# Antiparadox/Spartan-BN254

Hardware: AMD Instinct MI355X
Metric: msm_points_per_s (higher is better)
Workload: dtype u32; 1 GPU; synthetic BN254 G1 MSM, 2^20 uniform Fr scalars x distinct bases per GPU, inputs resident in HBM; steps_in_flight=6

## Files before the change

include/sbn254.h:

```cpp
#ifndef SBN254_H
#define SBN254_H
#include <stddef.h>
#include <stdint.h>
#ifdef __cplusplus
extern "C" {
#endif

#define SBN_OK 0
#define SBN_EINVAL (-1)
#define SBN_EHIP (-2)
#define SBN_ENODEV (-3)
#define SBN_ENOMEM (-4)

#define SBN_SCALARS_MONT 1u
#define SBN_POINTS_MONT 2u

typedef struct sbn_ctx sbn_ctx;
typedef struct sbn_bases sbn_bases;
typedef struct sbn_table sbn_table;

int sbn_ctx_create(int device, sbn_ctx** out);
void sbn_ctx_destroy(sbn_ctx* ctx);
const char* sbn_last_error(const sbn_ctx* ctx);
int sbn_ctx_set_stream(sbn_ctx* ctx, void* hip_stream);
int sbn_ctx_sync(sbn_ctx* ctx);
const char* sbn_version(void);

int sbn_dev_alloc(sbn_ctx* ctx, size_t bytes, void** out_dev);
int sbn_dev_free(sbn_ctx* ctx, void* dev);
int sbn_dev_upload(sbn_ctx* ctx, void* dst_dev, const void* src_host, size_t bytes);
int sbn_dev_download(sbn_ctx* ctx, void* dst_host, const void* src_dev, size_t bytes);

int sbn_msm(sbn_ctx* ctx, const uint8_t* scalars, const uint8_t* points, size_t n, uint32_t flags,
            uint8_t out_xy[64], int* out_is_inf);

int sbn_msm_jacobian(sbn_ctx* ctx, const uint8_t* scalars, const uint8_t* points_xyz, size_t n, uint32_t flags,
                     uint8_t out_xy[64], int* out_is_inf);

int sbn_bases_upload(sbn_ctx* ctx, const uint8_t* G_xy, size_t n, const uint8_t* h_xy, uint32_t flags, sbn_bases** out);
void sbn_bases_free(sbn_ctx* ctx, sbn_bases* b);
size_t sbn_bases_len(const sbn_bases* b);
int sbn_bases_precompute(sbn_ctx* ctx, sbn_bases* b, size_t max_bytes, int* window_bits);
int sbn_gens_new(sbn_ctx* ctx, size_t n, const uint8_t* label, size_t label_len, uint8_t* out_xy, sbn_bases** out);

int sbn_bases_synthetic(sbn_ctx* ctx, size_t n, uint64_t first, const uint8_t s0[32], const uint8_t d[32], sbn_bases** out);
int sbn_scalars_synthetic(sbn_ctx* ctx, uint64_t seed, uint64_t first, size_t n, void* out_dev);
int sbn_bases_download(sbn_ctx* ctx, const sbn_bases* b, size_t first, size_t count, uint8_t* out_xy);

int sbn_bases_split_at(sbn_ctx* ctx, const sbn_bases* b, size_t mid, sbn_bases** left, sbn_bases** right);
int sbn_bases_scale(sbn_ctx* ctx, const sbn_bases* b, const uint8_t s[32], sbn_bases** out);

int sbn_msm_bases(sbn_ctx* ctx, const sbn_bases* b, const uint8_t* scalars, size_t n, uint32_t flags,
                  uint8_t out_xy[64], int* out_is_inf);
int sbn_msm_bases_dev(sbn_ctx* ctx, const sbn_bases* b, const void* scalars_dev, size_t n, uint32_t flags,
                      uint8_t out_xy[64], int* out_is_inf);

int sbn_commit_rows(sbn_ctx* ctx, const sbn_bases* b, const uint8_t* Z, const uint8_t* blinds, size_t L, size_t R,
                    uint32_t flags, uint8_t* out_xy, uint8_t* out_inf);
int sbn_commit_rows_dev(sbn_ctx* ctx, const sbn_bases* b, const void* Z_dev, const void* blinds_dev, size_t L, size_t R,
                        uint32_t flags, uint8_t* out_xy, uint8_t* out_inf);
int sbn_g1_compress(const uint8_t* xy, size_t n, uint8_t* out32);
int sbn_g1_sum(const uint8_t* xy, size_t n, uint8_t out_xy[64], int* out_is_inf);
int sbn_unipoly_from_evals(const uint8_t* evals, size_t n, uint8_t* coeffs);
int sbn_unipoly_eval(const uint8_t* coeffs, size_t n, const uint8_t r[32], uint8_t out[32]);
void sbn_factored_lens(size_t ell, size_t* left, size_t* right);

int sbn_table_upload(sbn_ctx* ctx, const uint8_t* Z, size_t len, uint32_t flags, sbn_table** out);
int sbn_table_from_dev(sbn_ctx* ctx, const void* Z_dev, size_t len, uint32_t flags, sbn_table** out);
void sbn_table_free(sbn_ctx* ctx, sbn_table* t);
size_t sbn_table_len(const sbn_table* t);
int sbn_table_download(sbn_ctx* ctx, const sbn_table* t, uint8_t* out );
int sbn_table_read0(sbn_ctx* ctx, const sbn_table* t, uint8_t out[32]);
int sbn_table_read0_many(sbn_ctx* ctx, const sbn_table* const* ts, size_t count, uint8_t* out);
int sbn_bind_top(sbn_ctx* ctx, sbn_table* t, const uint8_t r[32]);
int sbn_bind_top_many(sbn_ctx* ctx, sbn_table* const* ts, size_t count, const uint8_t r[32]);
int sbn_sc_eval_cubic(sbn_ctx* ctx, const sbn_table* A, const sbn_table* B, const sbn_table* C, uint8_t out[96]);
int sbn_sc_eval_cubic_batched(sbn_ctx* ctx, const sbn_table* const* A, const sbn_table* const* B,
                              const sbn_table* const* C, size_t count, uint8_t* out );
int sbn_sc_eval_r1cs(sbn_ctx* ctx, const sbn_table* tau, const sbn_table* Az, const sbn_table* Bz, const sbn_table* Cz,
                     uint8_t out[96]);
int sbn_sc_eval_quad(sbn_ctx* ctx, const sbn_table* Z, const sbn_table* ABC, uint8_t out[64]);
int sbn_sc_bind_eval_cubic_batched(sbn_ctx* ctx, sbn_table* const* A, sbn_table* const* B, sbn_table* const* C, size_t count,
                                   const uint8_t r[32], uint8_t* out );
int sbn_sc_bind_eval_r1cs(sbn_ctx* ctx, sbn_table* tau, sbn_table* Az, sbn_table* Bz, sbn_table* Cz, const uint8_t r[32], uint8_t out[96]);
int sbn_sc_bind_eval_quad(sbn_ctx* ctx, sbn_table* Z, sbn_table* ABC, const uint8_t r[32], uint8_t out[64]);
typedef struct sbn_sumcheck sbn_sumcheck;
int sbn_sumcheck_begin(sbn_ctx* ctx, const sbn_table* const* A_par, const sbn_table* const* B_par, const sbn_table* C_par, size_t n_par,
                       const sbn_table* const* A_seq, const sbn_table* const* B_seq, const sbn_table* const* C_seq, size_t n_seq,
                       const uint8_t* coeffs, uint8_t out_evals[96], sbn_sumcheck** out);
int sbn_sumcheck_begin_eq(sbn_ctx* ctx, const sbn_table* const* A_par, const sbn_table* const* B_par, size_t n_par, const uint8_t* rand, size_t ell,
                          const sbn_table* const* A_seq, const sbn_table* const* B_seq, const sbn_table* const* C_seq, size_t n_seq,
                          const uint8_t* coeffs, uint8_t out_evals[96], sbn_sumcheck** out);
int sbn_sumcheck_round(sbn_ctx* ctx, sbn_sumcheck* st, const uint8_t r[32], uint8_t out_evals[96]);
size_t sbn_sumcheck_len(const sbn_sumcheck* st);
int sbn_sumcheck_finish(sbn_ctx* ctx, sbn_sumcheck* st, uint8_t* finals);
void sbn_sumcheck_free(sbn_ctx* ctx, sbn_sumcheck* st);
typedef struct sbn_transcript sbn_transcript;
int sbn_transcript_new(const uint8_t* label, size_t label_len, sbn_transcript** out);
int sbn_transcript_clone(const sbn_transcript* t, sbn_transcript** out);
void sbn_transcript_free(sbn_transcript* t);
int sbn_transcript_append_message(sbn_transcript* t, const uint8_t* label, size_t label_len, const uint8_t* msg, size_t msg_len);
int sbn_transcript_challenge_bytes(sbn_transcript* t, const uint8_t* label, size_t label_len, uint8_t* out, size_t out_len);
int sbn_transcript_challenge_scalar(sbn_transcript* t, const uint8_t* label, size_t label_len, uint8_t out[32]);
int sbn_transcript_state(const sbn_transcript* t, uint8_t out[203]);
int sbn_transcript_from_state(const uint8_t in[203], sbn_transcript** out);
int sbn_fr_from_wide(const uint8_t in[64], uint8_t out[32]);
int sbn_sumcheck_prove(sbn_ctx* ctx, sbn_sumcheck* st, sbn_transcript* tr, const uint8_t claim[32], uint8_t* out_polys, uint8_t* out_r, uint8_t* finals);
int sbn_product_proof_prove(sbn_ctx* ctx, const sbn_table* const* layers, size_t n_circ, size_t n_layers,
                            const sbn_table* const* dotp_left, const sbn_table* const* dotp_right, const sbn_table* const* dotp_weight, size_t n_dotp,
                            sbn_transcript* tr, uint8_t* out_polys, uint8_t* out_claims, uint8_t* out_rand, uint8_t* out_claims_final);
int sbn_eq_evals(sbn_ctx* ctx, const uint8_t* r, size_t ell, sbn_table** out);

int sbn_table_dot(sbn_ctx* ctx, const sbn_table* a, const sbn_table* b, uint8_t out[32]);
int sbn_table_evaluate(sbn_ctx* ctx, const sbn_table* Z, const uint8_t* r, size_t ell, uint8_t out[32]);
int sbn_table_evaluate_many(sbn_ctx* ctx, const sbn_table* const* Z, size_t count, const uint8_t* r, size_t ell, uint8_t* out);
int sbn_table_bound(sbn_ctx* ctx, const sbn_table* Z, const sbn_table* Lvec, sbn_table** out);

typedef struct sbn_bullet sbn_bullet;
int sbn_bullet_begin(sbn_ctx* ctx, const sbn_bases* G, const uint8_t* Q_xy, const sbn_table* a, const sbn_table* b, const uint8_t* blind,
                     uint8_t* Gamma_xy, int* Gamma_is_inf, sbn_bullet** out);
int sbn_bullet_begin_scaled(sbn_ctx* ctx, const sbn_bases* G, const uint8_t* Q_base_xy, const uint8_t q_scale[32], const sbn_table* a, const sbn_table* b,
                            const uint8_t* blind, uint8_t* Gamma_xy, int* Gamma_is_inf, sbn_bullet** out);
void sbn_bullet_free(sbn_ctx* ctx, sbn_bullet* st);
size_t sbn_bullet_len(const sbn_bullet* st);
int sbn_bullet_cross(sbn_ctx* ctx, sbn_bullet* st, const uint8_t* blind_L, const uint8_t* blind_R, uint8_t L_xy[64], int* L_is_inf,
                     uint8_t R_xy[64], int* R_is_inf, uint8_t c_L[32], uint8_t c_R[32]);
int sbn_bullet_fold(sbn_ctx* ctx, sbn_bullet* st, const uint8_t u[32], const uint8_t u_inv[32]);
int sbn_bullet_fold_cross(sbn_ctx* ctx, sbn_bullet* st, const uint8_t u[32], const uint8_t u_inv[32], const uint8_t* blind_L, const uint8_t* blind_R,
                          uint8_t L_xy[64], int* L_is_inf, uint8_t R_xy[64], int* R_is_inf, uint8_t c_L[32], uint8_t c_R[32]);
int sbn_bullet_finish(sbn_ctx* ctx, sbn_bullet* st, uint8_t a_hat[32], uint8_t b_hat[32], uint8_t g_hat_xy[64], int* g_hat_is_inf);

int sbn_polyeval_prove(sbn_ctx* ctx, const sbn_bases* gens, const sbn_table* Z, const uint8_t* blinds, const uint8_t* r, size_t ell, const uint8_t Zr[32],
                       const uint8_t* blind_Zr, const uint8_t* rnd, sbn_transcript* tr, uint8_t* out_proof,
                       uint8_t out_Cx_xy[64], int* Cx_is_inf, uint8_t out_Cy_xy[64], int* Cy_is_inf);
int sbn_joint_opening_prove(sbn_ctx* ctx, const sbn_bases* gens, const sbn_table* Z, const uint8_t* evals, size_t count,
                            const uint8_t* label_evals, size_t label_evals_len, const uint8_t* label_chal, size_t label_chal_len,
                            const uint8_t* label_claim, size_t label_claim_len, const uint8_t* r, size_t ell_r, const uint8_t* rnd, sbn_transcript* tr,
                            uint8_t* out_challenges, uint8_t out_joint_claim[32], uint8_t* out_proof,
                            uint8_t out_Cx_xy[64], int* Cx_is_inf, uint8_t out_Cy_xy[64], int* Cy_is_inf);

int sbn_zk_sumcheck_prove_r1cs(sbn_ctx* ctx, sbn_table* tau, sbn_table* Az, sbn_table* Bz, sbn_table* Cz,
                               const sbn_bases* gens_1, const sbn_bases* gens_4,
                               const uint8_t claim[32], const uint8_t blind_claim[32], const uint8_t* rnd, sbn_transcript* tr,
                               uint8_t* out_proof, uint8_t* out_r, uint8_t out_finals[128], uint8_t out_blind[32]);
int sbn_zk_sumcheck_prove_quad(sbn_ctx* ctx, sbn_table* Z, sbn_table* ABC,
                               const sbn_bases* gens_1, const sbn_bases* gens_3,
                               const uint8_t claim[32], const uint8_t blind_claim[32], const uint8_t* rnd, sbn_transcript* tr,
                               uint8_t* out_proof, uint8_t* out_r, uint8_t out_finals[64], uint8_t out_blind[32]);

int sbn_hash_layer(sbn_ctx* ctx, const void* addr_dev, const sbn_table* val, const void* ts_dev, uint32_t ts_add,
                   const uint8_t r_hash[32], const uint8_t r_multiset[32], sbn_table** out);
int sbn_hash_layer_pair(sbn_ctx* ctx, const void* addr_dev, const sbn_table* val, const void* ts_a_dev, uint32_t ts_a_add, const void* ts_b_dev, uint32_t ts_b_add,
                        const uint8_t r_hash[32], const uint8_t r_multiset[32], sbn_table** out_a, sbn_table** out_b);
int sbn_hash_layer_pair_product(sbn_ctx* ctx, const void* addr_dev, const sbn_table* val, const void* ts_a_dev, uint32_t ts_a_add, const void* ts_b_dev, uint32_t ts_b_add,
                                const uint8_t r_hash[32], const uint8_t r_multiset[32], sbn_table** out_a, sbn_table** out_b, sbn_table** prod_a, sbn_table** prod_b);
int sbn_product_layer(sbn_ctx* ctx, const sbn_table* in, sbn_table** out);
int sbn_product_circuit(sbn_ctx* ctx, const sbn_table* in, sbn_table** layers, size_t cap, size_t* count);
int sbn_product_circuit_many(sbn_ctx* ctx, const sbn_table* const* ins, size_t n, sbn_table** layers, size_t cap, size_t* count);
int sbn_table_halves(sbn_ctx* ctx, const sbn_table* t, sbn_table** left, sbn_table** right);

int sbn_table_slice(sbn_ctx* ctx, const sbn_table* t, size_t first, size_t len, sbn_table** out);

int sbn_gather_merge(sbn_ctx* ctx, const sbn_table* const* mem, const void* const* addr_dev, size_t count, size_t n, sbn_table** out);
int sbn_gather_merge_rows(sbn_ctx* ctx, const sbn_table* const* mem, const void* const* addr_dev, size_t count, size_t n, size_t R,
                          size_t row0, size_t rstep, size_t nrows, sbn_table** out);
int sbn_commit_table(sbn_ctx* ctx, const sbn_bases* b, const sbn_table* t, const uint8_t* blinds, size_t L, size_t R,
                     uint8_t* out_xy, uint8_t* out_inf);

typedef struct sbn_group sbn_group;
typedef struct sbn_group_bases sbn_group_bases;
int sbn_group_create(const int* devices, size_t n, sbn_group** out);
void sbn_group_destroy(sbn_group* g);
size_t sbn_group_size(const sbn_group* g);
sbn_ctx* sbn_group_ctx(sbn_group* g, size_t i);
const char* sbn_group_last_error(const sbn_group* g);
int sbn_group_bases_upload(sbn_group* g, const uint8_t* G_xy, size_t n, const uint8_t* h_xy, uint32_t flags, sbn_group_bases** out);
int sbn_group_gens_new(sbn_group* g, size_t n, const uint8_t* label, size_t label_len, uint8_t* out_xy, sbn_group_bases** out);
int sbn_group_bases_precompute(sbn_group* g, sbn_group_bases* gb, size_t max_bytes_per_device, int* window_bits);
void sbn_group_bases_free(sbn_group* g, sbn_group_bases* gb);
int sbn_group_commit_rows(sbn_group* g, const sbn_group_bases* gb, const uint8_t* Z, const uint8_t* blinds, size_t L, size_t R,
                          uint32_t flags, uint8_t* out_xy, uint8_t* out_inf);
int sbn_group_commit_rows_dev(sbn_group* g, const sbn_group_bases* gb, const void* const* Z_dev, const void* const* blinds_dev, size_t L, size_t R,
                              uint32_t flags, uint8_t* out_xy, uint8_t* out_inf);
int sbn_group_gather_commit(sbn_group* g, const sbn_group_bases* gb, const sbn_table* const* mem, const void* const* addr_dev, size_t count, size_t n,
                            size_t L, size_t R, uint8_t* out_xy, uint8_t* out_inf);
int sbn_group_msm(sbn_group* g, const uint8_t* scalars, const uint8_t* points, size_t n, uint32_t flags, uint8_t out_xy[64], int* out_is_inf);
int sbn_group_bases_upload_ranges(sbn_group* g, const uint8_t* G_xy, size_t n, uint32_t flags, sbn_group_bases** out);
int sbn_group_bases_synthetic_ranges(sbn_group* g, size_t n, const uint8_t s0[32], const uint8_t d[32], sbn_group_bases** out);
void sbn_group_range(const sbn_group_bases* gb, size_t device, size_t* lo, size_t* hi);
int sbn_group_msm_bases(sbn_group* g, const sbn_group_bases* gb, const uint8_t* scalars, size_t n, uint32_t flags, uint8_t out_xy[64], int* out_is_inf);
int sbn_group_msm_bases_dev(sbn_group* g, const sbn_group_bases* gb, const void* const* scalars_dev, uint32_t flags, uint8_t out_xy[64], int* out_is_inf);

int sbn_kzg_srs_upload(sbn_ctx* ctx, const uint8_t* powers_xy, size_t n, uint32_t flags, sbn_bases** out);
int sbn_kzg_srs_from_tau(sbn_ctx* ctx, const uint8_t tau[32], size_t n, sbn_bases** out);
int sbn_kzg_commit(sbn_ctx* ctx, const sbn_bases* srs, const sbn_table* t, size_t n, uint8_t out_xy[64], int* out_is_inf);
int sbn_poly_div_linear(sbn_ctx* ctx, const sbn_table* t, size_t n, const uint8_t z[32], uint8_t eval[32], sbn_table** q);
int sbn_kzg_open(sbn_ctx* ctx, const sbn_bases* srs, const sbn_table* t, size_t n, const uint8_t z[32],
                 uint8_t eval[32], uint8_t proof_xy[64], int* proof_is_inf);
int sbn_kzg_open_batched(sbn_ctx* ctx, const sbn_bases* srs, const sbn_table* const* ts, const size_t* ns, size_t count,
                         const uint8_t z[32], const uint8_t gamma[32], uint8_t* evals, uint8_t proof_xy[64], int* proof_is_inf);

typedef struct sbn_r1cs sbn_r1cs;
int sbn_r1cs_upload(sbn_ctx* ctx, size_t num_cons, size_t num_vars, const uint32_t* const* rows, const uint32_t* const* cols,
                    const uint8_t* const* vals, const size_t* nnz, uint32_t flags, sbn_r1cs** out);
void sbn_r1cs_free(sbn_ctx* ctx, sbn_r1cs* m);
int sbn_r1cs_multiply(sbn_ctx* ctx, const sbn_r1cs* m, const sbn_table* z, sbn_table** Az, sbn_table** Bz, sbn_table** Cz);
int sbn_r1cs_eval_table(sbn_ctx* ctx, const sbn_r1cs* m, const uint8_t* rx, size_t ell_x, const uint8_t rA[32], const uint8_t rB[32],
                        const uint8_t rC[32], sbn_table** out);
int sbn_r1cs_evaluate(sbn_ctx* ctx, const sbn_r1cs* m, const uint8_t* rx, size_t ell_x, const uint8_t* ry, size_t ell_y, uint8_t out[96]);

int sbn_r1cs_proof_sizes(size_t num_cons, size_t num_vars, size_t* rnd_scalars, size_t* proof_bytes);
int sbn_r1cs_proof_prove(sbn_ctx* ctx, const sbn_r1cs* inst, const sbn_table* vars, const uint8_t* input, size_t num_inputs,
                         const sbn_bases* gens_pc, const sbn_bases* gens_3, const sbn_bases* gens_4, const uint8_t* rnd, sbn_transcript* tr,
                         uint8_t* out_proof, uint8_t* out_rx, uint8_t* out_ry);

typedef struct sbn_dense sbn_dense;
int sbn_dense_build(sbn_ctx* ctx, size_t num_vars_x, size_t num_vars_y, const uint32_t* const* rows, const uint32_t* const* cols,
                    const uint8_t* const* vals, const size_t* nnz, size_t batch, uint32_t flags, sbn_dense** out);
void sbn_dense_free(sbn_ctx* ctx, sbn_dense* d);
size_t sbn_dense_num_ops(const sbn_dense* d);
size_t sbn_dense_num_cells(const sbn_dense* d);
size_t sbn_dense_batch(const sbn_dense* d);
const void* sbn_dense_addr_dev(const sbn_dense* d, int side, size_t k);
const void* sbn_dense_read_ts_dev(const sbn_dense* d, int side, size_t k);
const void* sbn_dense_audit_ts_dev(const sbn_dense* d, int side);
const sbn_table* sbn_dense_comb_ops(const sbn_dense* d);
const sbn_table* sbn_dense_comb_mem(const sbn_dense* d);

int sbn_sparse_eval_sizes(size_t num_vars_x, size_t num_vars_y, size_t num_ops , size_t batch, size_t* rnd_scalars, size_t* proof_bytes);
int sbn_sparse_eval_prove(sbn_ctx* ctx, const sbn_dense* dense, const uint8_t* rx, size_t nx, const uint8_t* ry, size_t ny, const uint8_t* evals ,
                          const sbn_bases* gens_ops, const sbn_bases* gens_mem, const sbn_bases* gens_derefs, const uint8_t* rnd, sbn_transcript* tr, uint8_t* out_proof);

typedef struct sbn_derefs_key sbn_derefs_key;
int sbn_derefs_key_build(sbn_ctx* ctx, const sbn_dense* dense, const sbn_bases* srs, sbn_derefs_key** out);
void sbn_derefs_key_free(sbn_ctx* ctx, sbn_derefs_key* key);
size_t sbn_derefs_key_len(const sbn_derefs_key* key);
int sbn_derefs_key_download(sbn_ctx* ctx, const sbn_derefs_key* key, size_t first, size_t count, uint32_t* out_cell, uint8_t* out_xy);
int sbn_derefs_key_commit(sbn_ctx* ctx, const sbn_derefs_key* key, const sbn_table* mem_rx, const sbn_table* mem_ry, uint8_t out_xy[64], int* out_is_inf);

int sbn_sparse_eval_kzg_sizes(size_t num_vars_x, size_t num_vars_y, size_t num_ops , size_t batch, size_t* rnd_scalars, size_t* proof_bytes);
int sbn_sparse_eval_prove_kzg(sbn_ctx* ctx, const sbn_dense* dense, const uint8_t* rx, size_t nx, const uint8_t* ry, size_t ny, const uint8_t* evals ,
                              const sbn_bases* gens_ops, const sbn_bases* gens_mem, const sbn_bases* srs, const sbn_derefs_key* key ,
                              const uint8_t* rnd, sbn_transcript* tr, uint8_t* out_proof);

int sbn_prof_enable(sbn_ctx* ctx, int on);
int sbn_prof_reset(sbn_ctx* ctx);
int sbn_prof_count(sbn_ctx* ctx);
int sbn_prof_get(sbn_ctx* ctx, int i, const char** name, double* total_ms, uint64_t* launches);
int sbn_prof_last_job(sbn_ctx* ctx, uint64_t out[4]);
int sbn_prof_last_acc(sbn_ctx* ctx, uint64_t out[8]);

int sbn_prof_last_polyeval(sbn_ctx* ctx, double out_us[3]);

#ifdef __cplusplus
}
#endif
#endif
```

spartan-bn254_amd/binding.py:

```python
import ctypes as C
import os
import subprocess

_HERE = os.path.dirname(os.path.abspath(__file__))
SBN_SCALARS_MONT = 1
SBN_POINTS_MONT = 2

EXPORTED_SYMBOLS = [
    "sbn_ctx_create", "sbn_ctx_destroy", "sbn_last_error", "sbn_ctx_set_stream", "sbn_ctx_sync", "sbn_version",
    "sbn_dev_alloc", "sbn_dev_free", "sbn_dev_upload", "sbn_dev_download",
    "sbn_msm", "sbn_msm_jacobian", "sbn_bases_split_at", "sbn_bases_scale", "sbn_bases_upload", "sbn_bases_precompute", "sbn_bases_free", "sbn_bases_len", "sbn_gens_new", "sbn_bases_synthetic", "sbn_scalars_synthetic", "sbn_bases_download",
    "sbn_msm_bases", "sbn_msm_bases_dev", "sbn_commit_rows", "sbn_commit_rows_dev", "sbn_g1_compress", "sbn_g1_sum", "sbn_unipoly_from_evals", "sbn_unipoly_eval", "sbn_factored_lens",
    "sbn_table_upload", "sbn_table_from_dev", "sbn_table_free", "sbn_table_len", "sbn_table_download", "sbn_table_read0", "sbn_table_read0_many",
    "sbn_bind_top", "sbn_bind_top_many", "sbn_sc_eval_cubic", "sbn_sc_eval_cubic_batched", "sbn_sc_eval_r1cs", "sbn_sc_eval_quad",
    "sbn_sc_bind_eval_cubic_batched", "sbn_sc_bind_eval_r1cs", "sbn_sc_bind_eval_quad",
    "sbn_sumcheck_begin", "sbn_sumcheck_begin_eq", "sbn_sumcheck_round", "sbn_sumcheck_len", "sbn_sumcheck_finish", "sbn_sumcheck_free",
    "sbn_transcript_new", "sbn_transcript_clone", "sbn_transcript_free", "sbn_transcript_append_message", "sbn_transcript_challenge_bytes", "sbn_transcript_challenge_scalar",
    "sbn_transcript_state", "sbn_transcript_from_state", "sbn_fr_from_wide", "sbn_sumcheck_prove", "sbn_product_proof_prove",
    "sbn_polyeval_prove", "sbn_joint_opening_prove", "sbn_prof_last_polyeval", "sbn_zk_sumcheck_prove_r1cs", "sbn_zk_sumcheck_prove_quad",
    "sbn_group_create", "sbn_group_destroy", "sbn_group_size", "sbn_group_ctx", "sbn_group_last_error", "sbn_group_bases_upload", "sbn_group_gens_new", "sbn_group_bases_precompute",
    "sbn_group_bases_free", "sbn_group_commit_rows", "sbn_group_commit_rows_dev", "sbn_group_gather_commit", "sbn_group_msm", "sbn_group_bases_upload_ranges", "sbn_group_bases_synthetic_ranges", "sbn_group_range", "sbn_group_msm_bases", "sbn_group_msm_bases_dev",
    "sbn_eq_evals", "sbn_hash_layer", "sbn_hash_layer_pair", "sbn_hash_layer_pair_product", "sbn_product_layer", "sbn_product_circuit", "sbn_product_circuit_many", "sbn_table_halves", "sbn_table_slice", "sbn_table_dot", "sbn_table_evaluate", "sbn_table_evaluate_many", "sbn_table_bound", "sbn_gather_merge", "sbn_gather_merge_rows", "sbn_commit_table", "sbn_bullet_begin", "sbn_bullet_begin_scaled", "sbn_bullet_free", "sbn_bullet_len", "sbn_bullet_cross", "sbn_bullet_fold_cross", "sbn_bullet_fold", "sbn_bullet_finish", "sbn_prof_enable", "sbn_prof_reset", "sbn_prof_count", "sbn_prof_get", "sbn_prof_last_job", "sbn_prof_last_acc",
    "sbn_kzg_srs_upload", "sbn_kzg_srs_from_tau", "sbn_kzg_commit", "sbn_poly_div_linear", "sbn_kzg_open", "sbn_kzg_open_batched",
    "sbn_r1cs_upload", "sbn_r1cs_free", "sbn_r1cs_multiply", "sbn_r1cs_eval_table", "sbn_r1cs_evaluate",
    "sbn_r1cs_proof_sizes", "sbn_r1cs_proof_prove", "sbn_sparse_eval_sizes", "sbn_sparse_eval_prove",
    "sbn_derefs_key_build", "sbn_derefs_key_free", "sbn_derefs_key_len", "sbn_derefs_key_download", "sbn_derefs_key_commit",
    "sbn_sparse_eval_kzg_sizes", "sbn_sparse_eval_prove_kzg",
    "sbn_dense_build", "sbn_dense_free", "sbn_dense_num_ops", "sbn_dense_num_cells", "sbn_dense_batch", "sbn_dense_addr_dev", "sbn_dense_read_ts_dev",
    "sbn_dense_audit_ts_dev", "sbn_dense_comb_ops", "sbn_dense_comb_mem",
]


class SbnError(RuntimeError):
    pass


def lib_path():
    return os.path.join(_HERE, "libsbn254_hip.so")


def build_library():
    subprocess.run(["make", "-s", "-C", _HERE], check=True)
    return lib_path()


_LIB = None


def lib():
    global _LIB
    if _LIB is None:
        try:
            import torch
        except ImportError:
            pass
        p = lib_path()
        if not os.path.exists(p):
            raise SbnError(f"{p} is missing: run `make -C {_HERE}` (or __graft_entry__.build()); there is no CPU fallback")
        L = C.CDLL(p)
        L.sbn_last_error.restype = C.c_char_p
        L.sbn_version.restype = C.c_char_p
        missing = [s for s in EXPORTED_SYMBOLS if not hasattr(L, s)]
        if missing:
            raise SbnError(f"{p} does not export {missing}; rebuild it")
        L.sbn_bases_len.restype = C.c_size_t
        L.sbn_table_len.restype = C.c_size_t
        L.sbn_bullet_len.restype = C.c_size_t
        L.sbn_sumcheck_len.restype = C.c_size_t
        L.sbn_group_size.restype = C.c_size_t
        L.sbn_group_ctx.restype = C.c_void_p
        L.sbn_group_last_error.restype = C.c_char_p
        L.sbn_factored_lens.restype = None
        for name in ("sbn_ctx_destroy", "sbn_bases_free", "sbn_table_free", "sbn_bullet_free", "sbn_sumcheck_free", "sbn_group_destroy", "sbn_group_bases_free", "sbn_group_range", "sbn_r1cs_free", "sbn_dense_free", "sbn_transcript_free"):
            getattr(L, name).restype = None
        for name in ("sbn_dense_num_ops", "sbn_dense_num_cells", "sbn_dense_batch"):
            getattr(L, name).restype = C.c_size_t; getattr(L, name).argtypes = [C.c_void_p]
        for name in ("sbn_dense_addr_dev", "sbn_dense_read_ts_dev"):
            getattr(L, name).restype = C.c_void_p; getattr(L, name).argtypes = [C.c_void_p, C.c_int, C.c_size_t]
        L.sbn_transcript_free.argtypes = [C.c_void_p]
        L.sbn_sumcheck_prove.argtypes = [C.c_void_p] * 7
        L.sbn_product_proof_prove.argtypes = [C.c_void_p, C.c_void_p, C.c_size_t, C.c_size_t, C.c_void_p, C.c_void_p, C.c_void_p, C.c_size_t] + [C.c_void_p] * 5
        L.sbn_polyeval_prove.argtypes = [C.c_void_p] * 5 + [C.c_size_t] + [C.c_void_p] * 9
        L.sbn_joint_opening_prove.argtypes = [C.c_void_p] * 4 + [C.c_size_t] + [C.c_void_p, C.c_size_t] * 3 + [C.c_void_p, C.c_size_t] + [C.c_void_p] * 9
        L.sbn_zk_sumcheck_prove_r1cs.argtypes = [C.c_void_p] * 15
        L.sbn_zk_sumcheck_prove_quad.argtypes = [C.c_void_p] * 13
        L.sbn_r1cs_proof_sizes.argtypes = [C.c_size_t, C.c_size_t, C.c_void_p, C.c_void_p]
        L.sbn_r1cs_proof_prove.argtypes = [C.c_void_p] * 4 + [C.c_size_t] + [C.c_void_p] * 8
        L.sbn_sparse_eval_sizes.argtypes = [C.c_size_t] * 4 + [C.c_void_p] * 2
        L.sbn_sparse_eval_prove.argtypes = [C.c_void_p] * 3 + [C.c_size_t, C.c_void_p, C.c_size_t] + [C.c_void_p] * 7
        L.sbn_sparse_eval_kzg_sizes.argtypes = [C.c_size_t] * 4 + [C.c_void_p] * 2
        L.sbn_sparse_eval_prove_kzg.argtypes = [C.c_void_p] * 3 + [C.c_size_t, C.c_void_p, C.c_size_t] + [C.c_void_p] * 8
        L.sbn_derefs_key_build.argtypes = [C.c_void_p] * 4
        L.sbn_derefs_key_free.restype = None; L.sbn_derefs_key_free.argtypes = [C.c_void_p] * 2
        L.sbn_derefs_key_len.restype = C.c_size_t; L.sbn_derefs_key_len.argtypes = [C.c_void_p]
        L.sbn_derefs_key_download.argtypes = [C.c_void_p, C.c_void_p, C.c_size_t, C.c_size_t, C.c_void_p, C.c_void_p]
        L.sbn_derefs_key_commit.argtypes = [C.c_void_p] * 6
        L.sbn_dense_audit_ts_dev.restype = C.c_void_p; L.sbn_dense_audit_ts_dev.argtypes = [C.c_void_p, C.c_int]
        for name in ("sbn_dense_comb_ops", "sbn_dense_comb_mem"):
            getattr(L, name).restype = C.c_void_p; getattr(L, name).argtypes = [C.c_void_p]
        _LIB = L
    return _LIB


HARNESS_STAGES = ["r1cs_sat_proof", "eq_evals", "derefs_computation", "derefs_commitment", "network_construction", "network_proof",
                  "sub_witness_commit", "sub_phase1_sumcheck", "sub_phase2_sumcheck", "sub_witness_opening", "sub_ops_sumchecks", "sub_mem_sumchecks",
                  "sub_evaluations", "sub_openings"]


class HarnessParams(C.Structure):
    _fields_ = [("log_ops", C.c_int32), ("log_mem", C.c_int32), ("log_cons", C.c_int32), ("stateful_sumcheck", C.c_int32),
                ("lookup_bytes_sat", C.c_uint64), ("lookup_bytes_eval", C.c_uint64), ("seed", C.c_uint64), ("rounds_out", C.c_uint32 * 4),
                ("passes", C.c_uint32), ("trace_markers", C.c_uint32)]


_HARNESS = None


def harness_lib():
    global _HARNESS
    if _HARNESS is None:
        lib()
        p = os.path.join(_HERE, "libsbn_prove_harness.so")
        if not os.path.exists(p):
            raise SbnError(f"{p} is missing: run `make -C {_HERE}`")
        _HARNESS = C.CDLL(p)
    return _HARNESS


def harness_prove(ctx, log_ops, log_mem, log_cons, stateful=True, lookup_bytes_sat=0, lookup_bytes_eval=0, seed=1, trace_cap=0, passes=1, trace_markers=False):
    prm = HarnessParams(log_ops, log_mem, log_cons, 1 if stateful else 0, lookup_bytes_sat, lookup_bytes_eval, seed)
    prm.passes = passes
    prm.trace_markers = 1 if trace_markers else 0
    ms = (C.c_double * 16)(); dig = (C.c_uint8 * 32)(); err = C.create_string_buffer(512)
    tr = (C.c_uint8 * trace_cap)() if trace_cap else None; tl = C.c_size_t(0)
    rc = harness_lib().sbn_harness_prove(ctx.h, C.byref(prm), ms, dig, tr, C.c_size_t(trace_cap), C.byref(tl), err, C.c_size_t(512))
    if rc:
        raise SbnError("sbn_harness_prove: " + err.value.decode())
    stages = {n: ms[i] for i, n in enumerate(HARNESS_STAGES)}
    rounds = {"sumcheck_rounds_ops": prm.rounds_out[0], "sumcheck_rounds_mem": prm.rounds_out[1], "bullet_rounds": prm.rounds_out[2], "layers": prm.rounds_out[3]}
    return stages, bytes(dig), (bytes(tr[:tl.value]) if trace_cap else b""), rounds


def _ptr(x):
    if x is None:
        return None
    if isinstance(x, (bytes, bytearray)):
        return (C.c_uint8 * len(x)).from_buffer_copy(x) if isinstance(x, bytes) else (C.c_uint8 * len(x)).from_buffer(x)
    if hasattr(x, "ctypes"):
        return x.ctypes.data_as(C.POINTER(C.c_uint8))
    raise TypeError(type(x))


def g1_compress(xy):
    n = len(xy) // 64
    out = (C.c_uint8 * (32 * n))()
    rc = lib().sbn_g1_compress(_ptr(xy), C.c_size_t(n), out)
    if rc:
        raise SbnError(f"sbn_g1_compress rc={rc}")
    return bytes(out)


def g1_sum(xy):
    n = len(xy) // 64
    out = (C.c_uint8 * 64)(); inf = C.c_int()
    rc = lib().sbn_g1_sum(_ptr(xy), C.c_size_t(n), out, C.byref(inf))
    if rc:
        raise SbnError(f"sbn_g1_sum rc={rc}")
    return bytes(out), bool(inf.value)


def unipoly_from_evals(evals):
    n = len(evals) // 32; out = (C.c_uint8 * (32 * n))()
    rc = lib().sbn_unipoly_from_evals(_ptr(evals), C.c_size_t(n), out)
    if rc:
        raise SbnError(f"sbn_unipoly_from_evals rc={rc}")
    return bytes(out)


def unipoly_eval(coeffs, r):
    out = (C.c_uint8 * 32)()
    rc = lib().sbn_unipoly_eval(_ptr(coeffs), C.c_size_t(len(coeffs) // 32), _ptr(r), out)
    if rc:
        raise SbnError(f"sbn_unipoly_eval rc={rc}")
    return bytes(out)


def r1cs_proof_sizes(num_cons, num_vars):
    a, b = C.c_size_t(0), C.c_size_t(0)
    rc = lib().sbn_r1cs_proof_sizes(C.c_size_t(num_cons), C.c_size_t(num_vars), C.byref(a), C.byref(b))
    if rc != 0:
        raise SbnError(f"sbn_r1cs_proof_sizes: {num_cons} x {num_vars} is a shape the call refuses (rc={rc})")
    return a.value, b.value


def factored_lens(ell):
    a, b = C.c_size_t(), C.c_size_t()
    lib().sbn_factored_lens(C.c_size_t(ell), C.byref(a), C.byref(b))
    return a.value, b.value


class Bases:
    def __init__(self, ctx, handle):
        self.ctx, self.h = ctx, handle

    def __len__(self):
        return lib().sbn_bases_len(self.h)

    def free(self):
        if self.h:
            lib().sbn_bases_free(self.ctx.h, self.h)
            self.h = None


class Bullet:
    def __init__(self, ctx, handle):
        self.ctx, self.h = ctx, handle

    def __len__(self):
        return lib().sbn_bullet_len(self.h)

    def free(self):
        if self.h:
            lib().sbn_bullet_free(self.ctx.h, self.h)
            self.h = None


def fr_from_wide(b64):
    if len(b64) != 64:
        raise ValueError("64 bytes are needed")
    out = (C.c_uint8 * 32)()
    rc = lib().sbn_fr_from_wide(_ptr(b64), out)
    if rc:
        raise SbnError(f"sbn_fr_from_wide rc={rc}")
    return bytes(out)


class Transcript:

    def __init__(self, label=None, _handle=None):
        if _handle is None:
            _handle = C.c_void_p()
            self._chk(lib().sbn_transcript_new(_ptr(label), C.c_size_t(len(label)), C.byref(_handle)), "sbn_transcript_new")
        self.h = _handle

    @staticmethod
    def _chk(rc, what):
        if rc:
            raise SbnError(f"{what} rc={rc}")

    def append_message(self, label, msg):
        self._chk(lib().sbn_transcript_append_message(self.h, _ptr(label), C.c_size_t(len(label)), _ptr(msg), C.c_size_t(len(msg))), "sbn_transcript_append_message")

    def append_scalar(self, label, scalar32):
        self.append_message(label, scalar32)

    def challenge_bytes(self, label, n):
        out = (C.c_uint8 * max(n, 1))()
        self._chk(lib().sbn_transcript_challenge_bytes(self.h, _ptr(label), C.c_size_t(len(label)), out, C.c_size_t(n)), "sbn_transcript_challenge_bytes")
        return bytes(out[:n])

    def challenge_scalar(self, label):
        out = (C.c_uint8 * 32)()
        self._chk(lib().sbn_transcript_challenge_scalar(self.h, _ptr(label), C.c_size_t(len(label)), out), "sbn_transcript_challenge_scalar")
        return bytes(out)

    def state(self):
        out = (C.c_uint8 * 203)()
        self._chk(lib().sbn_transcript_state(self.h, out), "sbn_transcript_state")
        return bytes(out)

    @classmethod
    def from_state(cls, rec):
        if len(rec) != 203:
            raise ValueError("a transcript state record has 203 bytes")
        h = C.c_void_p()
        cls._chk(lib().sbn_transcript_from_state(_ptr(rec), C.byref(h)), "sbn_transcript_from_state")
        return cls(_handle=h)

    def clone(self):
        h = C.c_void_p()
        self._chk(lib().sbn_transcript_clone(self.h, C.byref(h)), "sbn_transcript_clone")
        return Transcript(_handle=h)

    def free(self):
        if self.h:
            lib().sbn_transcript_free(self.h)
            self.h = None

    def __del__(self):
        try:
            self.free()
        except Exception:
            pass


class Sumcheck:

    def __init__(self, ctx, handle, n_par, n_seq):
        self.ctx, self.h, self.ntab = ctx, handle, 2 * n_par + (1 if n_par else 0) + 3 * n_seq

    def __len__(self):
        return lib().sbn_sumcheck_len(self.h)

    def round(self, r):
        out = (C.c_uint8 * 96)()
        self.ctx._chk(lib().sbn_sumcheck_round(self.ctx.h, self.h, _ptr(r), out), "sbn_sumcheck_round")
        return bytes(out)

    def finish(self):
        out = (C.c_uint8 * (32 * self.ntab))()
        self.ctx._chk(lib().sbn_sumcheck_finish(self.ctx.h, self.h, out), "sbn_sumcheck_finish")
        return [bytes(out[32 * t:32 * t + 32]) for t in range(self.ntab)]

    def free(self):
        if self.h:
            lib().sbn_sumcheck_free(self.ctx.h, self.h)
            self.h = None


class Table:
    def __init__(self, ctx, handle):
        self.ctx, self.h = ctx, handle

    def __len__(self):
        return lib().sbn_table_len(self.h)

    def free(self):
        if self.h:
            lib().sbn_table_free(self.ctx.h, self.h)
            self.h = None


class _BorrowedTable(Table):

    def free(self):
        self.h = None


class R1cs:

    def __init__(self, ctx, handle, num_cons, num_vars):
        self.ctx, self.h, self.num_cons, self.num_vars = ctx, handle, num_cons, num_vars

    def free(self):
        if self.h:
            lib().sbn_r1cs_free(self.ctx.h, self.h)
            self.h = None


def sparse_eval_sizes(num_vars_x, num_vars_y, num_ops, batch):
    a, b = C.c_size_t(0), C.c_size_t(0)
    rc = lib().sbn_sparse_eval_sizes(C.c_size_t(num_vars_x), C.c_size_t(num_vars_y), C.c_size_t(num_ops), C.c_size_t(batch), C.byref(a), C.byref(b))
    if rc:
        raise SbnError(f"sbn_sparse_eval_sizes: ({num_vars_x}, {num_vars_y}, N = {num_ops}, batch = {batch}) is a shape the call refuses (rc={rc})")
    return a.value, b.value


def sparse_eval_kzg_sizes(num_vars_x, num_vars_y, num_ops, batch):
    a, b = C.c_size_t(0), C.c_size_t(0)
    rc = lib().sbn_sparse_eval_kzg_sizes(C.c_size_t(num_vars_x), C.c_size_t(num_vars_y), C.c_size_t(num_ops), C.c_size_t(batch), C.byref(a), C.byref(b))
    if rc:
        raise SbnError(f"sbn_sparse_eval_kzg_sizes: ({num_vars_x}, {num_vars_y}, N = {num_ops}, batch = {batch}) is a shape the call refuses (rc={rc})")
    return a.value, b.value


class DerefsKey:

    def __init__(self, ctx, handle):
        self.ctx, self.h = ctx, handle

    def __len__(self):
        return lib().sbn_derefs_key_len(self.h)

    def download(self, first=0, count=None):
        count = len(self) - first if count is None else count
        ids = (C.c_uint32 * max(count, 1))(); xy = (C.c_uint8 * (64 * max(count, 1)))()
        self.ctx._chk(lib().sbn_derefs_key_download(self.ctx.h, self.h, C.c_size_t(first), C.c_size_t(count), ids, xy), "sbn_derefs_key_download")
        raw = bytes(xy)
        return [int(ids[j]) for j in range(count)], [raw[64 * j:64 * j + 64] for j in range(count)]

    def free(self):
        if self.h:
            lib().sbn_derefs_key_free(self.ctx.h, self.h)
            self.h = None


class Dense:

    def __init__(self, ctx, handle):
        self.ctx, self.h = ctx, handle
        self.num_ops = lib().sbn_dense_num_ops(handle); self.num_cells = lib().sbn_dense_num_cells(handle); self.batch = lib().sbn_dense_batch(handle)
        self.comb_ops = _BorrowedTable(ctx, C.c_void_p(lib().sbn_dense_comb_ops(handle)))
        self.comb_mem = _BorrowedTable(ctx, C.c_void_p(lib().sbn_dense_comb_mem(handle)))

    def addr_dev(self, side, k):
        return lib().sbn_dense_addr_dev(self.h, side, k)

    def read_ts_dev(self, side, k):
        return lib().sbn_dense_read_ts_dev(self.h, side, k)

    def audit_ts_dev(self, side):
        return lib().sbn_dense_audit_ts_dev(self.h, side)

    def ops_slice(self, group, j):
        return self.ctx.table_slice(self.comb_ops, (group * self.batch + j) * self.num_ops, self.num_ops)

    def free(self):
        if self.h:
            self.comb_ops.h = self.comb_mem.h = None
            lib().sbn_dense_free(self.ctx.h, self.h)
            self.h = None


class GroupBases:
    def __init__(self, group, handle):
        self.group, self.h = group, handle

    def range(self, device):
        lo, hi = C.c_size_t(), C.c_size_t()
        lib().sbn_group_range(self.h, C.c_size_t(device), C.byref(lo), C.byref(hi)); return lo.value, hi.value

    def free(self):
        if self.h:
            lib().sbn_group_bases_free(self.group.h, self.h); self.h = None


class Group:

    def __init__(self, devices):
        self.h = C.c_void_p()
        arr = (C.c_int * len(devices))(*devices)
        rc = lib().sbn_group_create(arr, C.c_size_t(len(devices)), C.byref(self.h))
        if rc:
            raise SbnError(f"sbn_group_create failed rc={rc}")

    def close(self):
        if self.h:
            lib().sbn_group_destroy(self.h); self.h = None

    def __len__(self):
        return lib().sbn_group_size(self.h)

    def _chk(self, rc, what):
        if rc:
            raise SbnError(f"{what}: rc={rc}: {lib().sbn_group_last_error(self.h).decode()}")

    def ctx(self, i):
        c = Context.__new__(Context); c.h = C.c_void_p(lib().sbn_group_ctx(self.h, C.c_size_t(i))); c.owned = False
        return c

    def bases_upload(self, G_xy, h_xy=None, flags=0):
        o = C.c_void_p()
        self._chk(lib().sbn_group_bases_upload(self.h, _ptr(G_xy), C.c_size_t(len(G_xy) // 64), _ptr(h_xy), C.c_uint32(flags), C.byref(o)), "sbn_group_bases_upload")
        return GroupBases(self, o)

    def gens_new(self, n, label, want_points=True):
        o = C.c_void_p(); out = (C.c_uint8 * (64 * (n + 1)))() if want_points else None
        self._chk(lib().sbn_group_gens_new(self.h, C.c_size_t(n), _ptr(label), C.c_size_t(len(label)), out, C.byref(o)), "sbn_group_gens_new")
        return GroupBases(self, o), (bytes(out) if want_points else None)

    def bases_precompute(self, gb, max_bytes_per_device):
        cw = C.c_int(0)
        self._chk(lib().sbn_group_bases_precompute(self.h, gb.h, C.c_size_t(max_bytes_per_device), C.byref(cw)), "sbn_group_bases_precompute"); return cw.value

    def commit_rows(self, gb, Z, blinds, L, R, flags=0):
        out = (C.c_uint8 * (64 * L))(); inf = (C.c_uint8 * L)()
        self._chk(lib().sbn_group_commit_rows(self.h, gb.h, _ptr(Z), _ptr(blinds), C.c_size_t(L), C.c_size_t(R), C.c_uint32(flags), out, inf), "sbn_group_commit_rows")
        return bytes(out), bytes(inf)

    def commit_rows_dev(self, gb, z_ptrs, blind_ptrs, L, R, flags=0):
        N = len(self)
        za = (C.c_void_p * N)(*z_ptrs); ba = (C.c_void_p * N)(*blind_ptrs) if blind_ptrs is not None else None
        out = (C.c_uint8 * (64 * L))(); inf = (C.c_uint8 * L)()
        self._chk(lib().sbn_group_commit_rows_dev(self.h, gb.h, za, ba, C.c_size_t(L), C.c_size_t(R), C.c_uint32(flags), out, inf), "sbn_group_commit_rows_dev")
        return bytes(out), bytes(inf)

    def gather_commit(self, gb, mem, addr_ptrs, n, L, R):
        N = len(self); count = len(mem[0])
        ma = (C.c_void_p * (N * count))(*[t.h for row in mem for t in row])
        aa = (C.c_void_p * (N * count))(*[a for row in addr_ptrs for a in row])
        out = (C.c_uint8 * (64 * L))(); inf = (C.c_uint8 * L)()
        self._chk(lib().sbn_group_gather_commit(self.h, gb.h, ma, aa, C.c_size_t(count), C.c_size_t(n), C.c_size_t(L), C.c_size_t(R), out, inf), "sbn_group_gather_commit")
        return bytes(out), bytes(inf)

    def msm(self, scalars, points, flags=0):
        out = (C.c_uint8 * 64)(); inf = C.c_int()
        self._chk(lib().sbn_group_msm(self.h, _ptr(scalars), _ptr(points), C.c_size_t(len(scalars) // 32), C.c_uint32(flags), out, C.byref(inf)), "sbn_group_msm")
        return bytes(out), bool(inf.value)

    def bases_upload_ranges(self, G_xy, flags=0):
        o = C.c_void_p()
        self._chk(lib().sbn_group_bases_upload_ranges(self.h, _ptr(G_xy), C.c_size_t(len(G_xy) // 64), C.c_uint32(flags), C.byref(o)), "sbn_group_bases_upload_ranges")
        return GroupBases(self, o)

    def bases_synthetic_ranges(self, n, s0, d):
        o = C.c_void_p()
        self._chk(lib().sbn_group_bases_synthetic_ranges(self.h, C.c_size_t(n), _ptr(s0), _ptr(d), C.byref(o)), "sbn_group_bases_synthetic_ranges")
        return GroupBases(self, o)

    def msm_bases(self, gb, scalars, flags=0):
        out = (C.c_uint8 * 64)(); inf = C.c_int()
        self._chk(lib().sbn_group_msm_bases(self.h, gb.h, _ptr(scalars), C.c_size_t(len(scalars) // 32), C.c_uint32(flags), out, C.byref(inf)), "sbn_group_msm_bases")
        return bytes(out), bool(inf.value)

    def msm_bases_dev(self, gb, dev_ptrs, flags=0):
        arr = (C.c_void_p * len(dev_ptrs))(*dev_ptrs); out = (C.c_uint8 * 64)(); inf = C.c_int()
        self._chk(lib().sbn_group_msm_bases_dev(self.h, gb.h, arr, C.c_uint32(flags), out, C.byref(inf)), "sbn_group_msm_bases_dev")
        return bytes(out), bool(inf.value)


class Context:
    owned = True

    def __init__(self, device=0):
        self.h = C.c_void_p()
        rc = lib().sbn_ctx_create(device, C.byref(self.h))
        if rc:
            raise SbnError(f"sbn_ctx_create failed rc={rc} (no gfx950 device? there is no CPU fallback)")

    def close(self):
        if self.h and self.owned:
            lib().sbn_ctx_destroy(self.h)
        self.h = None

    def __enter__(self):
        return self

    def __exit__(self, *a):
        self.close()

    def _chk(self, rc, what):
        if rc:
            raise SbnError(f"{what}: rc={rc}: {lib().sbn_last_error(self.h).decode()}")

    def set_stream(self, stream_ptr):
        self._chk(lib().sbn_ctx_set_stream(self.h, C.c_void_p(stream_ptr)), "set_stream")

    def sync(self):
        self._chk(lib().sbn_ctx_sync(self.h), "sync")

    def msm(self, scalars, points, flags=0):
        n = len(scalars) // 32
        assert len(points) == 64 * n
        out = (C.c_uint8 * 64)(); inf = C.c_int()
        self._chk(lib().sbn_msm(self.h, _ptr(scalars), _ptr(points), C.c_size_t(n), C.c_uint32(flags), out, C.byref(inf)), "sbn_msm")
        return bytes(out), bool(inf.value)

    def msm_jacobian(self, scalars, points_xyz, flags=0):
        n = len(scalars) // 32
        assert len(points_xyz) == 96 * n
        out = (C.c_uint8 * 64)(); inf = C.c_int()
        self._chk(lib().sbn_msm_jacobian(self.h, _ptr(scalars), _ptr(points_xyz), C.c_size_t(n), C.c_uint32(flags), out, C.byref(inf)), "sbn_msm_jacobian")
        return bytes(out), bool(inf.value)

    def bases_precompute(self, bases, max_bytes):
        cw = C.c_int(0)
        self._chk(lib().sbn_bases_precompute(self.h, bases.h, C.c_size_t(max_bytes), C.byref(cw)), "sbn_bases_precompute")
        return cw.value

    def bases_split_at(self, bases, mid):
        l, r = C.c_void_p(), C.c_void_p()
        self._chk(lib().sbn_bases_split_at(self.h, bases.h, C.c_size_t(mid), C.byref(l), C.byref(r)), "sbn_bases_split_at")
        return Bases(self, l), Bases(self, r)

    def bases_scale(self, bases, s):
        o = C.c_void_p()
        self._chk(lib().sbn_bases_scale(self.h, bases.h, _ptr(s), C.byref(o)), "sbn_bases_scale")
        return Bases(self, o)

    def bases_upload(self, G_xy, h_xy=None, flags=0):
        n = len(G_xy) // 64
        hb = C.c_void_p()
        self._chk(lib().sbn_bases_upload(self.h, _ptr(G_xy), C.c_size_t(n), _ptr(h_xy), C.c_uint32(flags), C.byref(hb)), "sbn_bases_upload")
        return Bases(self, hb)

    def gens_new(self, n, label, want_points=True):
        hb = C.c_void_p()
        out = (C.c_uint8 * (64 * (n + 1)))() if want_points else None
        self._chk(lib().sbn_gens_new(self.h, C.c_size_t(n), _ptr(label), C.c_size_t(len(label)), out, C.byref(hb)), "sbn_gens_new")
        return Bases(self, hb), (bytes(out) if want_points else None)

    def bases_synthetic(self, n, first, s0, d):
        hb = C.c_void_p()
        self._chk(lib().sbn_bases_synthetic(self.h, C.c_size_t(n), C.c_uint64(first), _ptr(s0), _ptr(d), C.byref(hb)), "sbn_bases_synthetic")
        return Bases(self, hb)

    def scalars_synthetic(self, seed, first, n, out_dev_ptr):
        self._chk(lib().sbn_scalars_synthetic(self.h, C.c_uint64(seed), C.c_uint64(first), C.c_size_t(n), C.c_void_p(out_dev_ptr)), "sbn_scalars_synthetic")

    def bases_download(self, bases, first, count):
        out = (C.c_uint8 * (64 * count))()
        self._chk(lib().sbn_bases_download(self.h, bases.h, C.c_size_t(first), C.c_size_t(count), out), "sbn_bases_download")
        return bytes(out)

    def msm_bases(self, bases, scalars, flags=0):
        n = len(scalars) // 32
        out = (C.c_uint8 * 64)(); inf = C.c_int()
        self._chk(lib().sbn_msm_bases(self.h, bases.h, _ptr(scalars), C.c_size_t(n), C.c_uint32(flags), out, C.byref(inf)), "sbn_msm_bases")
        return bytes(out), bool(inf.value)

    def msm_bases_dev(self, bases, scalars_dev_ptr, n, flags=0):
        out = (C.c_uint8 * 64)(); inf = C.c_int()
        self._chk(lib().sbn_msm_bases_dev(self.h, bases.h, C.c_void_p(scalars_dev_ptr), C.c_size_t(n), C.c_uint32(flags), out, C.byref(inf)), "sbn_msm_bases_dev")
        return bytes(out), bool(inf.value)

    def commit_rows(self, bases, Z, blinds, L, R, flags=0):
        out = (C.c_uint8 * (64 * L))(); inf = (C.c_uint8 * L)()
        self._chk(lib().sbn_commit_rows(self.h, bases.h, _ptr(Z), _ptr(blinds), C.c_size_t(L), C.c_size_t(R), C.c_uint32(flags), out, inf), "sbn_commit_rows")
        return bytes(out), bytes(inf)

    def commit_rows_dev(self, bases, Z_dev_ptr, blinds_dev_ptr, L, R, flags=0):
        out = (C.c_uint8 * (64 * L))(); inf = (C.c_uint8 * L)()
        self._chk(lib().sbn_commit_rows_dev(self.h, bases.h, C.c_void_p(Z_dev_ptr), C.c_void_p(blinds_dev_ptr or 0), C.c_size_t(L), C.c_size_t(R), C.c_uint32(flags), out, inf), "sbn_commit_rows_dev")
        return bytes(out), bytes(inf)

    def dev_alloc(self, nbytes):
        p = C.c_void_p(); self._chk(lib().sbn_dev_alloc(self.h, C.c_size_t(nbytes), C.byref(p)), "sbn_dev_alloc"); return p.value

    def dev_free(self, p):
        self._chk(lib().sbn_dev_free(self.h, C.c_void_p(p)), "sbn_dev_free")

    def dev_upload(self, dst, data):
        self._chk(lib().sbn_dev_upload(self.h, C.c_void_p(dst), _ptr(data), C.c_size_t(len(data) if not hasattr(data, "nbytes") else data.nbytes)), "sbn_dev_upload")

    def dev_download(self, src, nbytes):
        out = (C.c_uint8 * nbytes)(); self._chk(lib().sbn_dev_download(self.h, out, C.c_void_p(src), C.c_size_t(nbytes)), "sbn_dev_download"); return bytes(out)

    def table_upload(self, Z, flags=0):
        n = len(Z) // 32; ht = C.c_void_p()
        self._chk(lib().sbn_table_upload(self.h, _ptr(Z), C.c_size_t(n), C.c_uint32(flags), C.byref(ht)), "sbn_table_upload")
        return Table(self, ht)

    def table_from_dev(self, dev_ptr, n, flags=0):
        ht = C.c_void_p()
        self._chk(lib().sbn_table_from_dev(self.h, C.c_void_p(dev_ptr), C.c_size_t(n), C.c_uint32(flags), C.byref(ht)), "sbn_table_from_dev")
        return Table(self, ht)

    def table_download(self, t):
        n = len(t); out = (C.c_uint8 * (32 * n))()
        self._chk(lib().sbn_table_download(self.h, t.h, out), "sbn_table_download"); return bytes(out)

    def table_read0(self, t):
        out = (C.c_uint8 * 32)(); self._chk(lib().sbn_table_read0(self.h, t.h, out), "sbn_table_read0"); return bytes(out)

    def table_read0_many(self, ts):
        n = len(ts)
        arr = (C.c_void_p * max(n, 1))(*[t.h for t in ts]); out = (C.c_uint8 * (32 * max(n, 1)))()
        self._chk(lib().sbn_table_read0_many(self.h, arr, C.c_size_t(n), out), "sbn_table_read0_many")
        return [bytes(out[32 * i:32 * i + 32]) for i in range(n)]

    def bind_top(self, t, r):
        self._chk(lib().sbn_bind_top(self.h, t.h, _ptr(r)), "sbn_bind_top")

    def bind_top_many(self, ts, r):
        arr = (C.c_void_p * len(ts))(*[t.h for t in ts])
        self._chk(lib().sbn_bind_top_many(self.h, arr, C.c_size_t(len(ts)), _ptr(r)), "sbn_bind_top_many")

    def sc_eval_cubic(self, A, B, Cc):
        out = (C.c_uint8 * 96)(); self._chk(lib().sbn_sc_eval_cubic(self.h, A.h, B.h, Cc.h, out), "sbn_sc_eval_cubic"); return bytes(out)

    def sc_eval_cubic_batched(self, As, Bs, Cs):
        k = len(As); mk = lambda ts: (C.c_void_p * k)(*[t.h for t in ts])
        out = (C.c_uint8 * (96 * k))()
        self._chk(lib().sbn_sc_eval_cubic_batched(self.h, mk(As), mk(Bs), mk(Cs), C.c_size_t(k), out), "sbn_sc_eval_cubic_batched"); return bytes(out)

    def sc_eval_r1cs(self, T, A, B, Cc):
        out = (C.c_uint8 * 96)(); self._chk(lib().sbn_sc_eval_r1cs(self.h, T.h, A.h, B.h, Cc.h, out), "sbn_sc_eval_r1cs"); return bytes(out)

    def sc_eval_quad(self, Z, ABC):
        out = (C.c_uint8 * 64)(); self._chk(lib().sbn_sc_eval_quad(self.h, Z.h, ABC.h, out), "sbn_sc_eval_quad"); return bytes(out)

    def sc_bind_eval_cubic_batched(self, As, Bs, Cs, r):
        k = len(As); mk = lambda ts: (C.c_void_p * k)(*[t.h for t in ts])
        out = (C.c_uint8 * (96 * k))()
        self._chk(lib().sbn_sc_bind_eval_cubic_batched(self.h, mk(As), mk(Bs), mk(Cs), C.c_size_t(k), _ptr(r), out), "sbn_sc_bind_eval_cubic_batched"); return bytes(out)

    def sc_bind_eval_r1cs(self, T, A, B, Cc, r):
        out = (C.c_uint8 * 96)(); self._chk(lib().sbn_sc_bind_eval_r1cs(self.h, T.h, A.h, B.h, Cc.h, _ptr(r), out), "sbn_sc_bind_eval_r1cs"); return bytes(out)

    def sc_bind_eval_quad(self, Z, ABC, r):
        out = (C.c_uint8 * 64)(); self._chk(lib().sbn_sc_bind_eval_quad(self.h, Z.h, ABC.h, _ptr(r), out), "sbn_sc_bind_eval_quad"); return bytes(out)

    def sumcheck_begin(self, A_par, B_par, C_par, A_seq, B_seq, C_seq, coeffs):
        mk = lambda ts: (C.c_void_p * max(1, len(ts)))(*[t.h for t in ts])
        st = C.c_void_p(); out = (C.c_uint8 * 96)()
        self._chk(lib().sbn_sumcheck_begin(self.h, mk(A_par), mk(B_par), C_par.h if C_par is not None else None, C.c_size_t(len(A_par)),
                                           mk(A_seq), mk(B_seq), mk(C_seq), C.c_size_t(len(A_seq)), _ptr(coeffs), out, C.byref(st)), "sbn_sumcheck_begin")
        return Sumcheck(self, st, len(A_par), len(A_seq)), bytes(out)

    def sumcheck_begin_eq(self, A_par, B_par, rand, A_seq, B_seq, C_seq, coeffs):
        mk = lambda ts: (C.c_void_p * max(1, len(ts)))(*[t.h for t in ts])
        st = C.c_void_p(); out = (C.c_uint8 * 96)()
        self._chk(lib().sbn_sumcheck_begin_eq(self.h, mk(A_par), mk(B_par), C.c_size_t(len(A_par)), _ptr(rand), C.c_size_t(len(rand) // 32),
                                              mk(A_seq), mk(B_seq), mk(C_seq), C.c_size_t(len(A_seq)), _ptr(coeffs), out, C.byref(st)), "sbn_sumcheck_begin_eq")
        return Sumcheck(self, st, len(A_par), len(A_seq)), bytes(out)

    def sumcheck_prove(self, st, tr, claim):
        n = len(st)
        rounds = n.bit_length() - 1
        polys = (C.c_uint8 * (128 * max(rounds, 1)))(); rs = (C.c_uint8 * (32 * max(rounds, 1)))(); fin = (C.c_uint8 * (32 * st.ntab))()
        self._chk(lib().sbn_sumcheck_prove(self.h, st.h, tr.h, _ptr(claim), polys, rs, fin), "sbn_sumcheck_prove")
        pb, rb = bytes(polys), bytes(rs)
        return ([[pb[128 * j + 32 * k:128 * j + 32 * k + 32] for k in range(4)] for j in range(rounds)], [rb[32 * j:32 * j + 32] for j in range(rounds)],
                [bytes(fin[32 * t:32 * t + 32]) for t in range(st.ntab)])

    def product_proof_prove(self, layers, dotps, tr):
        n, L, nd = len(layers), len(layers[0]), len(dotps)
        arr = (C.c_void_p * (n * L))(*[layers[i][j].h for i in range(n) for j in range(L)])
        mk = lambda k: (C.c_void_p * max(1, nd))(*[d[k].h for d in dotps])
        polys = (C.c_uint8 * (128 * max(1, L * (L - 1) // 2)))(); claims = (C.c_uint8 * (32 * (2 * n * L + 3 * nd)))()
        rand = (C.c_uint8 * (32 * L))(); fin = (C.c_uint8 * (32 * n))()
        self._chk(lib().sbn_product_proof_prove(self.h, arr, C.c_size_t(n), C.c_size_t(L), mk(0), mk(1), mk(2), C.c_size_t(nd), tr.h, polys, claims, rand, fin),
                  "sbn_product_proof_prove")
        return bytes(polys)[:128 * (L * (L - 1) // 2)], bytes(claims), bytes(rand), bytes(fin)

    def eq_evals(self, r):
        ell = len(r) // 32; ht = C.c_void_p()
        self._chk(lib().sbn_eq_evals(self.h, _ptr(r), C.c_size_t(ell), C.byref(ht)), "sbn_eq_evals"); return Table(self, ht)

    def hash_layer(self, addr_dev_ptr, val, ts_dev_ptr, ts_add, r_hash, r_multiset):
        ht = C.c_void_p()
        self._chk(lib().sbn_hash_layer(self.h, C.c_void_p(addr_dev_ptr or 0), val.h, C.c_void_p(ts_dev_ptr or 0), C.c_uint32(ts_add), _ptr(r_hash), _ptr(r_multiset), C.byref(ht)), "sbn_hash_layer")
        return Table(self, ht)

    def hash_layer_pair(self, addr_dev_ptr, val, ts_a_ptr, ts_a_add, ts_b_ptr, ts_b_add, r_hash, r_multiset):
        ha, hb = C.c_void_p(), C.c_void_p()
        self._chk(lib().sbn_hash_layer_pair(self.h, C.c_void_p(addr_dev_ptr or 0), val.h, C.c_void_p(ts_a_ptr or 0), C.c_uint32(ts_a_add), C.c_void_p(ts_b_ptr or 0), C.c_uint32(ts_b_add),
                                            _ptr(r_hash), _ptr(r_multiset), C.byref(ha), C.byref(hb)), "sbn_hash_layer_pair")
        return Table(self, ha), Table(self, hb)

    def hash_layer_pair_product(self, addr_dev_ptr, val, ts_a_ptr, ts_a_add, ts_b_ptr, ts_b_add, r_hash, r_multiset):
        hs = [C.c_void_p() for _ in range(4)]
        self._chk(lib().sbn_hash_layer_pair_product(self.h, C.c_void_p(addr_dev_ptr or 0), val.h, C.c_void_p(ts_a_ptr or 0), C.c_uint32(ts_a_add), C.c_void_p(ts_b_ptr or 0),
                                                    C.c_uint32(ts_b_add), _ptr(r_hash), _ptr(r_multiset), *[C.byref(h) for h in hs]), "sbn_hash_layer_pair_product")
        return tuple(Table(self, h) for h in hs)

    def product_layer(self, t):
        ht = C.c_void_p(); self._chk(lib().sbn_product_layer(self.h, t.h, C.byref(ht)), "sbn_product_layer"); return Table(self, ht)

    def product_circuit(self, t):
        cap = max(1, len(t).bit_length())
        arr = (C.c_void_p * cap)(); cnt = C.c_size_t(0)
        self._chk(lib().sbn_product_circuit(self.h, t.h, arr, C.c_size_t(cap), C.byref(cnt)), "sbn_product_circuit")
        return [Table(self, C.c_void_p(arr[i])) for i in range(cnt.value)]

    def product_circuit_many(self, ts):
        n = len(ts); cap = max(1, len(ts[0]).bit_length())
        ins = (C.c_void_p * n)(*[t.h for t in ts]); arr = (C.c_void_p * (n * cap))(); cnt = C.c_size_t(0)
        self._chk(lib().sbn_product_circuit_many(self.h, ins, C.c_size_t(n), arr, C.c_size_t(cap), C.byref(cnt)), "sbn_product_circuit_many")
        return [[Table(self, C.c_void_p(arr[i * cap + k])) for k in range(cnt.value)] for i in range(n)]

    def table_halves(self, t):
        l, r = C.c_void_p(), C.c_void_p()
        self._chk(lib().sbn_table_halves(self.h, t.h, C.byref(l), C.byref(r)), "sbn_table_halves"); return Table(self, l), Table(self, r)

    def table_dot(self, a, b):
        out = (C.c_uint8 * 32)(); self._chk(lib().sbn_table_dot(self.h, a.h, b.h, out), "sbn_table_dot"); return bytes(out)

    def table_evaluate(self, Z, r):
        out = (C.c_uint8 * 32)(); self._chk(lib().sbn_table_evaluate(self.h, Z.h, _ptr(r), C.c_size_t(len(r) // 32), out), "sbn_table_evaluate"); return bytes(out)

    def table_evaluate_many(self, Zs, r):
        k = len(Zs); arr = (C.c_void_p * k)(*[t.h for t in Zs]); out = (C.c_uint8 * (32 * k))()
        self._chk(lib().sbn_table_evaluate_many(self.h, arr, C.c_size_t(k), _ptr(r), C.c_size_t(len(r) // 32), out), "sbn_table_evaluate_many")
        return bytes(out)

    def table_bound(self, Z, Lvec):
        ht = C.c_void_p(); self._chk(lib().sbn_table_bound(self.h, Z.h, Lvec.h, C.byref(ht)), "sbn_table_bound"); return Table(self, ht)

    def table_slice(self, t, first, length):
        ht = C.c_void_p()
        self._chk(lib().sbn_table_slice(self.h, t.h, C.c_size_t(first), C.c_size_t(length), C.byref(ht)), "sbn_table_slice")
        return Table(self, ht)

    def gather_merge(self, mems, addr_dev_ptrs, n):
        k = len(mems)
        ma = (C.c_void_p * k)(*[t.h for t in mems]); aa = (C.c_void_p * k)(*addr_dev_ptrs)
        ht = C.c_void_p()
        self._chk(lib().sbn_gather_merge(self.h, ma, aa, C.c_size_t(k), C.c_size_t(n), C.byref(ht)), "sbn_gather_merge")
        return Table(self, ht)

    def gather_merge_rows(self, mems, addr_dev_ptrs, n, R, row0, rstep, nrows):
        k = len(mems)
        ma = (C.c_void_p * k)(*[t.h for t in mems]); aa = (C.c_void_p * k)(*addr_dev_ptrs)
        ht = C.c_void_p()
        self._chk(lib().sbn_gather_merge_rows(self.h, ma, aa, C.c_size_t(k), C.c_size_t(n), C.c_size_t(R), C.c_size_t(row0), C.c_size_t(rstep), C.c_size_t(nrows), C.byref(ht)), "sbn_gather_merge_rows")
        return Table(self, ht)

    def commit_table(self, bases, t, blinds, L, R):
        out = (C.c_uint8 * (64 * L))(); inf = (C.c_uint8 * L)()
        self._chk(lib().sbn_commit_table(self.h, bases.h, t.h, _ptr(blinds), C.c_size_t(L), C.c_size_t(R), out, inf), "sbn_commit_table")
        return bytes(out), bytes(inf)

    def bullet_begin(self, G, Q_xy, a, b, blind=None, want_gamma=True):
        st = C.c_void_p(); gm = (C.c_uint8 * 64)() if want_gamma else None; gi = C.c_int(0)
        self._chk(lib().sbn_bullet_begin(self.h, G.h, _ptr(Q_xy), a.h, b.h, _ptr(blind), gm, C.byref(gi), C.byref(st)), "sbn_bullet_begin")
        return Bullet(self, st), (bytes(gm) if want_gamma else None)

    def bullet_begin_scaled(self, G, Q_base_xy, q_scale, a, b, blind=None, want_gamma=True):
        st = C.c_void_p(); gm = (C.c_uint8 * 64)() if want_gamma else None; gi = C.c_int(0)
        self._chk(lib().sbn_bullet_begin_scaled(self.h, G.h, _ptr(Q_base_xy), _ptr(q_scale), a.h, b.h, _ptr(blind), gm, C.byref(gi), C.byref(st)), "sbn_bullet_begin_scaled")
        return Bullet(self, st), (bytes(gm) if want_gamma else None)

    def bullet_cross(self, st, blind_L=None, blind_R=None):
        Lo, Ro = (C.c_uint8 * 64)(), (C.c_uint8 * 64)(); li, ri = C.c_int(0), C.c_int(0)
        cl, cr = (C.c_uint8 * 32)(), (C.c_uint8 * 32)()
        self._chk(lib().sbn_bullet_cross(self.h, st.h, _ptr(blind_L), _ptr(blind_R), Lo, C.byref(li), Ro, C.byref(ri), cl, cr), "sbn_bullet_cross")
        return bytes(Lo), bool(li.value), bytes(Ro), bool(ri.value), bytes(cl), bytes(cr)

    def bullet_fold_cross(self, st, u, u_inv, blind_L=None, blind_R=None):
        Lo, Ro = (C.c_uint8 * 64)(), (C.c_uint8 * 64)(); li, ri = C.c_int(0), C.c_int(0)
        cl, cr = (C.c_uint8 * 32)(), (C.c_uint8 * 32)()
        self._chk(lib().sbn_bullet_fold_cross(self.h, st.h, _ptr(u), _ptr(u_inv), _ptr(blind_L), _ptr(blind_R), Lo, C.byref(li), Ro, C.byref(ri), cl, cr), "sbn_bullet_fold_cross")
        return bytes(Lo), bool(li.value), bytes(Ro), bool(ri.value), bytes(cl), bytes(cr)

    def bullet_fold(self, st, u, u_inv):
        self._chk(lib().sbn_bullet_fold(self.h, st.h, _ptr(u), _ptr(u_inv)), "sbn_bullet_fold")

    def bullet_finish(self, st):
        ah, bh, gh = (C.c_uint8 * 32)(), (C.c_uint8 * 32)(), (C.c_uint8 * 64)(); gi = C.c_int(0)
        self._chk(lib().sbn_bullet_finish(self.h, st.h, ah, bh, gh, C.byref(gi)), "sbn_bullet_finish")
        return bytes(ah), bytes(bh), bytes(gh)

    def polyeval_prove(self, gens, Z, r, Zr, rnd, tr, blinds=None, blind_Zr=None):
        ell = len(r) // 32
        lg = ell - ell // 2
        proof = (C.c_uint8 * (64 * lg + 128))(); cx, cy = (C.c_uint8 * 64)(), (C.c_uint8 * 64)(); xi, yi = C.c_int(0), C.c_int(0)
        self._chk(lib().sbn_polyeval_prove(self.h, gens.h, Z.h, _ptr(blinds), _ptr(r), C.c_size_t(ell), _ptr(Zr), _ptr(blind_Zr), _ptr(rnd), tr.h,
                                           proof, cx, C.byref(xi), cy, C.byref(yi)), "sbn_polyeval_prove")
        return bytes(proof), bytes(cx), bytes(cy)

    def joint_opening_prove(self, gens, Z, evals, labels, r, rnd, tr):
        count = len(evals) // 32
        lc = count.bit_length() - 1
        ell = lc + len(r) // 32
        lg = ell - ell // 2
        ch = (C.c_uint8 * max(32 * lc, 1))(); claim = (C.c_uint8 * 32)()
        proof = (C.c_uint8 * (64 * lg + 128))(); cx, cy = (C.c_uint8 * 64)(), (C.c_uint8 * 64)(); xi, yi = C.c_int(0), C.c_int(0)
        le, lch, lcl = labels
        self._chk(lib().sbn_joint_opening_prove(self.h, gens.h, Z.h, _ptr(evals), C.c_size_t(count), _ptr(le), C.c_size_t(len(le)), _ptr(lch), C.c_size_t(len(lch)),
                                                _ptr(lcl), C.c_size_t(len(lcl)), _ptr(r), C.c_size_t(len(r) // 32), _ptr(rnd), tr.h, ch, claim, proof,
                                                cx, C.byref(xi), cy, C.byref(yi)), "sbn_joint_opening_prove")
        return bytes(ch[:32 * lc]), bytes(claim), bytes(proof), bytes(cx), bytes(cy)

    def prof_last_polyeval(self):
        out = (C.c_double * 3)()
        self._chk(lib().sbn_prof_last_polyeval(self.h, out), "sbn_prof_last_polyeval")
        return tuple(out)

    def _zk_sumcheck_prove(self, fn, name, tables, n, gens_1, gens_n, claim, blind_claim, rnd, tr):
        rounds = max(len(tables[0]).bit_length() - 1, 0)
        proof = (C.c_uint8 * max((6 + n) * 32 * rounds, 1))(); rs = (C.c_uint8 * max(32 * rounds, 1))()
        fin = (C.c_uint8 * (32 * len(tables)))(); bl = (C.c_uint8 * 32)()
        self._chk(fn(self.h, *[t.h for t in tables], gens_1.h, gens_n.h, _ptr(claim), _ptr(blind_claim), _ptr(rnd), tr.h, proof, rs, fin, bl), name)
        return bytes(proof[:(6 + n) * 32 * rounds]), bytes(rs[:32 * rounds]), bytes(fin), bytes(bl)

    def zk_sumcheck_prove_r1cs(self, tau, Az, Bz, Cz, gens_1, gens_4, claim, blind_claim, rnd, tr):
        return self._zk_sumcheck_prove(lib().sbn_zk_sumcheck_prove_r1cs, "sbn_zk_sumcheck_prove_r1cs", (tau, Az, Bz, Cz), 4, gens_1, gens_4, claim, blind_claim, rnd, tr)

    def zk_sumcheck_prove_quad(self, Z, ABC, gens_1, gens_3, claim, blind_claim, rnd, tr):
        return self._zk_sumcheck_prove(lib().sbn_zk_sumcheck_prove_quad, "sbn_zk_sumcheck_prove_quad", (Z, ABC), 3, gens_1, gens_3, claim, blind_claim, rnd, tr)

    def r1cs_proof_prove(self, inst, vars, inputs, gens_pc, gens_3, gens_4, rnd, tr):
        n_rnd, n_proof = r1cs_proof_sizes(inst.num_cons, inst.num_vars)
        if len(rnd) != 32 * n_rnd:
            raise ValueError(f"r1cs_proof_prove: rnd holds {len(rnd)} bytes, the shape needs {32 * n_rnd}")
        nx, ny = inst.num_cons.bit_length() - 1, inst.num_vars.bit_length()
        proof = (C.c_uint8 * n_proof)(); rx = (C.c_uint8 * (32 * nx))(); ry = (C.c_uint8 * (32 * ny))()
        self._chk(lib().sbn_r1cs_proof_prove(self.h, inst.h, vars.h, _ptr(inputs) if inputs else None, C.c_size_t(len(inputs) // 32 if inputs else 0),
                                             gens_pc.h, gens_3.h, gens_4.h, _ptr(rnd), tr.h, proof, rx, ry), "sbn_r1cs_proof_prove")
        return bytes(proof), bytes(rx), bytes(ry)

    def sparse_eval_prove(self, dense, rx, ry, evals, gens_ops, gens_mem, gens_derefs, rnd, tr):
        nx, ny = len(rx) // 32, len(ry) // 32
        n_rnd, n_proof = sparse_eval_sizes(nx, ny, dense.num_ops, dense.batch)
        if len(rnd) != 32 * n_rnd:
            raise ValueError(f"sparse_eval_prove: rnd holds {len(rnd)} bytes, the shape needs {32 * n_rnd}")
        if len(evals) != 32 * dense.batch:
            raise ValueError(f"sparse_eval_prove: evals holds {len(evals)} bytes, the batch needs {32 * dense.batch}  [sparse_mlpoly_full.rs:1711 assert_eq]")
        proof = (C.c_uint8 * n_proof)()
        self._chk(lib().sbn_sparse_eval_prove(self.h, dense.h, _ptr(rx) if rx else None, C.c_size_t(nx), _ptr(ry) if ry else None, C.c_size_t(ny), _ptr(evals),
                                              gens_ops.h, gens_mem.h, gens_derefs.h, _ptr(rnd), tr.h, proof), "sbn_sparse_eval_prove")
        return bytes(proof)

    def derefs_key_build(self, dense, srs):
        h = C.c_void_p()
        self._chk(lib().sbn_derefs_key_build(self.h, dense.h, srs.h, C.byref(h)), "sbn_derefs_key_build")
        return DerefsKey(self, h)

    def derefs_key_commit(self, key, mem_rx, mem_ry):
        out = (C.c_uint8 * 64)(); inf = C.c_int()
        self._chk(lib().sbn_derefs_key_commit(self.h, key.h, mem_rx.h, mem_ry.h, out, C.byref(inf)), "sbn_derefs_key_commit")
        return bytes(out), bool(inf.value)

    def sparse_eval_prove_kzg(self, dense, rx, ry, evals, gens_ops, gens_mem, srs, key, rnd, tr):
        nx, ny = len(rx) // 32, len(ry) // 32
        n_rnd, n_proof = sparse_eval_kzg_sizes(nx, ny, dense.num_ops, dense.batch)
        if len(rnd) != 32 * n_rnd:
            raise ValueError(f"sparse_eval_prove_kzg: rnd holds {len(rnd)} bytes, the shape needs {32 * n_rnd}")
        if len(evals) != 32 * dense.batch:
            raise ValueError(f"sparse_eval_prove_kzg: evals holds {len(evals)} bytes, the batch needs {32 * dense.batch}  [sparse_mlpoly_full.rs:1769 assert_eq]")
        proof = (C.c_uint8 * n_proof)()
        self._chk(lib().sbn_sparse_eval_prove_kzg(self.h, dense.h, _ptr(rx) if rx else None, C.c_size_t(nx), _ptr(ry) if ry else None, C.c_size_t(ny), _ptr(evals),
                                                  gens_ops.h, gens_mem.h, srs.h, key.h if key is not None else None, _ptr(rnd), tr.h, proof), "sbn_sparse_eval_prove_kzg")
        return bytes(proof)

    def kzg_srs_upload(self, powers_xy, flags=0):
        hb = C.c_void_p()
        self._chk(lib().sbn_kzg_srs_upload(self.h, _ptr(powers_xy), C.c_size_t(len(powers_xy) // 64), C.c_uint32(flags), C.byref(hb)), "sbn_kzg_srs_upload")
        return Bases(self, hb)

    def kzg_srs_from_tau(self, tau, n):
        hb = C.c_void_p()
        self._chk(lib().sbn_kzg_srs_from_tau(self.h, _ptr(tau), C.c_size_t(n), C.byref(hb)), "sbn_kzg_srs_from_tau")
        return Bases(self, hb)

    def kzg_commit(self, srs, t, n=None):
        out = (C.c_uint8 * 64)(); inf = C.c_int()
        self._chk(lib().sbn_kzg_commit(self.h, srs.h, t.h, C.c_size_t(len(t) if n is None else n), out, C.byref(inf)), "sbn_kzg_commit")
        return bytes(out), bool(inf.value)

    def poly_div_linear(self, t, n, z):
        ev = (C.c_uint8 * 32)(); q = C.c_void_p()
        self._chk(lib().sbn_poly_div_linear(self.h, t.h, C.c_size_t(n), _ptr(z), ev, C.byref(q)), "sbn_poly_div_linear")
        return bytes(ev), (Table(self, q) if q.value else None)

    def kzg_open(self, srs, t, n, z):
        ev = (C.c_uint8 * 32)(); out = (C.c_uint8 * 64)(); inf = C.c_int()
        self._chk(lib().sbn_kzg_open(self.h, srs.h, t.h, C.c_size_t(n), _ptr(z), ev, out, C.byref(inf)), "sbn_kzg_open")
        return bytes(ev), bytes(out), bool(inf.value)

    def kzg_open_batched(self, srs, ts, ns, z, gamma):
        k = len(ts)
        arr = (C.c_void_p * max(k, 1))(*[t.h for t in ts]); nn = (C.c_size_t * max(k, 1))(*ns)
        ev = (C.c_uint8 * (32 * max(k, 1)))(); out = (C.c_uint8 * 64)(); inf = C.c_int()
        self._chk(lib().sbn_kzg_open_batched(self.h, srs.h, arr, nn, C.c_size_t(k), _ptr(z), _ptr(gamma), ev, out, C.byref(inf)), "sbn_kzg_open_batched")
        return [bytes(ev[32 * i:32 * i + 32]) for i in range(k)], bytes(out), bool(inf.value)

    def r1cs_upload(self, num_cons, num_vars, mats, flags=0):
        import numpy as np
        if len(mats) != 3:
            raise ValueError("r1cs_upload: mats must hold A, B and C")
        keep, rows, cols, vals, nnz = [], (C.c_void_p * 3)(), (C.c_void_p * 3)(), (C.c_void_p * 3)(), (C.c_size_t * 3)()
        for m, (r, c, v) in enumerate(mats):
            r = np.ascontiguousarray(r, dtype=np.uint32); c = np.ascontiguousarray(c, dtype=np.uint32)
            v = np.frombuffer(v, dtype=np.uint8) if isinstance(v, (bytes, bytearray)) else np.ascontiguousarray(v, dtype=np.uint8).reshape(-1)
            n = len(r)
            if len(c) != n or len(v) != 32 * n:
                raise ValueError(f"r1cs_upload: matrix {m}: {n} rows, {len(c)} cols, {len(v)} value bytes")
            keep += [r, c, v]
            nnz[m] = n
            rows[m] = r.ctypes.data if n else None; cols[m] = c.ctypes.data if n else None; vals[m] = v.ctypes.data if n else None
        h = C.c_void_p()
        self._chk(lib().sbn_r1cs_upload(self.h, C.c_size_t(num_cons), C.c_size_t(num_vars), rows, cols, vals, nnz, C.c_uint32(flags), C.byref(h)),
                  "sbn_r1cs_upload")
        return R1cs(self, h, num_cons, num_vars)

    def r1cs_multiply(self, m, z):
        a, b, c = C.c_void_p(), C.c_void_p(), C.c_void_p()
        self._chk(lib().sbn_r1cs_multiply(self.h, m.h, z.h, C.byref(a), C.byref(b), C.byref(c)), "sbn_r1cs_multiply")
        return Table(self, a), Table(self, b), Table(self, c)

    def r1cs_eval_table(self, m, rx, rA, rB, rC):
        ht = C.c_void_p()
        self._chk(lib().sbn_r1cs_eval_table(self.h, m.h, _ptr(rx), C.c_size_t(len(rx) // 32), _ptr(rA), _ptr(rB), _ptr(rC), C.byref(ht)),
                  "sbn_r1cs_eval_table")
        return Table(self, ht)

    def r1cs_evaluate(self, m, rx, ry):
        out = (C.c_uint8 * 96)()
        self._chk(lib().sbn_r1cs_evaluate(self.h, m.h, _ptr(rx), C.c_size_t(len(rx) // 32), _ptr(ry), C.c_size_t(len(ry) // 32), out),
                  "sbn_r1cs_evaluate")
        return bytes(out[0:32]), bytes(out[32:64]), bytes(out[64:96])

    def dense_build(self, num_vars_x, num_vars_y, mats, flags=0):
        import numpy as np
        b = len(mats); nb = max(b, 1)
        keep, rows, cols, vals, nnz = [], (C.c_void_p * nb)(), (C.c_void_p * nb)(), (C.c_void_p * nb)(), (C.c_size_t * nb)()
        for m, (r, c, v) in enumerate(mats):
            r = np.ascontiguousarray(r, dtype=np.uint32); c = np.ascontiguousarray(c, dtype=np.uint32)
            v = np.frombuffer(v, dtype=np.uint8) if isinstance(v, (bytes, bytearray)) else np.ascontiguousarray(v, dtype=np.uint8).reshape(-1)
            n = len(r)
            if len(c) != n or len(v) != 32 * n:
                raise ValueError(f"dense_build: matrix {m}: {n} rows, {len(c)} cols, {len(v)} value bytes")
            keep += [r, c, v]
            nnz[m] = n
            rows[m] = r.ctypes.data if n else None; cols[m] = c.ctypes.data if n else None; vals[m] = v.ctypes.data if n else None
        h = C.c_void_p()
        self._chk(lib().sbn_dense_build(self.h, C.c_size_t(num_vars_x), C.c_size_t(num_vars_y), rows, cols, vals, nnz, C.c_size_t(b), C.c_uint32(flags),
                                        C.byref(h)), "sbn_dense_build")
        return Dense(self, h)

    def prof_enable(self, on=True):
        self._chk(lib().sbn_prof_enable(self.h, int(on)), "prof_enable")

    def prof_last_job(self):
        o = (C.c_uint64 * 4)(); self._chk(lib().sbn_prof_last_job(self.h, o), "prof_last_job")
        return {"c": int(o[0]), "W": int(o[1]), "slots": int(o[2]), "buckets": int(o[3])}

    def prof_last_acc(self):
        o = (C.c_uint64 * 8)(); self._chk(lib().sbn_prof_last_acc(self.h, o), "prof_last_acc")
        return dict(zip(("SEG", "LPB", "L", "chunks", "levels", "quad", "extra_count", "big_count"), (int(v) for v in o)))

    def prof_reset(self):
        self._chk(lib().sbn_prof_reset(self.h), "prof_reset")

    def prof_get(self):
        res = {}
        for i in range(lib().sbn_prof_count(self.h)):
            name = C.c_char_p(); ms = C.c_double(); cnt = C.c_uint64()
            lib().sbn_prof_get(self.h, i, C.byref(name), C.byref(ms), C.byref(cnt))
            res[name.value.decode()] = (ms.value, cnt.value)
        return res
```

spartan-bn254_amd/csrc/abi_derefs_key.inc:

```

struct sbn_derefs_key {
  size_t batch = 0, N = 0, cells = 0, srs_n = 0;
  const sbn_dense* dense = nullptr;
  const sbn_bases* srs = nullptr;
  sbn_bases* pts = nullptr;
  void* d_ids = nullptr;
  std::vector<uint32_t> ids;
};

static uint32_t derefs_key_seg(size_t cells, size_t bN, uint32_t maxcnt) {
  const size_t NB = 2 * cells, mean = bN / cells + 1;
  uint32_t SEG = 32; while (SEG < 2 * mean && SEG < ACC_SEG_MAX) SEG <<= 1;
  if (NB < 262144) { const size_t total = 2 * bN; uint32_t cap = 32; while ((size_t)cap * 262144 < total && cap < ACC_SEG_MAX) cap <<= 1; if (SEG > cap) SEG = cap; }
  while ((size_t)maxcnt / SEG / 64 > ACC_SEG_MAX && SEG < ACC_SEG_MAX) SEG <<= 1;
  return SEG;
}

static void derefs_key_release(sbn_ctx* c, sbn_derefs_key* k) {
  if (k->pts) sbn_bases_free(c, k->pts);
  if (k->d_ids) hipFree(k->d_ids);
  delete k;
}

static int derefs_key_commit_locked(sbn_ctx* c, const sbn_derefs_key* k, const sbn_table* mem_rx, const sbn_table* mem_ry, uint8_t out_xy[64], int* out_is_inf) {
  const size_t len = k->ids.size();
  int rc; if ((rc = ensure(c, c->scal_canon, len * 32))) return rc;
  LAUNCH(c, "k_dk_scalars", k_dk_scalars, stream_grid(len), 256, (const uint32_t*)mem_rx->d, (const uint32_t*)mem_ry->d, (const uint32_t*)k->d_ids, len, (uint32_t*)c->scal_canon.p);
  LAUNCHCHK(c);
  return msm_device(c, (const uint32_t*)c->scal_canon.p, (const uint32_t*)k->pts->d_pts, len, out_xy, out_is_inf, k->pts);
}

extern "C" {

int sbn_derefs_key_build(sbn_ctx* c, const sbn_dense* dn, const sbn_bases* srs, sbn_derefs_key** out) {
  if (!c || !dn || !srs || !out) return SBN_EINVAL;
  *out = nullptr;
  std::lock_guard<std::mutex> g(c->mu); hipSetDevice(c->device);
  const size_t b = dn->batch, N = dn->N, cells = dn->cells, bN = b * N, NB = 2 * cells;
  if (srs->has_h) return fail(c, SBN_EINVAL, "derefs key: the SRS handle has an h; an SRS is sbn_kzg_srs_upload's or sbn_kzg_srs_from_tau's");
  if (2 * bN >= ((size_t)1 << 31)) return fail(c, SBN_EINVAL, "derefs key: 2 * batch * N = %zu: an entry's index must leave bit 31 clear", 2 * bN);
  if (srs->n < 2 * bN) return fail(c, SBN_EINVAL, "derefs key: the SRS has %zu points, the derefs polynomial's non-zero prefix %zu coefficients", srs->n, 2 * bN);
  if (bN == 0 || cells == 0 || cells > ((size_t)1 << 30)) return fail(c, SBN_EINVAL, "derefs key: %zu cells, batch * N = %zu", cells, bN);
  int rc;
  std::vector<uint32_t> h(NB);
  HIPCHK(c, hipStreamSynchronize(c->stream));
  HIPCHK(c, hipMemcpy(h.data(), dense_audit(dn, 0), NB * 4, hipMemcpyDeviceToHost));
  uint32_t maxcnt = 0;
  std::unique_ptr<sbn_derefs_key> kp(new sbn_derefs_key());
  for (size_t t = 0; t < NB; t++) {
    if (h[t] > bN) return fail(c, SBN_EINVAL, "derefs key: audit_ts[%zu] = %u exceeds batch * N = %zu", t, h[t], bN);
    maxcnt = std::max(maxcnt, h[t]);
    if (h[t]) kp->ids.push_back((uint32_t)((t / cells) << 31) | (uint32_t)(t % cells));
  }
  for (int side = 0; side < 2; side++) {
    size_t sum = 0; for (size_t a = 0; a < cells; a++) sum += h[(size_t)side * cells + a];
    if (sum != bN) return fail(c, SBN_EINVAL, "derefs key: the %s side's audit_ts sum to %zu, not batch * N = %zu", side ? "column" : "row", sum, bN);
  }
  const size_t len = kp->ids.size();
  const uint32_t SEG = derefs_key_seg(cells, bN, maxcnt);
  const size_t max_extra = 2 * bN / SEG + 1, max_big = std::min(NB, max_extra);
  if ((rc = ensure(c, c->offs, NB * 4))) return rc;
  if ((rc = ensure(c, c->sorted, 2 * bN * 4))) return rc;
  if ((rc = ensure(c, c->buckets, NB * 128))) return rc;
  if ((rc = ensure(c, c->acc_ctr, 64 + (ACC_SEG_MAX + 2) * 4))) return rc;
  if ((rc = ensure(c, c->extra_list, max_extra * sizeof(ExtraItem)))) return rc;
  if ((rc = ensure(c, c->extra_out, max_extra * 128))) return rc;
  if ((rc = ensure(c, c->big_list, max_big * sizeof(BigItem)))) return rc;
  if ((rc = ensure(c, c->perm, NB * 4))) return rc;
  if ((rc = ensure(c, c->gen_tmp, len * 128))) return rc;
  const uint32_t* hist = dense_audit(dn, 0);
  uint32_t* offs = (uint32_t*)c->offs.p; uint32_t* sorted = (uint32_t*)c->sorted.p; uint32_t* buckets = (uint32_t*)c->buckets.p;
  AccCounters* ctr = (AccCounters*)c->acc_ctr.p;
  const uint32_t* points = (const uint32_t*)srs->d_pts;
  sbn_bases* pts = new sbn_bases(); pts->n = len; pts->has_h = false;
  kp->pts = pts;
  auto bail = [&](int code) { hipStreamSynchronize(c->stream); sbn_derefs_key* k = kp.release(); derefs_key_release(nullptr, k); return code; };
  if (hipMalloc(&pts->d_pts, len * 64) != hipSuccess || hipMalloc(&kp->d_ids, len * 4) != hipSuccess) { (void)hipGetLastError(); return bail(fail(c, SBN_ENOMEM, "derefs key: hipMalloc of %zu points", len)); }
  if (hipMemcpyAsync(kp->d_ids, kp->ids.data(), len * 4, hipMemcpyHostToDevice, c->stream) != hipSuccess) return bail(fail(c, SBN_EHIP, "derefs key: upload of the cell ids"));
  if (hipMemsetAsync(ctr, 0, 64 + (ACC_SEG_MAX + 2) * 4, c->stream) != hipSuccess) return bail(fail(c, SBN_EHIP, "derefs key: clearing the counters"));
  c->last_job[0] = 0; c->last_job[1] = 2; c->last_job[2] = (uint64_t)(2 * bN); c->last_job[3] = (uint64_t)NB;
  c->last_acc[0] = SEG; c->last_acc[1] = 1; c->last_acc[2] = 0; c->last_acc[3] = 0; c->last_acc[4] = 0; c->last_acc[5] = 0;
  LAUNCH(c, "k_scan", k_scan, 2, 1024, hist, offs, (int)cells);
  LAUNCH(c, "k_dk_place", k_dk_place, stream_grid(2 * bN), 256, (const uint32_t*)dn->u32s, bN, (uint32_t)cells, hist, (const uint32_t*)offs, sorted);
  uint32_t* size_bins = (uint32_t*)((uint8_t*)c->acc_ctr.p + 64);
  LAUNCH(c, "k_size_sort", k_size_hist, (unsigned)((NB + 1023) / 1024), 1024, hist, NB, SEG, size_bins);
  LAUNCH(c, "k_size_sort", k_size_scan, 1, 64, size_bins, SEG);
  LAUNCH(c, "k_size_sort", k_size_scatter, (unsigned)((NB + 1023) / 1024), 1024, hist, NB, SEG, size_bins, (uint32_t*)c->perm.p);
  LAUNCH(c, "k_acc_first", k_acc_first<1>, (unsigned)((NB + 255) / 256), 256, points, NB, (int)cells, bN, SEG, hist, (const uint32_t*)offs, (const uint32_t*)sorted,
         (const uint32_t*)c->perm.p, buckets, ctr, (ExtraItem*)c->extra_list.p, (BigItem*)c->big_list.p);
  LAUNCH(c, "k_acc_extra", k_acc_extra, 2048, 256, points, (int)cells, bN, SEG, hist, (const uint32_t*)offs, (const uint32_t*)sorted, (const AccCounters*)ctr,
         (const ExtraItem*)c->extra_list.p, (uint32_t*)c->extra_out.p);
  LAUNCH(c, "k_acc_merge", k_acc_merge, 4096, 64, (const AccCounters*)ctr, (const BigItem*)c->big_list.p, (const uint32_t*)c->extra_out.p, buckets, 1);
  LAUNCH(c, "k_dk_gather", k_dk_gather, stream_grid(len), 256, (const uint32_t*)buckets, (const uint32_t*)kp->d_ids, (uint32_t)cells, len, (uint32_t*)c->gen_tmp.p);
  LAUNCH(c, "k_xyzz_to_affine", k_xyzz_to_affine, (unsigned)((len + 63) / 64), 64, (const uint32_t*)c->gen_tmp.p, (uint32_t*)pts->d_pts, (uint32_t*)nullptr, (uint8_t*)nullptr, len);
  const hipError_t le = hipGetLastError(), se = hipStreamSynchronize(c->stream);
  if (c->prof) prof_drain(c);
  if (le != hipSuccess || se != hipSuccess) return bail(fail(c, SBN_EHIP, "derefs key build: %s", hipGetErrorString(le != hipSuccess ? le : se)));
  kp->batch = b; kp->N = N; kp->cells = cells; kp->srs_n = srs->n; kp->dense = dn; kp->srs = srs;
  *out = kp.release();
  return SBN_OK;
}

void sbn_derefs_key_free(sbn_ctx* c, sbn_derefs_key* k) {
  if (!k) return;
  std::unique_lock<std::mutex> g;
  if (c) { g = std::unique_lock<std::mutex>(c->mu); hipSetDevice(c->device); hipStreamSynchronize(c->stream); }
  derefs_key_release(c, k);
}

size_t sbn_derefs_key_len(const sbn_derefs_key* k) { return k ? k->ids.size() : 0; }

int sbn_derefs_key_download(sbn_ctx* c, const sbn_derefs_key* k, size_t first, size_t count, uint32_t* out_cell, uint8_t* out_xy) {
  if (!c || !k || (count && (!out_cell || !out_xy))) return SBN_EINVAL;
  if (first > k->ids.size() || count > k->ids.size() - first) return fail(c, SBN_EINVAL, "derefs key download: [%zu, %zu) of %zu cells", first, first + count, k->ids.size());
  if (!count) return SBN_OK;
  std::lock_guard<std::mutex> g(c->mu); hipSetDevice(c->device);
  int rc; if ((rc = ensure(c, c->out_small, count * 64))) return rc;
  LAUNCH(c, "k_points_from_mont", k_points_from_mont, (unsigned)((count + 255) / 256), 256, (const uint32_t*)k->pts->d_pts + 16 * first, (uint32_t*)c->out_small.p, count);
  LAUNCHCHK(c);
  HIPCHK(c, hipMemcpyAsync(out_xy, c->out_small.p, count * 64, hipMemcpyDeviceToHost, c->stream));
  HIPCHK(c, hipStreamSynchronize(c->stream));
  if (c->prof) prof_drain(c);
  memcpy(out_cell, k->ids.data() + first, count * 4);
  return SBN_OK;
}

int sbn_derefs_key_commit(sbn_ctx* c, const sbn_derefs_key* k, const sbn_table* mem_rx, const sbn_table* mem_ry, uint8_t out_xy[64], int* out_is_inf) {
  if (!c || !k || !mem_rx || !mem_ry || !out_xy) return SBN_EINVAL;
  if (mem_rx->len < k->cells || mem_ry->len < k->cells) return fail(c, SBN_EINVAL, "derefs key commit: the eq tables hold %zu and %zu entries, the memories %zu cells", mem_rx->len, mem_ry->len, k->cells);
  std::lock_guard<std::mutex> g(c->mu); hipSetDevice(c->device);
  return derefs_key_commit_locked(c, k, mem_rx, mem_ry, out_xy, out_is_inf);
}

}
```

spartan-bn254_amd/csrc/ctx.hpp:

```cpp
#pragma once
static const uint32_t SBN_SCALARS_INTERNAL = 0x10000u;
struct ProfEntry { std::string name; double ms = 0; uint64_t launches = 0; };
struct PendingEvt { int idx; hipEvent_t e0, e1; };

struct DevBuf {
  void* p = nullptr; size_t cap = 0;
};

struct ScKnobs {
  size_t comb_grid = 0;
  size_t comb_blocks = 512, seq_blocks = 512, comb_eval_blocks_mixed = 768, eval_blocks_mixed = 768, comb_eval_blocks = 1024, eval_blocks = 2048;
  size_t comb_min_q = (size_t)1 << 14, comb_lanes = 262144, single_max = (size_t)1 << 14, grid = 0, block_rounds = 4;
};
static ScKnobs sc_knobs_read() {
  ScKnobs k;
  auto num = [](const char* n, long long lo, size_t* out) { const char* e = getenv(n); if (!e) return false; const long long x = atoll(e); if (x < lo) return false; *out = (size_t)x; return true; };
  num("SBN_SC_COMB_GRID", 1, &k.comb_grid); num("SBN_SC_COMB_BLOCKS", 1, &k.comb_blocks); num("SBN_SC_SEQ_BLOCKS", 1, &k.seq_blocks);
  if (num("SBN_SC_COMB_EVAL_BLOCKS", 1, &k.comb_eval_blocks)) k.comb_eval_blocks_mixed = k.comb_eval_blocks;
  if (num("SBN_SC_EVAL_BLOCKS", 1, &k.eval_blocks)) k.eval_blocks_mixed = k.eval_blocks;
  num("SBN_SC_COMB_MIN_Q", 1, &k.comb_min_q); num("SBN_SC_COMB_LANES", 1, &k.comb_lanes); num("SBN_SC_SINGLE_MAX", 2, &k.single_max); num("SBN_SC_GRID", 1, &k.grid);
  { size_t v = 0; if (num("SBN_SC_BLOCK_ROUNDS", 1, &v) && v <= 16) k.block_rounds = v; }
  return k;
}

struct sbn_ctx {
  int device = 0;
  ScKnobs sck;
  hipStream_t own_stream = nullptr, stream = nullptr;
  std::mutex mu;
  std::string err;
  DevBuf scal_canon, hist, offs, sorted, buckets, red_a, red_b, wsum, stage_scal, stage_pts, out_small;
  DevBuf sc_args, sc_partial, sc_out, sc_r, sc_tabs, sc_tickets, sc_prove, gen_tmp, acc_ctr, extra_list, extra_out, big_list, digits, blockhist, perm, merged;
  hipStream_t copy_stream = nullptr;
  hipStream_t pp_stream = nullptr;
  hipEvent_t z_consumed = nullptr;
  DevBuf zstage[2], out_rows, comb_partial;
  DevBuf s2_cnt, s2_part, s2_idx, s2_lo;
  DevBuf glv_scal;
  DevBuf kzg_ws;
  DevBuf r1cs_ws;
  DevBuf dense_ws;
  int msm_glv = -1;
  bool sort2_ok = false;
  size_t sort2_min = (size_t)1 << 20;
  bool sort_rows_ok = false;
  int sort_rs_max = 16384;
  void* pin = nullptr; size_t pin_cap = 0;
  uint32_t* d_bad = nullptr;
  uint32_t* h_bad = nullptr;
  uint32_t* mbox = nullptr; uint32_t mbox_seq = 0;
  std::vector<std::pair<void*, size_t>> pool; size_t pool_bytes = 0;
  uint64_t last_job[4] = {0, 0, 0, 0};
  uint64_t last_acc[6] = {0, 0, 0, 0, 0, 0};
  double polyeval_us[3] = {0, 0, 0};
  bool prof = false;
  std::vector<ProfEntry> prof_entries;
  std::vector<PendingEvt> prof_pending;
  std::vector<hipEvent_t> evt_pool;
};

struct sbn_bases {
  size_t n = 0;
  bool has_h = false;
  void* d_pts = nullptr;
  mutable std::unordered_map<int, void*> tables;
  sbn_bases* uniq = nullptr;
  size_t U = 0; uint32_t nbig = 0; uint32_t hcol = 0;
  void* d_csr_off = nullptr; void* d_csr_cols = nullptr; void* d_big = nullptr;
  void* d_comb = nullptr; int comb_c = 0; size_t comb_bytes = 0;
  mutable std::vector<std::pair<std::string, sbn_bases*>> bullet_ext;
  mutable void* d_glv = nullptr;
  mutable std::string zk_key;
};
static const uint32_t MERGE_BIG = 64;
extern "C" void sbn_bases_free(sbn_ctx* c, sbn_bases* b);

struct sbn_table {
  void* d = nullptr; size_t len = 0; size_t cap = 0; bool owned = true;
  void* d2 = nullptr; size_t cap2 = 0; bool owned2 = true;
};

static const size_t POOL_MAX_ENTRIES = 1024;
static const size_t POOL_MAX_BYTES = (size_t)24 << 30;
static hipError_t pool_get(sbn_ctx* c, size_t bytes, void** out, size_t* got_bytes) {
  if (bytes == 0) bytes = 32;
  int best = -1;
  for (size_t i = 0; i < c->pool.size(); i++)
    if (c->pool[i].second >= bytes && c->pool[i].second <= 2 * bytes && (best < 0 || c->pool[i].second < c->pool[(size_t)best].second)) best = (int)i;
  if (best >= 0) { *out = c->pool[(size_t)best].first; *got_bytes = c->pool[(size_t)best].second; c->pool_bytes -= *got_bytes; c->pool.erase(c->pool.begin() + best); return hipSuccess; }
  hipError_t e = hipMalloc(out, bytes);
  if (e != hipSuccess && !c->pool.empty()) {
    (void)hipGetLastError();
    for (auto& b : c->pool) hipFree(b.first);
    c->pool.clear(); c->pool_bytes = 0;
    e = hipMalloc(out, bytes);
  }
  *got_bytes = bytes;
  return e;
}
static void pool_put(sbn_ctx* c, void* p, size_t bytes) {
  if (!p) return;
  if (!c || c->pool.size() >= POOL_MAX_ENTRIES || c->pool_bytes + bytes > POOL_MAX_BYTES) { hipFree(p); return; }
  c->pool.emplace_back(p, bytes); c->pool_bytes += bytes;
}

static int fail(sbn_ctx* c, int code, const char* fmt, ...) {
  char buf[512]; va_list ap; va_start(ap, fmt); vsnprintf(buf, sizeof buf, fmt, ap); va_end(ap);
  if (c) c->err = buf;
  return code;
}
#define HIPCHK(c, call) do { hipError_t _e = (call); if (_e != hipSuccess) return fail((c), SBN_EHIP, "%s failed: %s (%s:%d)", #call, hipGetErrorString(_e), __FILE__, __LINE__); } while (0)

static void table_release(sbn_ctx* c, sbn_table* t) {
  if (!t) return;
  if (t->d && t->owned) pool_put(c, t->d, t->cap * 32);
  if (t->d2 && t->owned2) pool_put(c, t->d2, t->cap2 * 32);
  delete t;
}
static int table_alloc(sbn_ctx* c, size_t len, const char* what, sbn_table** out) {
  sbn_table* t = new sbn_table(); t->len = len;
  size_t got = 0; const hipError_t e = pool_get(c, len * 32, &t->d, &got);
  if (e != hipSuccess) { delete t; *out = nullptr; return fail(c, SBN_ENOMEM, "hipMalloc %s: %s", what, hipGetErrorString(e)); }
  t->cap = got / 32;
  *out = t;
  return SBN_OK;
}
static sbn_table* table_view(const sbn_table* t, size_t first, size_t len) {
  sbn_table* v = new sbn_table();
  v->d = (uint8_t*)t->d + first * 32; v->len = v->cap = len; v->owned = false;
  return v;
}
struct TableScope {
  sbn_ctx* c; bool ok = false;
  std::vector<sbn_table*> held;
  explicit TableScope(sbn_ctx* c_) : c(c_) {}
  TableScope(const TableScope&) = delete;
  TableScope& operator=(const TableScope&) = delete;
  ~TableScope() {
    if (!ok) hipStreamSynchronize(c->stream);
    for (sbn_table* t : held) table_release(c, t);
  }
  sbn_table* keep(sbn_table* t) { if (t) held.push_back(t); return t; }
  int alloc(size_t len, const char* what, sbn_table** out) { const int rc = table_alloc(c, len, what, out); keep(*out); return rc; }
  const sbn_table* view(const sbn_table* t, size_t first, size_t len) { return keep(table_view(t, first, len)); }
  sbn_table* give(sbn_table* t) { held.erase(std::find(held.begin(), held.end(), t)); return t; }
  void give_all() { held.clear(); }
  int done() { ok = true; return SBN_OK; }
};

static int ensure(sbn_ctx* c, DevBuf& b, size_t bytes) {
  if (bytes <= b.cap) return SBN_OK;
  if (b.p) { HIPCHK(c, hipStreamSynchronize(c->stream)); HIPCHK(c, hipFree(b.p)); b.p = nullptr; b.cap = 0; }
  size_t want = bytes + (bytes >> 3);
  hipError_t e = hipMalloc(&b.p, want);
  if (e != hipSuccess) { b.p = nullptr; return fail(c, SBN_ENOMEM, "hipMalloc(%zu) failed: %s", want, hipGetErrorString(e)); }
  b.cap = want;
  return SBN_OK;
}
static int input_check_begin(sbn_ctx* c) { HIPCHK(c, hipMemsetAsync(c->d_bad, 0, 4, c->stream)); return SBN_OK; }
static int input_check_fetch(sbn_ctx* c) { HIPCHK(c, hipMemcpyAsync(c->h_bad, c->d_bad, 4, hipMemcpyDeviceToHost, c->stream)); return SBN_OK; }
static int input_check_end(sbn_ctx* c) {
  if (*c->h_bad) return fail(c, SBN_EINVAL, "%u input scalars are not canonical (>= r; Scalar::from_bytes rejects them, scalar.rs:87-95)", *c->h_bad);
  return SBN_OK;
}
static int ensure_pin(sbn_ctx* c, size_t bytes) {
  if (bytes <= c->pin_cap) return SBN_OK;
  if (c->pin) { HIPCHK(c, hipStreamSynchronize(c->stream)); HIPCHK(c, hipHostFree(c->pin)); c->pin = nullptr; c->pin_cap = 0; }
  HIPCHK(c, hipHostMalloc(&c->pin, bytes, hipHostMallocDefault));
  c->pin_cap = bytes;
  return SBN_OK;
}

static int prof_index(sbn_ctx* c, const char* name) {
  for (size_t i = 0; i < c->prof_entries.size(); i++) if (c->prof_entries[i].name == name) return (int)i;
  ProfEntry e; e.name = name; c->prof_entries.push_back(e); return (int)c->prof_entries.size() - 1;
}
static hipEvent_t evt_get(sbn_ctx* c) {
  if (!c->evt_pool.empty()) { hipEvent_t e = c->evt_pool.back(); c->evt_pool.pop_back(); return e; }
  hipEvent_t e; hipEventCreate(&e); return e;
}
static void prof_drain(sbn_ctx* c) {
  for (auto& p : c->prof_pending) {
    hipEventSynchronize(p.e1);
    float ms = 0; hipEventElapsedTime(&ms, p.e0, p.e1);
    c->prof_entries[p.idx].ms += ms; c->prof_entries[p.idx].launches += 1;
    c->evt_pool.push_back(p.e0); c->evt_pool.push_back(p.e1);
  }
  c->prof_pending.clear();
}
struct ProfScope {
  sbn_ctx* c; PendingEvt pe; bool on;
  ProfScope(sbn_ctx* c_, const char* name) : c(c_), on(c_->prof) {
    if (on) { pe.idx = prof_index(c, name); pe.e0 = evt_get(c); pe.e1 = evt_get(c); hipEventRecord(pe.e0, c->stream); }
  }
  ~ProfScope() { if (on) { hipEventRecord(pe.e1, c->stream); c->prof_pending.push_back(pe); } }
};
#define LAUNCH(c, name, kern, grid, block, ...) \
  do { ProfScope _ps((c), name); hipLaunchKernelGGL(kern, dim3(grid), dim3(block), 0, (c)->stream, __VA_ARGS__); } while (0)
#define LAUNCHCHK(c) HIPCHK(c, hipGetLastError())

static int sc_tickets(sbn_ctx* c) {
  if (c->mbox && c->sc_tickets.cap) return SBN_OK;
  if (!c->mbox) {
    uint32_t* mb = nullptr;
    HIPCHK(c, hipHostMalloc((void**)&mb, SC_MBOX_WORDS * 4, hipHostMallocMapped | hipHostMallocCoherent));
    memset(mb, 0, SC_MBOX_WORDS * 4);
    c->mbox = mb;
  }
  if (!c->sc_tickets.cap) {
    int rc; if ((rc = ensure(c, c->sc_tickets, 4096 * 4))) return rc;
    HIPCHK(c, hipMemsetAsync(c->sc_tickets.p, 0, 4096 * 4, c->stream));
  }
  return SBN_OK;
}
static int sc_mbox_wait(sbn_ctx* c, size_t count, uint32_t seq) {
  volatile uint32_t* fl = c->mbox + SC_MBOX_FLAGS;
  if (!c->prof) {
    for (int spin = 0; spin < 200000; spin++) {
      size_t done = 0; while (done < count && fl[done] == seq) done++;
      if (done == count) { std::atomic_thread_fence(std::memory_order_acquire); return SBN_OK; }
    }
  }
  HIPCHK(c, hipStreamSynchronize(c->stream));
  if (c->prof) prof_drain(c);
  for (size_t i = 0; i < count; i++) if (fl[i] != seq) return fail(c, SBN_EHIP, "sumcheck round: result flag %zu missing after synchronisation", i);
  return SBN_OK;
}
static int sc_flag_wait(sbn_ctx* c, volatile uint32_t* flag, uint32_t seq) {
  if (!c->prof) {
    for (int spin = 0; spin < 200000; spin++) if (*flag == seq) { std::atomic_thread_fence(std::memory_order_acquire); return SBN_OK; }
  }
  HIPCHK(c, hipStreamSynchronize(c->stream));
  if (c->prof) prof_drain(c);
  if (*flag != seq) return fail(c, SBN_EHIP, "result flag missing in the host mailbox after synchronisation");
  return SBN_OK;
}
```

spartan-bn254_amd/csrc/msm_host.hpp:

```cpp
#pragma once
static int ilog2_ceil(size_t n) { int l = 0; while (((size_t)1 << l) < n) l++; return l; }

static MsmShape make_shape(int c, int bits = 254) {
  MsmShape s; s.c = c; s.nb = 1 << (c - 1);
  int W = (bits + c - 1) / c;
  int tb = bits - (W - 1) * c;
  if (tb > c - 1) W += 1;
  s.W = W;
  return s;
}
static MsmShape choose_shape(size_t terms, bool shared_bucket_set, int cmax, size_t problems = 0, int chard = MSM_C_MAX) {
  const char* env = getenv("SBN_MSM_C");
  if (env && atoi(env) >= 7 && atoi(env) <= chard) return make_shape(atoi(env));
  if (cmax > chard) cmax = chard;
  if (problems && problems * terms <= 32768) {
    if (!shared_bucket_set && problems == 1 && terms >= 512 && terms <= 4096 && cmax >= 8) return make_shape(terms <= 512 ? 8 : 7);
    double bl = 1e300; int bcl = 7;
    for (int c = 7; c <= cmax; c++) {
      MsmShape s = make_shape(c);
      const int tb = 254 - (s.W - 1) * c;
      const double top = (double)terms / (double)(1u << (tb > 0 ? (tb < 20 ? tb : 20) : 0));
      const double load = (shared_bucket_set ? (double)terms * s.W / s.nb : (double)terms / s.nb) + top;
      if (load <= 6.0) return s;
      if (load < bl) { bl = load; bcl = c; }
    }
    return make_shape(bcl);
  }
  if (!shared_bucket_set && terms < ((size_t)1 << 20) && cmax >= 15) return make_shape(15);
  double best = 1e300; int bc = 7;
  for (int c = 7; c <= cmax; c++) {
    MsmShape s = make_shape(c);
    double sets = shared_bucket_set ? 1.0 : (double)s.W;
    const double per_bucket = (chard > MSM_C_MAX || (shared_bucket_set && problems >= 256)) ? 40.0 : 56.0;
    double cost = (double)terms * s.W * 10.0 + sets * s.nb * per_bucket;
    if (!shared_bucket_set && 254 - (s.W - 1) * c < c - 1) cost += (double)terms * 5.0;
    if (cost < best) { best = cost; bc = c; }
  }
  return make_shape(bc);
}

#define S2_FOR_EACH_C(X) X(13) X(14) X(15) X(16) X(17) X(18) X(19) X(20) X(21) X(22)
#define S2_GLV_FOR_EACH_C(X) X(13) X(14) X(15) X(16) X(17)
static bool sort2_set_lds() {
  bool ok = true;
  const int bytes = (int)s2_scatter_lds_bytes(S2_P_MAX);
  if (hipFuncSetAttribute((const void*)k_s2_place, hipFuncAttributeMaxDynamicSharedMemorySize, (int)s2_place_lds_bytes(S2_LO_LOG_MAX)) != hipSuccess) { (void)hipGetLastError(); ok = false; }
#define X(C) if (hipFuncSetAttribute((const void*)k_s2_scatter<C, S2_SPT>, hipFuncAttributeMaxDynamicSharedMemorySize, bytes) != hipSuccess) { (void)hipGetLastError(); ok = false; } \
             if (hipFuncSetAttribute((const void*)k_s2_scatter<C, S2_SPT_SMALL>, hipFuncAttributeMaxDynamicSharedMemorySize, bytes) != hipSuccess) { (void)hipGetLastError(); ok = false; }
  S2_FOR_EACH_C(X)
#undef X
  const int cnt_bytes = 24 * S2_P_MAX * 4;
#define X(C) if (hipFuncSetAttribute((const void*)k_s2_count<C, S2_SPT>, hipFuncAttributeMaxDynamicSharedMemorySize, cnt_bytes) != hipSuccess) { (void)hipGetLastError(); ok = false; } \
             if (hipFuncSetAttribute((const void*)k_s2_count<C, S2_SPT_SMALL>, hipFuncAttributeMaxDynamicSharedMemorySize, cnt_bytes) != hipSuccess) { (void)hipGetLastError(); ok = false; }
  S2_FOR_EACH_C(X)
#undef X
#define X(C) if (hipFuncSetAttribute((const void*)k_s2_count<C, S2_SPT, 4>, hipFuncAttributeMaxDynamicSharedMemorySize, cnt_bytes) != hipSuccess) { (void)hipGetLastError(); ok = false; } \
             if (hipFuncSetAttribute((const void*)k_s2_count<C, S2_SPT_SMALL, 4>, hipFuncAttributeMaxDynamicSharedMemorySize, cnt_bytes) != hipSuccess) { (void)hipGetLastError(); ok = false; } \
             if (hipFuncSetAttribute((const void*)k_s2_scatter<C, S2_SPT, 4>, hipFuncAttributeMaxDynamicSharedMemorySize, bytes) != hipSuccess) { (void)hipGetLastError(); ok = false; } \
             if (hipFuncSetAttribute((const void*)k_s2_scatter<C, S2_SPT_SMALL, 4>, hipFuncAttributeMaxDynamicSharedMemorySize, bytes) != hipSuccess) { (void)hipGetLastError(); ok = false; }
  S2_GLV_FOR_EACH_C(X)
#undef X
  return ok;
}
static bool sort2_applies(const sbn_ctx* c, int mode, size_t n, int cbits) {
  return mode == MODE_SINGLE && c->sort2_ok && c->sort2_min && n >= c->sort2_min && cbits >= S2_C_MIN && cbits <= S2_C_MAX;
}
static int sort2_run(sbn_ctx* c, const uint32_t* scalars, size_t n, const MsmShape& s, size_t estride, uint32_t* hist, uint32_t* offs, uint32_t* sorted, bool glv = false, size_t glv_gap = 0) {
  S2Geom g; g.n = n; g.c = s.c; g.W = s.W; g.half = n / 2; g.gap = glv ? glv_gap : 0;
  if (glv && (s.c < 13 || s.c > 17)) return fail(c, SBN_EINVAL, "two-level sort: no GLV instantiation for windows of %d bits", s.c);
  g.lo_log = std::max(s.c - 1 - 8, 8); if (g.lo_log > S2_LO_LOG_MAX) g.lo_log = S2_LO_LOG_MAX;
  if (const char* e = getenv("SBN_SORT2_LO")) { int v = atoi(e); if (v >= 4 && v <= S2_LO_LOG_MAX) g.lo_log = v; }
  if (s.c - 1 - g.lo_log < 0) g.lo_log = s.c - 1;
  while ((s.nb >> g.lo_log) > S2_P_MAX) g.lo_log++;
  if (g.lo_log > S2_LO_LOG_MAX) return fail(c, SBN_EINVAL, "two-level sort: window of %d bits is too wide", s.c);
  g.P = s.nb >> g.lo_log;
  const int LO = 1 << g.lo_log;
  int spt = (n <= ((size_t)1 << 21) && g.P <= 64) ? S2_SPT_SMALL : S2_SPT;
  if (const char* e = getenv("SBN_SORT2_SPT")) { const int v = atoi(e); if (v == S2_SPT || v == S2_SPT_SMALL) spt = v; }
  const size_t ch = (size_t)1024 * spt;
  g.K = (int)((n + ch - 1) / ch);
  const size_t WP = (size_t)g.W * g.P;
  const size_t max_sc = ((size_t)g.W * n) / S2_SUB + WP;
  int rc;
  if ((rc = ensure(c, c->s2_cnt, WP * g.K * 4))) return rc;
  if ((rc = ensure(c, c->s2_part, (3 * WP + 1) * 4))) return rc;
  if ((rc = ensure(c, c->s2_idx, (size_t)g.W * n * 4))) return rc;
  if ((rc = ensure(c, c->s2_lo, (size_t)g.W * n * 2))) return rc;
  if ((rc = ensure(c, c->blockhist, max_sc * LO * 4))) return rc;
  uint32_t* cntA = (uint32_t*)c->s2_cnt.p; uint32_t* part_cnt = (uint32_t*)c->s2_part.p; uint32_t* part_off = part_cnt + WP; uint32_t* sc_off = part_off + WP;
  uint32_t* tmp_idx = (uint32_t*)c->s2_idx.p; uint16_t* tmp_lo = (uint16_t*)c->s2_lo.p; uint32_t* bh = (uint32_t*)c->blockhist.p;
  const size_t lds_a = WP * 4, lds_c = s2_scatter_lds_bytes(g.P, spt);
  if (lds_a > (size_t)24 * S2_P_MAX * 4) return fail(c, SBN_EINVAL, "two-level sort: %zu level-1 counters do not fit the LDS granted to k_s2_count", WP);
  {
    ProfScope _ps(c, "k_s2_count");
    if (glv) switch (s.c) {
#define X(C) case C: if (spt == S2_SPT) hipLaunchKernelGGL((k_s2_count<C, S2_SPT, 4>), dim3(g.K), dim3(1024), lds_a, c->stream, scalars, g, cntA, c->d_bad); \
                     else hipLaunchKernelGGL((k_s2_count<C, S2_SPT_SMALL, 4>), dim3(g.K), dim3(1024), lds_a, c->stream, scalars, g, cntA, c->d_bad); break;
      S2_GLV_FOR_EACH_C(X)
#undef X
    } else switch (s.c) {
#define X(C) case C: if (spt == S2_SPT) hipLaunchKernelGGL((k_s2_count<C, S2_SPT>), dim3(g.K), dim3(1024), lds_a, c->stream, scalars, g, cntA, c->d_bad); \
                     else hipLaunchKernelGGL((k_s2_count<C, S2_SPT_SMALL>), dim3(g.K), dim3(1024), lds_a, c->stream, scalars, g, cntA, c->d_bad); break;
      S2_FOR_EACH_C(X)
#undef X
    }
  }
  LAUNCH(c, "k_s2_prefix", k_s2_prefix_k, (unsigned)WP, 256, cntA, g.K, part_cnt);
  LAUNCH(c, "k_s2_prefix", k_s2_prefix_hi, 1, 1024, (const uint32_t*)part_cnt, g.W, g.P, part_off, sc_off);
  {
    ProfScope _ps(c, "k_s2_scatter");
    if (glv) switch (s.c) {
#define X(C) case C: if (spt == S2_SPT) hipLaunchKernelGGL((k_s2_scatter<C, S2_SPT, 4>), dim3(g.K), dim3(1024), lds_c, c->stream, scalars, g, (const uint32_t*)cntA, (const uint32_t*)part_off, tmp_idx, tmp_lo); \
                     else hipLaunchKernelGGL((k_s2_scatter<C, S2_SPT_SMALL, 4>), dim3(g.K), dim3(1024), lds_c, c->stream, scalars, g, (const uint32_t*)cntA, (const uint32_t*)part_off, tmp_idx, tmp_lo); break;
      S2_GLV_FOR_EACH_C(X)
#undef X
    } else switch (s.c) {
#define X(C) case C: if (spt == S2_SPT) hipLaunchKernelGGL((k_s2_scatter<C, S2_SPT>), dim3(g.K), dim3(1024), lds_c, c->stream, scalars, g, (const uint32_t*)cntA, (const uint32_t*)part_off, tmp_idx, tmp_lo); \
                     else hipLaunchKernelGGL((k_s2_scatter<C, S2_SPT_SMALL>), dim3(g.K), dim3(1024), lds_c, c->stream, scalars, g, (const uint32_t*)cntA, (const uint32_t*)part_off, tmp_idx, tmp_lo); break;
      S2_FOR_EACH_C(X)
#undef X
    }
  }
  const unsigned l2 = s2_level2_blocks(max_sc);
  LAUNCH(c, "k_s2_hist", k_s2_hist, l2, 1024, (const uint16_t*)tmp_lo, g, (const uint32_t*)part_off, (const uint32_t*)part_cnt, (const uint32_t*)sc_off, bh);
  LAUNCH(c, "k_s2_prefix", k_s2_prefix2, (unsigned)WP, 1024, bh, g, (const uint32_t*)part_off, (const uint32_t*)sc_off, hist, offs);
  {
    ProfScope _ps(c, "k_s2_place");
    hipLaunchKernelGGL(k_s2_place, dim3(l2), dim3(1024), s2_place_lds_bytes(g.lo_log), c->stream,
                       (const uint16_t*)tmp_lo, (const uint32_t*)tmp_idx, g, (const uint32_t*)part_off, (const uint32_t*)part_cnt, (const uint32_t*)sc_off, (const uint32_t*)bh, (const uint32_t*)offs, sorted, estride);
  }
  LAUNCHCHK(c);
  return SBN_OK;
}

struct BucketJob {
  int mode; DigitArgs da; MsmShape s;
  size_t P;
  size_t threads;
  const uint32_t* points;
  const uint8_t* skip;
  bool glv;
  size_t glv_gap;
};

static int run_bucket_job(sbn_ctx* c, const BucketJob& J) {
  const MsmShape& s = J.s;
  const size_t NB = J.P * (size_t)s.nb;
  if (NB > 0xffffffffull) return fail(c, SBN_EINVAL, "bucket space too large");
  const size_t estride = J.da.estride;
  c->last_job[0] = (uint64_t)s.c; c->last_job[1] = (uint64_t)s.W; c->last_job[2] = (uint64_t)(J.P * estride); c->last_job[3] = (uint64_t)NB;
  size_t mean = estride / (size_t)s.nb + 1;
  uint32_t SEG = 32; while (SEG < 2 * mean && SEG < ACC_SEG_MAX) SEG <<= 1;
  if (NB < 262144) { const size_t total = J.P * estride; uint32_t cap = 32; while ((size_t)cap * 262144 < total && cap < ACC_SEG_MAX) cap <<= 1; if (SEG > cap) SEG = cap; }
  if (J.mode == MODE_SINGLE && J.da.n >= 512 && J.da.n <= 4096) SEG = 8;
  if (const char* es = getenv("SBN_MSM_SEG")) { int v = atoi(es); if (v >= 8 && v <= (int)ACC_SEG_MAX) SEG = (uint32_t)v; }
  int LPB = 1; if (J.mode == MODE_SINGLE && mean >= 48 && NB <= ((size_t)1 << 19)) LPB = 2;
  const size_t max_extra = J.P * estride / SEG + 1;
  const size_t max_big = std::min(NB, max_extra);
  int rc;
  if ((rc = ensure(c, c->hist, NB * 4))) return rc;
  if ((rc = ensure(c, c->offs, NB * 4))) return rc;
  if ((rc = ensure(c, c->sorted, J.P * estride * 4))) return rc;
  if ((rc = ensure(c, c->buckets, NB * 128 * (size_t)LPB))) return rc;
  if ((rc = ensure(c, c->acc_ctr, 64 + (ACC_SEG_MAX + 2) * 4))) return rc;
  if ((rc = ensure(c, c->extra_list, max_extra * sizeof(ExtraItem)))) return rc;
  if ((rc = ensure(c, c->extra_out, max_extra * 128))) return rc;
  if ((rc = ensure(c, c->big_list, max_big * sizeof(BigItem)))) return rc;
  int L = 1; while ((size_t)L * 64 * 2048 < NB && L < 16) L <<= 1;
  if (L < 4) L = 4;
  if (L > s.nb / 64) L = s.nb / 64;
  if (L < 1) L = 1;
  if (NB <= (size_t)64 * 16 * 1024) {
    double best = 1e300; int bl = L;
    for (int t = 1; t <= 32 && t * 64 <= std::max(s.nb, 64); t++) {
      const size_t waves = J.P * (size_t)((s.nb + 64 * t - 1) / (64 * t));
      const double cost = (double)((waves + 1023) / 1024) * (double)((2 * t - 1) + t * (LPB - 1) + 10);
      if (cost < best) { best = cost; bl = t; }
    }
    L = bl;
  }
  if (const char* el = getenv("SBN_RED_L")) { int v = atoi(el); if (v >= 1 && v <= 64) L = v; }
  const int chunks = (s.nb + 64 * L - 1) / (64 * L);
  if ((rc = ensure(c, c->red_a, J.P * chunks * 256))) return rc;
  if ((rc = ensure(c, c->red_b, J.P * ((chunks + 63) / 64) * 256))) return rc;
  if ((rc = ensure(c, c->wsum, J.P * 128))) return rc;

  uint32_t* hist = (uint32_t*)c->hist.p; uint32_t* offs = (uint32_t*)c->offs.p;
  uint32_t* sorted = (uint32_t*)c->sorted.p; uint32_t* buckets = (uint32_t*)c->buckets.p;
  AccCounters* ctr = (AccCounters*)c->acc_ctr.p;

  static_assert(sizeof(AccCounters) <= 64, "the size bins follow the counters at byte 64");
  HIPCHK(c, hipMemsetAsync(ctr, 0, 64 + (ACC_SEG_MAX + 2) * 4, c->stream));
  SortGeom g; memset(&g, 0, sizeof g);
  g.E = estride; g.estride = estride; g.nb = s.nb; g.mode = J.mode; g.ncol = J.da.n; g.tstride = J.da.tstride;
  g.RS = std::min(s.nb, c->sort_rs_max); g.logRS = 0; while ((1 << g.logRS) < g.RS) g.logRS++;
  g.R = s.nb / g.RS;
  { size_t want = (1024 + J.P * g.R - 1) / (J.P * g.R); size_t maxk = std::max<size_t>(1, estride / 4096); g.K = (int)std::max<size_t>(1, std::min(want, maxk)); }
  g.chunk = (estride + g.K - 1) / g.K;
  const uint8_t* skip = nullptr;
  const bool two_level = sort2_applies(c, J.mode, J.da.n, s.c) && !J.skip;
  if (s.c > MSM_C_MAX && !two_level) return fail(c, SBN_EINVAL, "window of %d bits needs the two-level sort", s.c);
  if (J.glv && !two_level) return fail(c, SBN_EINVAL, "GLV half-scalars need the two-level sort");
  if (two_level) {
    if ((rc = sort2_run(c, J.da.scalars, J.da.n, s, estride, hist, offs, sorted, J.glv, J.glv_gap))) return rc;
  } else {
  if (J.P > 65535 || g.R > 65535) return fail(c, SBN_EINVAL, "sort grid too large (P=%zu R=%d)", J.P, g.R);
  if ((rc = ensure(c, c->digits, J.P * estride * sizeof(dig_t)))) return rc;
  if ((rc = ensure(c, c->blockhist, J.P * (size_t)g.R * g.K * g.RS * 4))) return rc;
  dig_t* dig = (dig_t*)c->digits.p; uint32_t* bh = (uint32_t*)c->blockhist.p;
  const unsigned gd = (unsigned)((J.threads + 255) / 256);
  const size_t rows_lds = sort_rows_lds_bytes(s.nb);
  const bool fused_rows = J.mode == MODE_ROWS && c->sort_rows_ok && rows_lds <= 160 * 1024 && estride <= 8 * (size_t)SORT_SL;
  skip = fused_rows ? J.skip : nullptr;
  if (J.mode == MODE_SINGLE) LAUNCH(c, "k_digits_store", (k_digits_store<MODE_SINGLE>), gd, 256, J.da, s, dig, (const uint8_t*)nullptr);
  else LAUNCH(c, "k_digits_store", (k_digits_store<MODE_ROWS>), gd, 256, J.da, s, dig, skip);
  if (c->z_consumed && J.mode == MODE_ROWS) HIPCHK(c, hipEventRecord(c->z_consumed, c->stream));
  if (fused_rows) {
    ProfScope _ps(c, "k_sort_rows");
    hipLaunchKernelGGL(k_sort_rows, dim3((unsigned)J.P), dim3(1024), rows_lds, c->stream, (const dig_t*)dig, g, hist, offs, sorted, skip);
  } else {
    {
      ProfScope _ps(c, "k_hist_lds");
      hipLaunchKernelGGL(k_hist_lds, dim3(g.K, g.R, (unsigned)J.P), dim3(1024), (size_t)g.RS * 4, c->stream, (const dig_t*)dig, g, bh);
    }
    LAUNCH(c, "k_block_prefix", k_block_prefix, (unsigned)((NB + 255) / 256), 256, bh, g, NB, hist);
    LAUNCH(c, "k_scan", k_scan, (unsigned)J.P, 1024, hist, offs, s.nb);
    {
      ProfScope _ps(c, "k_scatter_lds");
      hipLaunchKernelGGL(k_scatter_lds, dim3(g.K, g.R, (unsigned)J.P), dim3(1024), (size_t)g.RS * 4, c->stream, (const dig_t*)dig, g, (const uint32_t*)bh, (const uint32_t*)offs, sorted);
    }
  }
  }
  if ((rc = ensure(c, c->perm, NB * 4))) return rc;
  uint32_t* size_bins = (uint32_t*)((uint8_t*)c->acc_ctr.p + 64);
  LAUNCH(c, "k_size_sort", k_size_hist, (unsigned)((NB + 1023) / 1024), 1024, hist, NB, SEG, size_bins);
  LAUNCH(c, "k_size_sort", k_size_scan, 1, 64, size_bins, SEG);
  LAUNCH(c, "k_size_sort", k_size_scatter, (unsigned)((NB + 1023) / 1024), 1024, hist, NB, SEG, size_bins, (uint32_t*)c->perm.p);
  const unsigned agrid = (unsigned)((NB * (size_t)LPB + 255) / 256);
#define ACC_FIRST_ARGS J.points, NB, s.nb, estride, SEG, hist, offs, sorted, (const uint32_t*)c->perm.p, buckets, ctr, (ExtraItem*)c->extra_list.p, (BigItem*)c->big_list.p
  if (LPB == 1) LAUNCH(c, "k_acc_first", k_acc_first<1>, agrid, 256, ACC_FIRST_ARGS);
  else LAUNCH(c, "k_acc_first", k_acc_first<2>, agrid, 256, ACC_FIRST_ARGS);
#undef ACC_FIRST_ARGS
  LAUNCH(c, "k_acc_extra", k_acc_extra, 2048, 256, J.points, s.nb, estride, SEG, hist, offs, sorted, ctr, (const ExtraItem*)c->extra_list.p, (uint32_t*)c->extra_out.p);
  LAUNCH(c, "k_acc_merge", k_acc_merge, 4096, 64, ctr, (const BigItem*)c->big_list.p, (const uint32_t*)c->extra_out.p, buckets, LPB);
  const bool red_quad = J.P * (size_t)chunks <= 2048;
  LAUNCH(c, "k_reduce_l1", k_reduce_l1, (unsigned)(J.P * chunks), 64, buckets, L, s.nb, (uint32_t*)c->red_a.p, skip, chunks, LPB);
  uint32_t* in = (uint32_t*)c->red_a.p; uint32_t* outb = (uint32_t*)c->red_b.p;
  int G = chunks, k64 = 1;
  c->last_acc[0] = SEG; c->last_acc[1] = (uint64_t)LPB; c->last_acc[2] = (uint64_t)L; c->last_acc[3] = (uint64_t)chunks; c->last_acc[4] = 0; c->last_acc[5] = red_quad ? 1 : 0;
  for (;;) {
    c->last_acc[4] += 1;
    int Gout = (G + 63) / 64;
    int final = (Gout == 1);
    if (red_quad) LAUNCH(c, "k_reduce_combine", k_reduce_combine_quad, (unsigned)(J.P * Gout), 256, in, G, Gout, k64, L, final, final ? (uint32_t*)c->wsum.p : outb);
    else LAUNCH(c, "k_reduce_combine", k_reduce_combine, (unsigned)(J.P * Gout), 64, in, G, Gout, k64, L, final, final ? (uint32_t*)c->wsum.p : outb);
    if (final) break;
    std::swap(in, outb); G = Gout; k64 += 1;
  }
  LAUNCHCHK(c);
  return SBN_OK;
}

static std::mutex g_bases_tables_mu;

static double single_msm_cost(size_t terms, const MsmShape& s, int bits) {
  double cost = (double)terms * s.W * 10.0 + (double)s.W * s.nb * 40.0;
  if (bits - (s.W - 1) * s.c < s.c - 1) cost += (double)terms * 5.0;
  return cost;
}
static MsmShape glv_shape(size_t n) {
  if (const char* env = getenv("SBN_MSM_C")) { const int v = atoi(env); if (v >= 13 && v <= 17) return make_shape(v, 127); }
  MsmShape best = make_shape(16, 127);
  for (int cc = 13; cc <= 17; cc++) { const MsmShape s = make_shape(cc, 127); if (single_msm_cost(2 * n, s, 127) < single_msm_cost(2 * n, best, 127)) best = s; }
  return best;
}
static bool glv_applies(const sbn_ctx* c, const sbn_bases* b, size_t n, const MsmShape& plain) {
  if (!b || c->msm_glv == 0 || (c->msm_glv < 0 && getenv("SBN_MSM_C"))) return false;
  const size_t npts = b->n + (b->has_h ? 1 : 0);
  if (2 * npts > 0x7fffffffull || !sort2_applies(c, MODE_SINGLE, 2 * n, S2_C_MIN)) return false;
  if (c->msm_glv == 1) return true;
  return single_msm_cost(2 * n, glv_shape(n), 127) * 1.04 < single_msm_cost(n, plain, 254);
}
static int bases_glv_table(sbn_ctx* c, const sbn_bases* b, const uint32_t** out) {
  std::lock_guard<std::mutex> tg(g_bases_tables_mu);
  if (b->d_glv) { *out = (const uint32_t*)b->d_glv; return SBN_OK; }
  const size_t npts = b->n + (b->has_h ? 1 : 0);
  void* tab = nullptr;
  hipError_t e = hipMalloc(&tab, 2 * npts * 64);
  if (e != hipSuccess) { (void)hipGetLastError(); return fail(c, SBN_ENOMEM, "hipMalloc GLV table (%zu B): %s", 2 * npts * 64, hipGetErrorString(e)); }
  LAUNCH(c, "k_glv_table", k_glv_table, (unsigned)((npts + 255) / 256), 256, (const uint32_t*)b->d_pts, npts, (uint32_t*)tab);
  hipError_t le = hipGetLastError();
  hipError_t se = hipStreamSynchronize(c->stream);
  if (le != hipSuccess || se != hipSuccess) { hipFree(tab); return fail(c, SBN_EHIP, "GLV table build: %s", hipGetErrorString(le != hipSuccess ? le : se)); }
  b->d_glv = tab;
  *out = (const uint32_t*)tab;
  return SBN_OK;
}

static int msm_device(sbn_ctx* c, const uint32_t* d_scal, const uint32_t* d_bases, size_t n, uint8_t out_xy[64], int* out_is_inf, const sbn_bases* b = nullptr) {
  if (n == 0) { memset(out_xy, 0, 64); if (out_is_inf) *out_is_inf = 1; return SBN_OK; }
  if (n > 0x7fffffffull) return fail(c, SBN_EINVAL, "msm: n=%zu exceeds 2^31-1", n);
  BucketJob J; memset(&J, 0, sizeof J);
  J.mode = MODE_SINGLE;
  {
    int cm = 1; while ((1 << cm) < c->sort_rs_max) cm++;
    const bool s2 = sort2_applies(c, MODE_SINGLE, n, S2_C_MIN);
    J.s = choose_shape(n, false, s2 ? S2_C_MAX : cm + 1, 1, s2 ? S2_C_MAX : MSM_C_MAX);
  }
  J.P = (size_t)J.s.W; J.threads = n; J.points = d_bases;
  J.da.scalars = d_scal; J.da.n = n; J.da.estride = n; J.da.bad = c->d_bad;
  const bool glv = glv_applies(c, b, n, J.s);
  int rc;
  if (glv) {
    const uint32_t* tab;
    if ((rc = bases_glv_table(c, b, &tab))) return rc;
    if ((rc = ensure(c, c->glv_scal, 2 * n * 16))) return rc;
    J.s = glv_shape(n); J.P = (size_t)J.s.W; J.threads = 2 * n; J.points = tab;
    J.da.scalars = (const uint32_t*)c->glv_scal.p; J.da.n = 2 * n; J.da.estride = 2 * n;
    J.glv = true; J.glv_gap = b->n + (b->has_h ? 1 : 0) - n;
  }
  if ((rc = ensure_pin(c, std::max<size_t>(4096, J.P * 128)))) return rc;
  if ((rc = input_check_begin(c))) return rc;
  if (glv) LAUNCH(c, "k_glv_split", k_glv_split, (unsigned)((n + 255) / 256), 256, d_scal, n, (uint32_t*)c->glv_scal.p, c->d_bad);
  if ((rc = run_bucket_job(c, J))) return rc;
  HIPCHK(c, hipMemcpyAsync(c->pin, c->wsum.p, J.P * 128, hipMemcpyDeviceToHost, c->stream));
  if ((rc = input_check_fetch(c))) return rc;
  HIPCHK(c, hipStreamSynchronize(c->stream));
  if (c->prof) prof_drain(c);
  if ((rc = input_check_end(c))) return rc;
  std::vector<sbn_host::Pt> S((size_t)J.s.W);
  for (int w = 0; w < J.s.W; w++) S[(size_t)w] = sbn_host::pt_from_device(((const sbn_host::Pt*)c->pin)[w]);
  sbn_host::Pt total = sbn_host::combine_windows(S.data(), J.s.W, J.s.c);
  sbn_host::to_affine_bytes(total, out_xy, out_is_inf);
  return SBN_OK;
}

static int bases_window_table(sbn_ctx* c, const sbn_bases* b, const MsmShape& s, const uint32_t** out) {
  std::lock_guard<std::mutex> tg(g_bases_tables_mu);
  auto it = b->tables.find(s.c);
  if (it != b->tables.end()) { *out = (const uint32_t*)it->second; return SBN_OK; }
  const size_t npts = b->n + (b->has_h ? 1 : 0);
  const size_t tot = npts * (size_t)s.W;
  int rc;
  if ((rc = ensure(c, c->gen_tmp, tot * 128))) return rc;
  void* tab = nullptr;
  hipError_t e = hipMalloc(&tab, tot * 64);
  if (e != hipSuccess) return fail(c, SBN_ENOMEM, "hipMalloc window table (%zu B): %s", tot * 64, hipGetErrorString(e));
  LAUNCH(c, "k_window_table", k_window_table, (unsigned)((npts + 63) / 64), 64, (const uint32_t*)b->d_pts, npts, s.c, s.W, (uint32_t*)c->gen_tmp.p);
  LAUNCH(c, "k_xyzz_to_affine", k_xyzz_to_affine, (unsigned)((tot + 63) / 64), 64, (const uint32_t*)c->gen_tmp.p, (uint32_t*)tab, (uint32_t*)nullptr, (uint8_t*)nullptr, tot);
  LAUNCHCHK(c);
  HIPCHK(c, hipStreamSynchronize(c->stream));
  b->tables[s.c] = tab;
  *out = (const uint32_t*)tab;
  return SBN_OK;
}

static int bases_build_comb(sbn_ctx* c, sbn_bases* b, size_t max_bytes) {
  const size_t npts = b->n + (b->has_h ? 1 : 0);
  if (npts == 0) return fail(c, SBN_EINVAL, "precompute: empty generator set");
  int cc = 0; size_t bytes = 0;
  for (int t = COMB_C_MAX; t >= 7; t--) {
    const MsmShape s = make_shape(t);
    const size_t need = npts * (size_t)s.W * (size_t)s.nb * 64;
    if (need <= max_bytes) { cc = t; bytes = need; break; }
  }
  if (!cc) return fail(c, SBN_EINVAL, "precompute: even the c = 7 table (%zu B) exceeds the budget of %zu B", npts * (size_t)make_shape(7).W * 64 * 64, max_bytes);
  {
    std::lock_guard<std::mutex> tg(g_bases_tables_mu);
    if (b->d_comb && b->comb_c == cc) return SBN_OK;
  }
  const MsmShape s = make_shape(cc);
  int rc; const uint32_t* wtab;
  if ((rc = bases_window_table(c, b, s, &wtab))) return rc;
  std::lock_guard<std::mutex> tg(g_bases_tables_mu);
  if (b->d_comb) { HIPCHK(c, hipStreamSynchronize(c->stream)); hipFree(b->d_comb); b->d_comb = nullptr; b->comb_c = 0; }
  void* tab = nullptr;
  hipError_t e = hipMalloc(&tab, bytes);
  if (e != hipSuccess) { (void)hipGetLastError(); return fail(c, SBN_ENOMEM, "hipMalloc lookup table (%zu B): %s", bytes, hipGetErrorString(e)); }
  const size_t slab_lanes = npts * ((size_t)s.nb / COMB_CH);
  const size_t BL = std::min<size_t>(slab_lanes, (size_t)1 << 18);
  void* tx = nullptr; void* tp = nullptr;
  if ((e = hipMalloc(&tx, BL * COMB_CH * 128)) != hipSuccess || (e = hipMalloc(&tp, BL * COMB_CH * 32)) != hipSuccess) {
    (void)hipGetLastError(); hipFree(tab); if (tx) hipFree(tx);
    return fail(c, SBN_ENOMEM, "hipMalloc lookup-table build scratch: %s", hipGetErrorString(e));
  }
  for (int w = 0; w < s.W; w++)
    for (size_t l0 = 0; l0 < slab_lanes; l0 += BL) {
      const size_t lanes = std::min(BL, slab_lanes - l0);
      LAUNCH(c, "k_comb_build", k_comb_build, (unsigned)((lanes + 63) / 64), 64, wtab + 16 * ((size_t)w * npts), npts, cc, l0, lanes, (uint32_t*)tx, (uint32_t*)tp,
             (uint32_t*)tab + 16 * (((size_t)w * npts) << (cc - 1)));
    }
  hipError_t le = hipGetLastError();
  hipError_t se = hipStreamSynchronize(c->stream);
  hipFree(tx); hipFree(tp);
  if (le != hipSuccess || se != hipSuccess) { hipFree(tab); return fail(c, SBN_EHIP, "lookup-table build: %s", hipGetErrorString(le != hipSuccess ? le : se)); }
  if (c->prof) prof_drain(c);
  b->d_comb = tab; b->comb_c = cc; b->comb_bytes = bytes;
  return SBN_OK;
}

struct RowInfo {
  const uint8_t* flags = nullptr;
  bool skip_zero = false;
  size_t col_value = ~(size_t)0, col_blind = ~(size_t)0;
  bool internal_rows = false;
  bool mont_scalars = false;
};
static int commit_rows_launch(sbn_ctx* c, const sbn_bases* b, const uint32_t* dZ, const uint32_t* dBl, size_t L, size_t R, uint32_t* d_xy, uint8_t* d_inf, const RowInfo& ri = RowInfo()) {
  if (L == 0) return SBN_OK;
  const uint8_t* skip_rows = ri.skip_zero ? ri.flags : nullptr;
  if (b->uniq) {
    const size_t U = b->U; int rc;
    if ((rc = ensure(c, c->merged, L * (U + 1) * 32 + L))) return rc;
    uint32_t* m = (uint32_t*)c->merged.p; uint8_t* rowflags = (uint8_t*)c->merged.p + L * (U + 1) * 32;
    if (ri.internal_rows) rowflags = nullptr;
    else if (R) LAUNCH(c, "k_merge_scalars", k_row_const_flags, (unsigned)L, 256, dZ, dBl, R, rowflags, ri.mont_scalars ? (uint32_t*)nullptr : c->d_bad);
    else HIPCHK(c, hipMemsetAsync(rowflags, 0, L, c->stream));
    {
      const size_t nsmall = (L * (U + 1) + 255) / 256, nbigb = L * (size_t)b->nbig;
      if (nsmall + nbigb > 0x7fffffffull) return fail(c, SBN_EINVAL, "commit: merge grid too large");
      LAUNCH(c, "k_merge_scalars", k_merge, (unsigned)(nsmall + nbigb), 256, dZ, dBl, L, R, U, (const uint32_t*)b->d_csr_off, (const uint32_t*)b->d_csr_cols, MERGE_BIG,
             (const uint32_t*)b->d_big, b->nbig, (const uint8_t*)rowflags, b->hcol, m, ri.mont_scalars ? 1 : 0, (uint32_t)nsmall);
    }
    if (c->z_consumed) HIPCHK(c, hipEventRecord(c->z_consumed, c->stream));
    RowInfo info; info.flags = rowflags; info.skip_zero = dBl == nullptr;
    info.col_value = U; info.col_blind = (dBl && b->hcol <= U) ? (size_t)b->hcol : ~(size_t)0;
    return commit_rows_launch(c, b->uniq, m, nullptr, L, U + 1, d_xy, d_inf, info);
  }
  if (ri.mont_scalars) return fail(c, SBN_EINVAL, "commit: internal: Montgomery scalars without merged bases");
  const size_t ncol = R + (dBl ? 1 : 0);
  if (ncol == 0) {
    if (!d_xy) { int rc0; if ((rc0 = ensure(c, c->wsum, L * 128))) return rc0; HIPCHK(c, hipMemsetAsync(c->wsum.p, 0, L * 128, c->stream)); return SBN_OK; }
    HIPCHK(c, hipMemsetAsync(d_xy, 0, 64 * L, c->stream)); HIPCHK(c, hipMemsetAsync(d_inf, 1, L, c->stream)); return SBN_OK;
  }
  const size_t npts = b->n + (b->has_h ? 1 : 0);
  if (b->d_comb) {
    const MsmShape s = make_shape(b->comb_c);
    DigitArgs da; memset(&da, 0, sizeof da);
    da.scalars = dZ; da.blinds = dBl; da.n = ncol; da.R = R; da.L = L; da.tstride = npts; da.bad = c->d_bad;
    unsigned S = 1;
    if ((size_t)L * 64 < 2048 && ncol * (size_t)s.W > 1024) {
      S = (unsigned)std::min<size_t>(128, (ncol * (size_t)s.W + 511) / 512);
      while (S > 1 && (size_t)L * S > 4096) S--;
    }
    if (const char* es = getenv("SBN_COMB_S")) { int v = atoi(es); if (v >= 1 && v <= 128) S = (unsigned)v; }
    int rc;
    if ((rc = ensure(c, c->wsum, L * 128))) return rc;
    if ((rc = ensure(c, c->comb_partial, S > 1 ? L * S * 128 : L * 257 * 128))) return rc;
    if (L > 0x7fffffffull || ncol * (size_t)s.W > 0x7fffffffull) return fail(c, SBN_EINVAL, "commit: too many rows / columns");
    c->last_job[0] = (uint64_t)s.c; c->last_job[1] = (uint64_t)s.W; c->last_job[2] = (uint64_t)(L * ncol * (size_t)s.W); c->last_job[3] = 0;
    if (S > 1) {
      LAUNCH(c, "k_comb_rows", k_comb_rows_flat, dim3((unsigned)L, S), 256, (const uint32_t*)b->d_comb, da, s, skip_rows, (uint32_t*)c->comb_partial.p);
      LAUNCH(c, "k_comb_fold", k_comb_fold, (unsigned)L, S > 64 ? 128 : 64, (const uint32_t*)c->comb_partial.p, S, (uint32_t*)c->wsum.p, (const uint8_t*)nullptr, (const uint32_t*)nullptr);
    } else {
      const uint8_t* fl = (ri.flags && ri.col_value != ~(size_t)0) ? ri.flags : nullptr;
      uint32_t* sparse = (uint32_t*)c->comb_partial.p + (size_t)32 * L * 256;
      LAUNCH(c, "k_comb_rows", k_comb_rows, dim3((unsigned)L, 1), 256, (const uint32_t*)b->d_comb, da, s, fl, (uint32_t*)c->comb_partial.p);
      if (fl) LAUNCH(c, "k_comb_rows_const", k_comb_rows_const, (unsigned)L, 64, (const uint32_t*)b->d_comb, da, s, fl, ri.skip_zero ? 1 : 0, ri.col_value, ri.col_blind, sparse);
      LAUNCH(c, "k_comb_fold", k_comb_fold, (unsigned)L, 64, (const uint32_t*)c->comb_partial.p, 256u, (uint32_t*)c->wsum.p, fl, (const uint32_t*)sparse);
    }
    if (c->z_consumed) HIPCHK(c, hipEventRecord(c->z_consumed, c->stream));
    if (d_xy) LAUNCH(c, "k_xyzz_to_affine", k_xyzz_to_affine, (unsigned)((L + 63) / 64), 64, (const uint32_t*)c->wsum.p, (uint32_t*)nullptr, d_xy, d_inf, L);
    LAUNCHCHK(c);
    return SBN_OK;
  }
  BucketJob J; memset(&J, 0, sizeof J);
  J.mode = MODE_ROWS; J.s = choose_shape(ncol, true, 16, L); J.P = L; J.threads = L * ncol;
  if ((size_t)J.s.W * npts > 0x7fffffffull) return fail(c, SBN_EINVAL, "commit: table index overflow");
  int rc; const uint32_t* tab;
  if ((rc = bases_window_table(c, b, J.s, &tab))) return rc;
  J.points = tab;
  J.da.scalars = dZ; J.da.blinds = dBl; J.da.n = ncol; J.da.R = R; J.da.L = L; J.da.tstride = npts; J.da.estride = ncol * (size_t)J.s.W; J.da.bad = c->d_bad;
  J.skip = skip_rows;
  if ((rc = run_bucket_job(c, J))) return rc;
  if (d_xy) LAUNCH(c, "k_xyzz_to_affine", k_xyzz_to_affine, (unsigned)((L + 63) / 64), 64, (const uint32_t*)c->wsum.p, (uint32_t*)nullptr, d_xy, d_inf, L);
  LAUNCHCHK(c);
  return SBN_OK;
}
static int commit_rows_device(sbn_ctx* c, const sbn_bases* b, const uint32_t* dZ, const uint32_t* dBl, size_t L, size_t R, uint8_t* out_xy, uint8_t* out_inf, const RowInfo& ri = RowInfo()) {
  if (L == 0) return SBN_OK;
  int rc;
  if ((rc = input_check_begin(c))) return rc;
  if (L <= 16) {
    if ((rc = sc_tickets(c))) return rc;
    if ((rc = commit_rows_launch(c, b, dZ, dBl, L, R, nullptr, nullptr, ri))) return rc;
    const uint32_t seq = ++c->mbox_seq;
    uint32_t* hfin = c->mbox + SC_MBOX_FINALS;
    static_assert(16 * 32 + 1 <= SC_MBOX_WORDS - SC_MBOX_FINALS, "mailbox: 16 XYZZ sums + the counter must fit the final-claims area");
    LAUNCH(c, "k_points_to_host", k_sc_finals_raw, 1, 256, (const uint32_t*)c->wsum.p, (uint32_t)(L * 32), (const uint32_t*)c->d_bad, hfin, c->mbox + SC_MBOX_FLAGS + SC_PACK_MAX, seq);
    LAUNCHCHK(c);
    if ((rc = sc_flag_wait(c, c->mbox + SC_MBOX_FLAGS + SC_PACK_MAX, seq))) return rc;
    *c->h_bad = hfin[L * 32];
    if ((rc = input_check_end(c))) return rc;
    sbn_host::Pt S[16]; memcpy(S, hfin, L * 128);
    for (size_t i = 0; i < L; i++) { int inf = 0; sbn_host::to_affine_bytes(sbn_host::pt_from_device(S[i]), out_xy + 64 * i, &inf); if (out_inf) out_inf[i] = (uint8_t)inf; }
    return SBN_OK;
  }
  if ((rc = ensure(c, c->out_small, L * 65))) return rc;
  if ((rc = ensure_pin(c, std::max<size_t>(4096, L * 65)))) return rc;
  if ((rc = commit_rows_launch(c, b, dZ, dBl, L, R, (uint32_t*)c->out_small.p, (uint8_t*)c->out_small.p + L * 64, ri))) return rc;
  HIPCHK(c, hipMemcpyAsync(c->pin, c->out_small.p, L * 65, hipMemcpyDeviceToHost, c->stream));
  if ((rc = input_check_fetch(c))) return rc;
  HIPCHK(c, hipStreamSynchronize(c->stream));
  if (c->prof) prof_drain(c);
  if ((rc = input_check_end(c))) return rc;
  memcpy(out_xy, c->pin, L * 64);
  if (out_inf) memcpy(out_inf, (uint8_t*)c->pin + L * 64, L);
  return SBN_OK;
}

static int stage_scalars(sbn_ctx* c, const uint8_t* host_scalars, size_t n, uint32_t flags, const uint32_t** d_out) {
  int rc;
  if ((rc = ensure(c, c->stage_scal, n * 32))) return rc;
  HIPCHK(c, hipMemcpyAsync(c->stage_scal.p, host_scalars, n * 32, hipMemcpyHostToDevice, c->stream));
  if (flags & SBN_SCALARS_MONT) {
    if ((rc = ensure(c, c->scal_canon, n * 32))) return rc;
    LAUNCH(c, "k_scalars_from_mont", k_scalars_from_mont, (unsigned)((n + 255) / 256), 256, (const uint32_t*)c->stage_scal.p, (uint32_t*)c->scal_canon.p, n);
    *d_out = (const uint32_t*)c->scal_canon.p;
  } else *d_out = (const uint32_t*)c->stage_scal.p;
  return SBN_OK;
}
static int canon_scalars_dev(sbn_ctx* c, const void* d_scalars, size_t n, uint32_t flags, const uint32_t** d_out) {
  if (flags & SBN_SCALARS_MONT) {
    int rc; if ((rc = ensure(c, c->scal_canon, n * 32))) return rc;
    LAUNCH(c, "k_scalars_from_mont", k_scalars_from_mont, (unsigned)((n + 255) / 256), 256, (const uint32_t*)d_scalars, (uint32_t*)c->scal_canon.p, n);
    *d_out = (const uint32_t*)c->scal_canon.p;
  } else *d_out = (const uint32_t*)d_scalars;
  return SBN_OK;
}

static int bases_build_dedupe(sbn_ctx* c, sbn_bases* b, const std::vector<std::string>& keys) {
  const size_t tot = keys.size();
  std::unordered_map<std::string, uint32_t> idx;
  std::vector<uint32_t> umap(tot);
  std::vector<uint32_t> first_col;
  for (size_t j = 0; j < tot; j++) {
    auto it = idx.find(keys[j]);
    if (it == idx.end()) { uint32_t u = (uint32_t)first_col.size(); idx.emplace(keys[j], u); first_col.push_back((uint32_t)j); umap[j] = u; }
    else umap[j] = it->second;
  }
  const size_t U = first_col.size();
  if (U * 10 > tot * 9) return SBN_OK;
  std::vector<uint32_t> off(U + 1, 0), cols(tot), big;
  for (size_t j = 0; j < tot; j++) off[umap[j] + 1]++;
  for (size_t u = 0; u < U; u++) off[u + 1] += off[u];
  { std::vector<uint32_t> cur(off.begin(), off.end() - 1); for (size_t j = 0; j < tot; j++) cols[cur[umap[j]]++] = (uint32_t)j; }
  for (size_t u = 0; u < U; u++) if (off[u + 1] - off[u] > MERGE_BIG) big.push_back((uint32_t)u);
  sbn_bases* q = new sbn_bases(); q->n = U + 1; q->has_h = false;
  hipError_t e = hipMalloc(&q->d_pts, (U + 1) * 64);
  if (e != hipSuccess) { delete q; return fail(c, SBN_ENOMEM, "hipMalloc unique bases: %s", hipGetErrorString(e)); }
  for (size_t u = 0; u < U; u++)
    HIPCHK(c, hipMemcpyAsync((uint8_t*)q->d_pts + 64 * u, (const uint8_t*)b->d_pts + 64 * (size_t)first_col[u], 64, hipMemcpyDeviceToDevice, c->stream));
  auto up = [&](void** dst, const std::vector<uint32_t>& v) -> int {
    hipError_t e2 = hipMalloc(dst, std::max<size_t>(4, v.size() * 4)); if (e2 != hipSuccess) return SBN_ENOMEM;
    if (!v.empty() && hipMemcpy(*dst, v.data(), v.size() * 4, hipMemcpyHostToDevice) != hipSuccess) return SBN_EHIP;
    return SBN_OK;
  };
  HIPCHK(c, hipStreamSynchronize(c->stream));
  int rc;
  if ((rc = up(&b->d_csr_off, off)) || (rc = up(&b->d_csr_cols, cols)) || (rc = up(&b->d_big, big))) { sbn_bases_free(c, q); return fail(c, rc, "dedupe tables"); }
  b->uniq = q; b->U = U; b->nbig = (uint32_t)big.size();
  b->hcol = (b->has_h) ? umap[tot - 1] : (uint32_t)(U + 1);
  {
    const size_t n = b->n;
    std::vector<uint8_t> mult(U * 32, 0);
    for (size_t j = 0; j < n; j++) { uint32_t* m = (uint32_t*)&mult[32 * umap[j]]; m[0] += 1; }
    int rc2;
    if ((rc2 = ensure(c, c->stage_scal, U * 32))) return rc2;
    HIPCHK(c, hipMemcpyAsync(c->stage_scal.p, mult.data(), U * 32, hipMemcpyHostToDevice, c->stream));
    uint8_t sxy[64]; int sinf = 0;
    if ((rc2 = msm_device(c, (const uint32_t*)c->stage_scal.p, (const uint32_t*)q->d_pts, U, sxy, &sinf))) return rc2;
    uint8_t sm[64]; memset(sm, 0, 64);
    if (!sinf) memcpy(sm, sxy, 64);
    HIPCHK(c, hipMemcpy((uint8_t*)q->d_pts + 64 * U, sm, 64, hipMemcpyHostToDevice));
    LAUNCH(c, "k_points_to_mont", k_points_to_mont, 1, 256, (const uint32_t*)q->d_pts + 16 * U, (uint32_t*)q->d_pts + 16 * U, (size_t)1);
    LAUNCHCHK(c);
    HIPCHK(c, hipStreamSynchronize(c->stream));
  }
  return SBN_OK;
}
```

spartan-bn254_amd/csrc/sbn254.hip:

```cpp
#include "../../include/sbn254.h"
#include "host_field.hpp"
#include "msm_kernels.cuh"
#include "sort2_kernels.cuh"
#include "glv_kernels.cuh"
#include "comb_kernels.cuh"
#include "sumcheck_kernels.cuh"
#include "sumcheck_comb_kernels.cuh"
#include "kzg_kernels.cuh"
#include "r1cs_kernels.cuh"
#include "dense_kernels.cuh"
#include "transcript_kernels.cuh"
#include "polyeval_kernels.cuh"
#include "zk_sumcheck_kernels.cuh"
#include "r1cs_proof_kernels.cuh"
#include "sparse_eval_kernels.cuh"
#include "derefs_key_kernels.cuh"
#include "host_keccak.hpp"
#include "host_strobe.hpp"

#include <hip/hip_runtime.h>
#include <algorithm>
#include <atomic>
#include <chrono>
#include <cstdarg>
#include <cstdio>
#include <cstdlib>
#include <condition_variable>
#include <cstring>
#include <functional>
#include <memory>
#include <mutex>
#include <string>
#include <thread>
#include <unordered_map>
#include <vector>

using namespace sbn;

#include "ctx.hpp"
#include "msm_host.hpp"

#include "abi_msm.inc"
#include "abi_tables.inc"
#include "abi_transcript.inc"
#include "abi_sumcheck.inc"
#include "abi_product_proof.inc"
#include "abi_bullet.inc"
#include "abi_polyeval.inc"
#include "abi_zk_sumcheck.inc"
#include "abi_group.inc"
#include "abi_kzg.inc"
#include "abi_r1cs.inc"
#include "abi_r1cs_proof.inc"
#include "abi_dense.inc"
#include "abi_derefs_key.inc"
#include "abi_sparse_eval.inc"

extern "C" {

int sbn_prof_enable(sbn_ctx* c, int on) { if (!c) return SBN_EINVAL; std::lock_guard<std::mutex> g(c->mu); c->prof = on != 0; return SBN_OK; }
int sbn_prof_reset(sbn_ctx* c) { if (!c) return SBN_EINVAL; std::lock_guard<std::mutex> g(c->mu); hipStreamSynchronize(c->stream); prof_drain(c); c->prof_entries.clear(); return SBN_OK; }
int sbn_prof_count(sbn_ctx* c) { if (!c) return 0; std::lock_guard<std::mutex> g(c->mu); hipStreamSynchronize(c->stream); prof_drain(c); return (int)c->prof_entries.size(); }
int sbn_prof_get(sbn_ctx* c, int i, const char** name, double* total_ms, uint64_t* launches) {
  if (!c || i < 0 || (size_t)i >= c->prof_entries.size()) return SBN_EINVAL;
  if (name) *name = c->prof_entries[i].name.c_str();
  if (total_ms) *total_ms = c->prof_entries[i].ms;
  if (launches) *launches = c->prof_entries[i].launches;
  return SBN_OK;
}
int sbn_prof_last_job(sbn_ctx* c, uint64_t out[4]) {
  if (!c || !out) return SBN_EINVAL;
  std::lock_guard<std::mutex> g(c->mu);
  for (int i = 0; i < 4; i++) out[i] = c->last_job[i];
  return SBN_OK;
}
int sbn_prof_last_acc(sbn_ctx* c, uint64_t out[8]) {
  if (!c || !out) return SBN_EINVAL;
  std::lock_guard<std::mutex> g(c->mu);
  for (int i = 0; i < 6; i++) out[i] = c->last_acc[i];
  out[6] = out[7] = 0;
  if (!c->acc_ctr.p) return SBN_OK;
  AccCounters h;
  HIPCHK(c, hipStreamSynchronize(c->stream));
  HIPCHK(c, hipMemcpy(&h, c->acc_ctr.p, sizeof h, hipMemcpyDeviceToHost));
  out[6] = h.extra_count; out[7] = h.big_count;
  return SBN_OK;
}

}
```

spartan-bn254_amd/csrc/sort2_kernels.cuh:

```cuda
#pragma once
#include "msm_kernels.cuh"
#include <utility>

namespace sbn {

constexpr int S2_LO_LOG_MAX = 11, S2_LO_MAX = 1 << S2_LO_LOG_MAX;
constexpr int S2_P_MAX = 1024;
constexpr int S2_SPT = 8, S2_CH = 1024 * S2_SPT;
constexpr int S2_SPT_SMALL = 2;
constexpr int S2_C_MIN = 13, S2_C_MAX = 22;
struct S2Geom {
  size_t n;
  int c, W, P;
  int lo_log;
  int K;
  size_t half, gap;
};

template <int C, int SW = 8> struct S2Shape {
  static constexpr int BITS = SW == 8 ? 254 : 127;
  static constexpr int W0 = (BITS + C - 1) / C;
  static constexpr int W = W0 + ((BITS - (W0 - 1) * C) > C - 1 ? 1 : 0);
};
typedef uint32_t s2_u32x8 __attribute__((ext_vector_type(8)));
template <int C, int w> __device__ __forceinline__ int s2_digit(const s2_u32x8 k, uint32_t& carry) {
  constexpr int bit = w * C, limb = bit >> 5, sh = bit & 31;
  uint64_t x = 0;
  if constexpr (limb < 8) x = k[limb];
  if constexpr (limb + 1 < 8) x |= (uint64_t)k[limb + 1] << 32;
  const uint32_t raw = (uint32_t)(x >> sh) & ((1u << C) - 1u);
  const uint32_t v = raw + carry;
  if (v >= (1u << (C - 1))) { carry = 1; return (int)v - (1 << C); }
  carry = 0;
  return (int)v;
}
template <int SW = 8> __device__ __forceinline__ s2_u32x8 s2_load_scalar(const uint32_t* __restrict__ scalars, size_t t) {
  const uint4* p = reinterpret_cast<const uint4*>(scalars + (size_t)SW * t);
  const uint4 a = p[0], b = SW == 8 ? p[1] : make_uint4(0u, 0u, 0u, 0u);
  s2_u32x8 k; k[0] = a.x; k[1] = a.y; k[2] = a.z; k[3] = a.w; k[4] = b.x; k[5] = b.y; k[6] = b.z; k[7] = b.w;
  return k;
}
__device__ __forceinline__ bool s2_is_canonical(const s2_u32x8 k) { uint32_t kk[8]; for (int i = 0; i < 8; i++) kk[i] = k[i]; return fe_is_canonical<FrP>(kk); }

extern __shared__ uint32_t s2_lds[];

template <int C, int... Ws>
__device__ __forceinline__ void s2_count_scalar(const s2_u32x8 kk, int P, int lo_log, std::integer_sequence<int, Ws...>) {
  uint32_t carry = 0;
  auto one = [&](auto wc) {
    constexpr int w = decltype(wc)::value;
    const int d = s2_digit<C, w>(kk, carry);
    if (d != 0) atomicAdd(&s2_lds[w * P + (((d < 0 ? -d : d) - 1) >> lo_log)], 1u);
  };
  (one(std::integral_constant<int, Ws>{}), ...);
}
template <int C, int SPT, int SW = 8>
__global__ void __launch_bounds__(1024) k_s2_count(const uint32_t* __restrict__ scalars, S2Geom g, uint32_t* __restrict__ cntA, uint32_t* __restrict__ bad) {
  constexpr int W = S2Shape<C, SW>::W; constexpr int CH = 1024 * SPT;
  const int k = blockIdx.x, P = g.P;
  for (int j = threadIdx.x; j < W * P; j += 1024) s2_lds[j] = 0;
  __syncthreads();
  for (int i = 0; i < SPT; i++) {
    const size_t t = (size_t)k * CH + (size_t)i * 1024 + threadIdx.x;
    if (t >= g.n) break;
    const s2_u32x8 kk = s2_load_scalar<SW>(scalars, t);
    if (SW == 8 && !s2_is_canonical(kk)) atomicAdd(bad, 1u);
    s2_count_scalar<C>(kk, P, g.lo_log, std::make_integer_sequence<int, W>{});
  }
  __syncthreads();
  for (int j = threadIdx.x; j < W * P; j += 1024) cntA[(size_t)j * g.K + k] = s2_lds[j];
}

__device__ __forceinline__ uint32_t s2_block_scan(uint32_t v, uint32_t* tmp , uint32_t* total) {
  const int lane = threadIdx.x & 63, wv = threadIdx.x >> 6, nw = (blockDim.x + 63) >> 6;
  uint32_t inc = v;
#pragma unroll
  for (int d = 1; d < 64; d <<= 1) { const uint32_t o = __shfl_up(inc, d); if (lane >= d) inc += o; }
  if (lane == 63) tmp[wv] = inc;
  __syncthreads();
  if (threadIdx.x == 0) { uint32_t run = 0; for (int i = 0; i < nw; i++) { const uint32_t x = tmp[i]; tmp[i] = run; run += x; } tmp[16] = run; }
  __syncthreads();
  const uint32_t r = inc - v + tmp[wv];
  *total = tmp[16];
  __syncthreads();
  return r;
}
__global__ void __launch_bounds__(256) k_s2_prefix_k(uint32_t* __restrict__ cntA, int K, uint32_t* __restrict__ part_cnt) {
  __shared__ uint32_t tmp[17];
  uint32_t* row = cntA + (size_t)blockIdx.x * K;
  const int per = (K + 255) / 256, b0 = threadIdx.x * per;
  uint32_t sum = 0;
  for (int i = 0; i < per; i++) if (b0 + i < K) sum += row[b0 + i];
  uint32_t total; uint32_t run = s2_block_scan(sum, tmp, &total);
  for (int i = 0; i < per; i++) if (b0 + i < K) { const uint32_t v = row[b0 + i]; row[b0 + i] = run; run += v; }
  if (threadIdx.x == 0) part_cnt[blockIdx.x] = total;
}
constexpr uint32_t S2_SUB = 16384;
__global__ void __launch_bounds__(1024) k_s2_prefix_hi(const uint32_t* __restrict__ part_cnt, int W, int P, uint32_t* __restrict__ part_off, uint32_t* __restrict__ sc_off) {
  __shared__ uint32_t tmp[17];
  __shared__ uint32_t wstart[32];
  const int n = W * P, per = (n + 1023) / 1024, i0 = (int)threadIdx.x * per, i1 = (i0 + per < n) ? i0 + per : n;
  uint32_t sv = 0, sk = 0;
  for (int i = i0; i < i1; i++) { const uint32_t v = part_cnt[i]; sv += v; sk += (v + S2_SUB - 1) / S2_SUB; }
  uint32_t tv, tk;
  uint32_t rv = s2_block_scan(sv, tmp, &tv), rk = s2_block_scan(sk, tmp, &tk);
  for (int i = i0; i < i1; i++) { const uint32_t v = part_cnt[i]; part_off[i] = rv; sc_off[i] = rk; rv += v; rk += (v + S2_SUB - 1) / S2_SUB; }
  if (threadIdx.x == 0) sc_off[(size_t)n] = tk;
  __syncthreads();
  if ((int)threadIdx.x < W) wstart[threadIdx.x] = part_off[(size_t)threadIdx.x * P];
  __syncthreads();
  for (int i = i0; i < i1; i++) part_off[i] -= wstart[i / P];
}

__host__ __device__ inline size_t s2_scatter_lds_bytes(int P, int spt = S2_SPT) { return ((size_t)3 * P + 32) * 4 + (size_t)1024 * spt * 8; }
struct S2ScatterArgs {
  const uint32_t* cntA; const uint32_t* part_off; uint32_t* tmp_idx; uint16_t* tmp_lo;
  size_t n, half, gap; int P, K, k, lo_log;
};
template <int C, int w, int SPT>
__device__ __forceinline__ void s2_scatter_window(const s2_u32x8 (&kk)[SPT], uint32_t (&carry)[SPT], const S2ScatterArgs& a) {
  constexpr int CH = 1024 * SPT;
  const int P = a.P, tid = threadIdx.x;
  uint32_t* cnt = s2_lds; uint32_t* base = cnt + P; uint32_t* gdelta = base + P; uint32_t* tmp = gdelta + P;
  uint32_t* stage_idx = tmp + 32;
  uint16_t* stage_lo = reinterpret_cast<uint16_t*>(stage_idx + CH); uint16_t* stage_hi = stage_lo + CH;
  for (int j = tid; j < P; j += 1024) cnt[j] = 0;
  __syncthreads();
  int d[SPT]; uint32_t rank[SPT];
#pragma unroll
  for (int i = 0; i < SPT; i++) {
    const int dd = s2_digit<C, w>(kk[i], carry[i]);
    d[i] = dd; rank[i] = 0;
    if (dd != 0) rank[i] = atomicAdd(&cnt[((dd < 0 ? -dd : dd) - 1) >> a.lo_log], 1u);
  }
  __syncthreads();
  uint32_t total;
  {
    const uint32_t v = tid < P ? cnt[tid] : 0;
    const uint32_t r = s2_block_scan(v, tmp, &total);
    if (tid < P) { base[tid] = r; gdelta[tid] = a.part_off[(size_t)w * P + tid] + a.cntA[((size_t)w * P + tid) * a.K + a.k] - r; }
  }
  __syncthreads();
  const size_t t0 = (size_t)a.k * CH + tid;
#pragma unroll
  for (int i = 0; i < SPT; i++) {
    if (d[i] == 0) continue;
    const uint32_t b = (uint32_t)((d[i] < 0 ? -d[i] : d[i]) - 1), hi = b >> a.lo_log;
    const uint32_t pos = base[hi] + rank[i];
    size_t e = t0 + (size_t)i * 1024;
    if (a.gap && e >= a.half) e += a.gap;
    stage_idx[pos] = (uint32_t)e | (d[i] < 0 ? 0x80000000u : 0u);
    stage_lo[pos] = (uint16_t)(b & ((1u << a.lo_log) - 1u)); stage_hi[pos] = (uint16_t)hi;
  }
  __syncthreads();
  uint32_t* oi = a.tmp_idx + (size_t)w * a.n; uint16_t* ol = a.tmp_lo + (size_t)w * a.n;
  for (uint32_t j = tid; j < total; j += 1024) {
    const uint32_t pos = j + gdelta[stage_hi[j]];
    oi[pos] = stage_idx[j]; ol[pos] = stage_lo[j];
  }
  __syncthreads();
}
template <int C, int SPT, int... Ws>
__device__ __forceinline__ void s2_scatter_windows(const s2_u32x8 (&kk)[SPT], uint32_t (&carry)[SPT], const S2ScatterArgs& a, std::integer_sequence<int, Ws...>) {
  (s2_scatter_window<C, Ws, SPT>(kk, carry, a), ...);
}
template <int C, int SPT, int SW = 8>
__global__ void __launch_bounds__(1024) k_s2_scatter(const uint32_t* __restrict__ scalars, S2Geom g, const uint32_t* __restrict__ cntA ,
                                                     const uint32_t* __restrict__ part_off, uint32_t* __restrict__ tmp_idx, uint16_t* __restrict__ tmp_lo) {
  S2ScatterArgs a; a.cntA = cntA; a.part_off = part_off; a.tmp_idx = tmp_idx; a.tmp_lo = tmp_lo; a.n = g.n; a.P = g.P; a.K = g.K; a.k = blockIdx.x; a.lo_log = g.lo_log;
  a.half = g.half; a.gap = SW == 8 ? 0 : g.gap;
  s2_u32x8 kk[SPT]; uint32_t carry[SPT];
#pragma unroll
  for (int i = 0; i < SPT; i++) {
    const size_t t = (size_t)blockIdx.x * (1024 * SPT) + (size_t)i * 1024 + threadIdx.x;
    carry[i] = 0;
    kk[i] = t < g.n ? s2_load_scalar<SW>(scalars, t) : (s2_u32x8)(0u);
  }
  s2_scatter_windows<C, SPT>(kk, carry, a, std::make_integer_sequence<int, S2Shape<C, SW>::W>{});
}

__device__ __forceinline__ bool s2_decode(const S2Geom& g, const uint32_t* __restrict__ sc_off, int& q, uint32_t& sidx, uint32_t& k2) {
  const uint32_t Lid = blockIdx.x, xcd = Lid & 7u, slot = Lid >> 3;
  sidx = (slot >> 4) * 128u + xcd * 16u + (slot & 15u);
  const int WP = g.W * g.P;
  if (sidx >= sc_off[WP]) return false;
  int lo = 0, hi = WP;
  while (hi - lo > 1) { const int mid = (lo + hi) >> 1; if (sc_off[mid] <= sidx) lo = mid; else hi = mid; }
  q = lo; k2 = sidx - sc_off[q];
  return true;
}
__host__ __device__ inline uint32_t s2_level2_blocks(size_t max_subchunks) { return (uint32_t)(((max_subchunks + 127) / 128) * 128); }
__device__ __forceinline__ void s2_range(const S2Geom& g, const uint32_t* __restrict__ part_off, const uint32_t* __restrict__ part_cnt, int q, uint32_t k2, size_t& e0, size_t& e1) {
  const uint32_t start = part_off[q], cn = part_cnt[q];
  uint32_t a = k2 * S2_SUB, b = a + S2_SUB; if (a > cn) a = cn; if (b > cn) b = cn;
  const size_t w = (size_t)(q / g.P);
  e0 = w * g.n + start + a; e1 = w * g.n + start + b;
}
__global__ void __launch_bounds__(1024) k_s2_hist(const uint16_t* __restrict__ tmp_lo, S2Geom g, const uint32_t* __restrict__ part_off, const uint32_t* __restrict__ part_cnt, const uint32_t* __restrict__ sc_off, uint32_t* __restrict__ blockhist) {
  __shared__ uint32_t h[S2_LO_MAX];
  int q; uint32_t sidx, k2; if (!s2_decode(g, sc_off, q, sidx, k2)) return;
  const int LO = 1 << g.lo_log;
  for (int j = threadIdx.x; j < LO; j += 1024) h[j] = 0;
  __syncthreads();
  size_t e0, e1; s2_range(g, part_off, part_cnt, q, k2, e0, e1);
  for (size_t e = e0 + threadIdx.x; e < e1; e += 1024) atomicAdd(&h[tmp_lo[e]], 1u);
  __syncthreads();
  uint32_t* o = blockhist + (size_t)sidx * LO;
  for (int j = threadIdx.x; j < LO; j += 1024) o[j] = h[j];
}
__global__ void __launch_bounds__(1024) k_s2_prefix2(uint32_t* __restrict__ blockhist, S2Geom g, const uint32_t* __restrict__ part_off, const uint32_t* __restrict__ sc_off, uint32_t* __restrict__ hist, uint32_t* __restrict__ offs) {
  __shared__ uint32_t tmp[17];
  const int q = blockIdx.x, LO = 1 << g.lo_log, w = q / g.P, hi = q - w * g.P;
  const uint32_t s0 = sc_off[q], nk = sc_off[q + 1] - s0;
  const int j0 = 2 * threadIdx.x;
  uint32_t r0 = 0, r1 = 0;
  if (j0 < LO) {
    uint2* col = reinterpret_cast<uint2*>(blockhist + (size_t)s0 * LO + j0);
    for (uint32_t k = 0; k < nk; k++) { uint2* pq = col + (size_t)k * (LO / 2); const uint2 v = *pq; *pq = make_uint2(r0, r1); r0 += v.x; r1 += v.y; }
  }
  uint32_t total; const uint32_t r = s2_block_scan(r0 + r1, tmp, &total);
  if (j0 < LO) {
    const size_t b = ((size_t)w * g.P + hi) * LO + j0;
    hist[b] = r0; hist[b + 1] = r1;
    offs[b] = part_off[q] + r; offs[b + 1] = part_off[q] + r + r0;
  }
}
constexpr int S2_EPT = 8;
__host__ __device__ inline size_t s2_place_lds_bytes(int lo_log) { return ((size_t)3 * ((size_t)1 << lo_log) + 32) * 4 + (size_t)1024 * S2_EPT * 6; }
__global__ void __launch_bounds__(1024) k_s2_place(const uint16_t* __restrict__ tmp_lo, const uint32_t* __restrict__ tmp_idx, S2Geom g, const uint32_t* __restrict__ part_off, const uint32_t* __restrict__ part_cnt,
                                                   const uint32_t* __restrict__ sc_off, const uint32_t* __restrict__ blockhist ,
                                                   const uint32_t* __restrict__ offs, uint32_t* __restrict__ sorted, size_t estride) {
  constexpr uint32_t T = 1024 * S2_EPT;
  int q; uint32_t sidx, k2; if (!s2_decode(g, sc_off, q, sidx, k2)) return;
  const int LO = 1 << g.lo_log, tid = threadIdx.x;
  uint32_t* cnt = s2_lds; uint32_t* base = cnt + LO; uint32_t* cur = base + LO; uint32_t* tmp = cur + LO;
  uint32_t* stage_idx = tmp + 32; uint16_t* stage_lo = reinterpret_cast<uint16_t*>(stage_idx + T);
  const int w = q / g.P, hi = q - w * g.P;
  const size_t nb = (size_t)g.P << g.lo_log;
  const uint32_t* b0 = blockhist + (size_t)sidx * LO;
  const uint32_t* of = offs + (size_t)w * nb + ((size_t)hi << g.lo_log);
  for (int j = tid; j < LO; j += 1024) { cur[j] = of[j] + b0[j]; cnt[j] = 0; }
  __syncthreads();
  size_t e0, e1; s2_range(g, part_off, part_cnt, q, k2, e0, e1);
  uint32_t* out = sorted + (size_t)w * estride;
  for (size_t tile = e0; tile < e1; tile += T) {
    uint32_t lo[S2_EPT], idx[S2_EPT], rank[S2_EPT];
#pragma unroll
    for (int i = 0; i < S2_EPT; i++) {
      const size_t e = tile + (size_t)i * 1024 + tid;
      lo[i] = 0xffffffffu;
      if (e < e1) { lo[i] = tmp_lo[e]; idx[i] = tmp_idx[e]; rank[i] = atomicAdd(&cnt[lo[i]], 1u); }
    }
    __syncthreads();
    uint32_t total;
    {
      const int j0 = 2 * tid, j1 = 2 * tid + 1;
      const uint32_t v0 = j0 < LO ? cnt[j0] : 0, v1 = j1 < LO ? cnt[j1] : 0;
      const uint32_t r = s2_block_scan(v0 + v1, tmp, &total);
      if (j0 < LO) base[j0] = r;
      if (j1 < LO) base[j1] = r + v0;
    }
    __syncthreads();
#pragma unroll
    for (int i = 0; i < S2_EPT; i++) {
      if (lo[i] == 0xffffffffu) continue;
      const uint32_t pos = base[lo[i]] + rank[i];
      stage_idx[pos] = idx[i]; stage_lo[pos] = (uint16_t)lo[i];
    }
    __syncthreads();
    for (uint32_t j = tid; j < total; j += 1024) {
      const uint32_t l = stage_lo[j];
      out[cur[l] + (j - base[l])] = stage_idx[j];
    }
    __syncthreads();
    for (int j = tid; j < LO; j += 1024) { cur[j] += cnt[j]; cnt[j] = 0; }
    __syncthreads();
  }
}

}
```

Measured before the change: 748.1 million points/s.

## Pack low radix digit and sign into index word for two-level sort

When the index bits plus sign plus low-digit bits fit in 32, the scatter pass writes one packed u32 per entry instead of a u32 index plus a separate u16 low digit. The hist and place kernels unpack it, and the GLV gap is applied at place time. This cuts intermediate HBM traffic and drops the tmp_lo buffer. k_s2_hist also gains vectorized uint4 loads and per-wavefront privatized LDS histogram copies to reduce atomic contention, at the cost of a reduction over the copies and more template instantiations.

```diff
diff --git a/include/sbn254.h b/include/sbn254.h
--- a/include/sbn254.h
+++ b/include/sbn254.h
@@ -247,7 +247,7 @@
 int sbn_prof_reset(sbn_ctx* ctx);
 int sbn_prof_count(sbn_ctx* ctx);
 int sbn_prof_get(sbn_ctx* ctx, int i, const char** name, double* total_ms, uint64_t* launches);
-int sbn_prof_last_job(sbn_ctx* ctx, uint64_t out[4]);
+int sbn_prof_last_job(sbn_ctx* ctx, uint64_t out[5]);
 int sbn_prof_last_acc(sbn_ctx* ctx, uint64_t out[8]);
 
 int sbn_prof_last_polyeval(sbn_ctx* ctx, double out_us[3]);
diff --git a/spartan-bn254_amd/binding.py b/spartan-bn254_amd/binding.py
--- a/spartan-bn254_amd/binding.py
+++ b/spartan-bn254_amd/binding.py
@@ -995,8 +995,8 @@
         self._chk(lib().sbn_prof_enable(self.h, int(on)), "prof_enable")
 
     def prof_last_job(self):
-        o = (C.c_uint64 * 4)(); self._chk(lib().sbn_prof_last_job(self.h, o), "prof_last_job")
-        return {"c": int(o[0]), "W": int(o[1]), "slots": int(o[2]), "buckets": int(o[3])}
+        o = (C.c_uint64 * 5)(); self._chk(lib().sbn_prof_last_job(self.h, o), "prof_last_job")
+        return {"c": int(o[0]), "W": int(o[1]), "slots": int(o[2]), "buckets": int(o[3]), "sort2_entry": int(o[4])}
 
     def prof_last_acc(self):
         o = (C.c_uint64 * 8)(); self._chk(lib().sbn_prof_last_acc(self.h, o), "prof_last_acc")
diff --git a/spartan-bn254_amd/csrc/abi_derefs_key.inc b/spartan-bn254_amd/csrc/abi_derefs_key.inc
--- a/spartan-bn254_amd/csrc/abi_derefs_key.inc
+++ b/spartan-bn254_amd/csrc/abi_derefs_key.inc
@@ -78,7 +78,7 @@
   if (hipMalloc(&pts->d_pts, len * 64) != hipSuccess || hipMalloc(&kp->d_ids, len * 4) != hipSuccess) { (void)hipGetLastError(); return bail(fail(c, SBN_ENOMEM, "derefs key: hipMalloc of %zu points", len)); }
   if (hipMemcpyAsync(kp->d_ids, kp->ids.data(), len * 4, hipMemcpyHostToDevice, c->stream) != hipSuccess) return bail(fail(c, SBN_EHIP, "derefs key: upload of the cell ids"));
   if (hipMemsetAsync(ctr, 0, 64 + (ACC_SEG_MAX + 2) * 4, c->stream) != hipSuccess) return bail(fail(c, SBN_EHIP, "derefs key: clearing the counters"));
-  c->last_job[0] = 0; c->last_job[1] = 2; c->last_job[2] = (uint64_t)(2 * bN); c->last_job[3] = (uint64_t)NB;
+  c->last_job[0] = 0; c->last_job[1] = 2; c->last_job[2] = (uint64_t)(2 * bN); c->last_job[3] = (uint64_t)NB; c->last_job[4] = 0;
   c->last_acc[0] = SEG; c->last_acc[1] = 1; c->last_acc[2] = 0; c->last_acc[3] = 0; c->last_acc[4] = 0; c->last_acc[5] = 0;
   LAUNCH(c, "k_scan", k_scan, 2, 1024, hist, offs, (int)cells);
   LAUNCH(c, "k_dk_place", k_dk_place, stream_grid(2 * bN), 256, (const uint32_t*)dn->u32s, bN, (uint32_t)cells, hist, (const uint32_t*)offs, sorted);
diff --git a/spartan-bn254_amd/csrc/ctx.hpp b/spartan-bn254_amd/csrc/ctx.hpp
--- a/spartan-bn254_amd/csrc/ctx.hpp
+++ b/spartan-bn254_amd/csrc/ctx.hpp
@@ -50,7 +50,7 @@
   uint32_t* h_bad = nullptr;
   uint32_t* mbox = nullptr; uint32_t mbox_seq = 0;
   std::vector<std::pair<void*, size_t>> pool; size_t pool_bytes = 0;
-  uint64_t last_job[4] = {0, 0, 0, 0};
+  uint64_t last_job[5] = {0, 0, 0, 0, 0};
   uint64_t last_acc[6] = {0, 0, 0, 0, 0, 0};
   double polyeval_us[3] = {0, 0, 0};
   bool prof = false;
diff --git a/spartan-bn254_amd/csrc/msm_host.hpp b/spartan-bn254_amd/csrc/msm_host.hpp
--- a/spartan-bn254_amd/csrc/msm_host.hpp
+++ b/spartan-bn254_amd/csrc/msm_host.hpp
@@ -44,9 +44,12 @@
 static bool sort2_set_lds() {
   bool ok = true;
   const int bytes = (int)s2_scatter_lds_bytes(S2_P_MAX);
-  if (hipFuncSetAttribute((const void*)k_s2_place, hipFuncAttributeMaxDynamicSharedMemorySize, (int)s2_place_lds_bytes(S2_LO_LOG_MAX)) != hipSuccess) { (void)hipGetLastError(); ok = false; }
+  if (hipFuncSetAttribute((const void*)k_s2_place<false>, hipFuncAttributeMaxDynamicSharedMemorySize, (int)s2_place_lds_bytes(S2_LO_LOG_MAX)) != hipSuccess) { (void)hipGetLastError(); ok = false; }
+  if (hipFuncSetAttribute((const void*)k_s2_place<true>, hipFuncAttributeMaxDynamicSharedMemorySize, (int)s2_place_lds_bytes(S2_LO_LOG_MAX)) != hipSuccess) { (void)hipGetLastError(); ok = false; }
 #define X(C) if (hipFuncSetAttribute((const void*)k_s2_scatter<C, S2_SPT>, hipFuncAttributeMaxDynamicSharedMemorySize, bytes) != hipSuccess) { (void)hipGetLastError(); ok = false; } \
-             if (hipFuncSetAttribute((const void*)k_s2_scatter<C, S2_SPT_SMALL>, hipFuncAttributeMaxDynamicSharedMemorySize, bytes) != hipSuccess) { (void)hipGetLastError(); ok = false; }
+             if (hipFuncSetAttribute((const void*)k_s2_scatter<C, S2_SPT_SMALL>, hipFuncAttributeMaxDynamicSharedMemorySize, bytes) != hipSuccess) { (void)hipGetLastError(); ok = false; } \
+             if (hipFuncSetAttribute((const void*)k_s2_scatter<C, S2_SPT, 8, true>, hipFuncAttributeMaxDynamicSharedMemorySize, bytes) != hipSuccess) { (void)hipGetLastError(); ok = false; } \
+             if (hipFuncSetAttribute((const void*)k_s2_scatter<C, S2_SPT_SMALL, 8, true>, hipFuncAttributeMaxDynamicSharedMemorySize, bytes) != hipSuccess) { (void)hipGetLastError(); ok = false; }
   S2_FOR_EACH_C(X)
 #undef X
   const int cnt_bytes = 24 * S2_P_MAX * 4;
@@ -57,7 +60,9 @@
 #define X(C) if (hipFuncSetAttribute((const void*)k_s2_count<C, S2_SPT, 4>, hipFuncAttributeMaxDynamicSharedMemorySize, cnt_bytes) != hipSuccess) { (void)hipGetLastError(); ok = false; } \
              if (hipFuncSetAttribute((const void*)k_s2_count<C, S2_SPT_SMALL, 4>, hipFuncAttributeMaxDynamicSharedMemorySize, cnt_bytes) != hipSuccess) { (void)hipGetLastError(); ok = false; } \
              if (hipFuncSetAttribute((const void*)k_s2_scatter<C, S2_SPT, 4>, hipFuncAttributeMaxDynamicSharedMemorySize, bytes) != hipSuccess) { (void)hipGetLastError(); ok = false; } \
-             if (hipFuncSetAttribute((const void*)k_s2_scatter<C, S2_SPT_SMALL, 4>, hipFuncAttributeMaxDynamicSharedMemorySize, bytes) != hipSuccess) { (void)hipGetLastError(); ok = false; }
+             if (hipFuncSetAttribute((const void*)k_s2_scatter<C, S2_SPT_SMALL, 4>, hipFuncAttributeMaxDynamicSharedMemorySize, bytes) != hipSuccess) { (void)hipGetLastError(); ok = false; } \
+             if (hipFuncSetAttribute((const void*)k_s2_scatter<C, S2_SPT, 4, true>, hipFuncAttributeMaxDynamicSharedMemorySize, bytes) != hipSuccess) { (void)hipGetLastError(); ok = false; } \
+             if (hipFuncSetAttribute((const void*)k_s2_scatter<C, S2_SPT_SMALL, 4, true>, hipFuncAttributeMaxDynamicSharedMemorySize, bytes) != hipSuccess) { (void)hipGetLastError(); ok = false; }
   S2_GLV_FOR_EACH_C(X)
 #undef X
   return ok;
@@ -79,16 +84,24 @@
   if (const char* e = getenv("SBN_SORT2_SPT")) { const int v = atoi(e); if (v == S2_SPT || v == S2_SPT_SMALL) spt = v; }
   const size_t ch = (size_t)1024 * spt;
   g.K = (int)((n + ch - 1) / ch);
+  bool pack = s2_pack_fits(n, g.lo_log);
+  if (const char* e = getenv("SBN_SORT2_PACK")) {
+    const int v = atoi(e);
+    if (v == 1 && !pack) return fail(c, SBN_EINVAL, "two-level sort: SBN_SORT2_PACK=1, but %d index bits + sign + %d lo bits exceed 32", s2_index_bits(n), g.lo_log);
+    if (v == 0) pack = false;
+  }
+  g.ib = s2_index_bits(n);
+  c->last_job[4] = pack ? 2 : 1;
   const size_t WP = (size_t)g.W * g.P;
   const size_t max_sc = ((size_t)g.W * n) / S2_SUB + WP;
   int rc;
   if ((rc = ensure(c, c->s2_cnt, WP * g.K * 4))) return rc;
   if ((rc = ensure(c, c->s2_part, (3 * WP + 1) * 4))) return rc;
   if ((rc = ensure(c, c->s2_idx, (size_t)g.W * n * 4))) return rc;
-  if ((rc = ensure(c, c->s2_lo, (size_t)g.W * n * 2))) return rc;
+  if (!pack && (rc = ensure(c, c->s2_lo, (size_t)g.W * n * 2))) return rc;
   if ((rc = ensure(c, c->blockhist, max_sc * LO * 4))) return rc;
   uint32_t* cntA = (uint32_t*)c->s2_cnt.p; uint32_t* part_cnt = (uint32_t*)c->s2_part.p; uint32_t* part_off = part_cnt + WP; uint32_t* sc_off = part_off + WP;
-  uint32_t* tmp_idx = (uint32_t*)c->s2_idx.p; uint16_t* tmp_lo = (uint16_t*)c->s2_lo.p; uint32_t* bh = (uint32_t*)c->blockhist.p;
+  uint32_t* tmp_idx = (uint32_t*)c->s2_idx.p; uint16_t* tmp_lo = pack ? nullptr : (uint16_t*)c->s2_lo.p; uint32_t* bh = (uint32_t*)c->blockhist.p;
   const size_t lds_a = WP * 4, lds_c = s2_scatter_lds_bytes(g.P, spt);
   if (lds_a > (size_t)24 * S2_P_MAX * 4) return fail(c, SBN_EINVAL, "two-level sort: %zu level-1 counters do not fit the LDS granted to k_s2_count", WP);
   {
@@ -110,24 +123,28 @@
   {
     ProfScope _ps(c, "k_s2_scatter");
     if (glv) switch (s.c) {
-#define X(C) case C: if (spt == S2_SPT) hipLaunchKernelGGL((k_s2_scatter<C, S2_SPT, 4>), dim3(g.K), dim3(1024), lds_c, c->stream, scalars, g, (const uint32_t*)cntA, (const uint32_t*)part_off, tmp_idx, tmp_lo); \
-                     else hipLaunchKernelGGL((k_s2_scatter<C, S2_SPT_SMALL, 4>), dim3(g.K), dim3(1024), lds_c, c->stream, scalars, g, (const uint32_t*)cntA, (const uint32_t*)part_off, tmp_idx, tmp_lo); break;
+#define S2_SCATTER(C, SPT, SW) do { if (pack) hipLaunchKernelGGL((k_s2_scatter<C, SPT, SW, true>), dim3(g.K), dim3(1024), lds_c, c->stream, scalars, g, (const uint32_t*)cntA, (const uint32_t*)part_off, tmp_idx, tmp_lo); \
+                                     else hipLaunchKernelGGL((k_s2_scatter<C, SPT, SW, false>), dim3(g.K), dim3(1024), lds_c, c->stream, scalars, g, (const uint32_t*)cntA, (const uint32_t*)part_off, tmp_idx, tmp_lo); } while (0)
+#define X(C) case C: if (spt == S2_SPT) S2_SCATTER(C, S2_SPT, 4); else S2_SCATTER(C, S2_SPT_SMALL, 4); break;
       S2_GLV_FOR_EACH_C(X)
 #undef X
     } else switch (s.c) {
-#define X(C) case C: if (spt == S2_SPT) hipLaunchKernelGGL((k_s2_scatter<C, S2_SPT>), dim3(g.K), dim3(1024), lds_c, c->stream, scalars, g, (const uint32_t*)cntA, (const uint32_t*)part_off, tmp_idx, tmp_lo); \
-                     else hipLaunchKernelGGL((k_s2_scatter<C, S2_SPT_SMALL>), dim3(g.K), dim3(1024), lds_c, c->stream, scalars, g, (const uint32_t*)cntA, (const uint32_t*)part_off, tmp_idx, tmp_lo); break;
+#define X(C) case C: if (spt == S2_SPT) S2_SCATTER(C, S2_SPT, 8); else S2_SCATTER(C, S2_SPT_SMALL, 8); break;
       S2_FOR_EACH_C(X)
 #undef X
+#undef S2_SCATTER
     }
   }
   const unsigned l2 = s2_level2_blocks(max_sc);
-  LAUNCH(c, "k_s2_hist", k_s2_hist, l2, 1024, (const uint16_t*)tmp_lo, g, (const uint32_t*)part_off, (const uint32_t*)part_cnt, (const uint32_t*)sc_off, bh);
+  if (pack) LAUNCH(c, "k_s2_hist", k_s2_hist<true>, l2, 1024, (const void*)tmp_idx, g, (const uint32_t*)part_off, (const uint32_t*)part_cnt, (const uint32_t*)sc_off, bh);
+  else LAUNCH(c, "k_s2_hist", k_s2_hist<false>, l2, 1024, (const void*)tmp_lo, g, (const uint32_t*)part_off, (const uint32_t*)part_cnt, (const uint32_t*)sc_off, bh);
   LAUNCH(c, "k_s2_prefix", k_s2_prefix2, (unsigned)WP, 1024, bh, g, (const uint32_t*)part_off, (const uint32_t*)sc_off, hist, offs);
   {
     ProfScope _ps(c, "k_s2_place");
-    hipLaunchKernelGGL(k_s2_place, dim3(l2), dim3(1024), s2_place_lds_bytes(g.lo_log), c->stream,
-                       (const uint16_t*)tmp_lo, (const uint32_t*)tmp_idx, g, (const uint32_t*)part_off, (const uint32_t*)part_cnt, (const uint32_t*)sc_off, (const uint32_t*)bh, (const uint32_t*)offs, sorted, estride);
+    if (pack) hipLaunchKernelGGL(k_s2_place<true>, dim3(l2), dim3(1024), s2_place_lds_bytes(g.lo_log), c->stream,
+                                 (const uint16_t*)tmp_lo, (const uint32_t*)tmp_idx, g, (const uint32_t*)part_off, (const uint32_t*)part_cnt, (const uint32_t*)sc_off, (const uint32_t*)bh, (const uint32_t*)offs, sorted, estride);
+    else hipLaunchKernelGGL(k_s2_place<false>, dim3(l2), dim3(1024), s2_place_lds_bytes(g.lo_log), c->stream,
+                            (const uint16_t*)tmp_lo, (const uint32_t*)tmp_idx, g, (const uint32_t*)part_off, (const uint32_t*)part_cnt, (const uint32_t*)sc_off, (const uint32_t*)bh, (const uint32_t*)offs, sorted, estride);
   }
   LAUNCHCHK(c);
   return SBN_OK;
@@ -149,6 +166,7 @@
   if (NB > 0xffffffffull) return fail(c, SBN_EINVAL, "bucket space too large");
   const size_t estride = J.da.estride;
   c->last_job[0] = (uint64_t)s.c; c->last_job[1] = (uint64_t)s.W; c->last_job[2] = (uint64_t)(J.P * estride); c->last_job[3] = (uint64_t)NB;
+  c->last_job[4] = 0;
   size_t mean = estride / (size_t)s.nb + 1;
   uint32_t SEG = 32; while (SEG < 2 * mean && SEG < ACC_SEG_MAX) SEG <<= 1;
   if (NB < 262144) { const size_t total = J.P * estride; uint32_t cap = 32; while ((size_t)cap * 262144 < total && cap < ACC_SEG_MAX) cap <<= 1; if (SEG > cap) SEG = cap; }
@@ -448,7 +466,7 @@
     if ((rc = ensure(c, c->wsum, L * 128))) return rc;
     if ((rc = ensure(c, c->comb_partial, S > 1 ? L * S * 128 : L * 257 * 128))) return rc;
     if (L > 0x7fffffffull || ncol * (size_t)s.W > 0x7fffffffull) return fail(c, SBN_EINVAL, "commit: too many rows / columns");
-    c->last_job[0] = (uint64_t)s.c; c->last_job[1] = (uint64_t)s.W; c->last_job[2] = (uint64_t)(L * ncol * (size_t)s.W); c->last_job[3] = 0;
+    c->last_job[0] = (uint64_t)s.c; c->last_job[1] = (uint64_t)s.W; c->last_job[2] = (uint64_t)(L * ncol * (size_t)s.W); c->last_job[3] = 0; c->last_job[4] = 0;
     if (S > 1) {
       LAUNCH(c, "k_comb_rows", k_comb_rows_flat, dim3((unsigned)L, S), 256, (const uint32_t*)b->d_comb, da, s, skip_rows, (uint32_t*)c->comb_partial.p);
       LAUNCH(c, "k_comb_fold", k_comb_fold, (unsigned)L, S > 64 ? 128 : 64, (const uint32_t*)c->comb_partial.p, S, (uint32_t*)c->wsum.p, (const uint8_t*)nullptr, (const uint32_t*)nullptr);
diff --git a/spartan-bn254_amd/csrc/sbn254.hip b/spartan-bn254_amd/csrc/sbn254.hip
--- a/spartan-bn254_amd/csrc/sbn254.hip
+++ b/spartan-bn254_amd/csrc/sbn254.hip
@@ -68,10 +68,10 @@
   if (launches) *launches = c->prof_entries[i].launches;
   return SBN_OK;
 }
-int sbn_prof_last_job(sbn_ctx* c, uint64_t out[4]) {
+int sbn_prof_last_job(sbn_ctx* c, uint64_t out[5]) {
   if (!c || !out) return SBN_EINVAL;
   std::lock_guard<std::mutex> g(c->mu);
-  for (int i = 0; i < 4; i++) out[i] = c->last_job[i];
+  for (int i = 0; i < 5; i++) out[i] = c->last_job[i];
   return SBN_OK;
 }
 int sbn_prof_last_acc(sbn_ctx* c, uint64_t out[8]) {
diff --git a/spartan-bn254_amd/csrc/sort2_kernels.cuh b/spartan-bn254_amd/csrc/sort2_kernels.cuh
--- a/spartan-bn254_amd/csrc/sort2_kernels.cuh
+++ b/spartan-bn254_amd/csrc/sort2_kernels.cuh
@@ -15,7 +15,10 @@
   int lo_log;
   int K;
   size_t half, gap;
+  int ib;
 };
+__host__ __device__ inline int s2_index_bits(size_t n) { int b = 0; while (n > 1 && ((n - 1) >> b)) b++; return b; }
+__host__ __device__ inline bool s2_pack_fits(size_t n, int lo_log) { return s2_index_bits(n) + 1 + lo_log <= 32; }
 
 template <int C, int SW = 8> struct S2Shape {
   static constexpr int BITS = SW == 8 ? 254 : 127;
@@ -115,9 +118,9 @@
 __host__ __device__ inline size_t s2_scatter_lds_bytes(int P, int spt = S2_SPT) { return ((size_t)3 * P + 32) * 4 + (size_t)1024 * spt * 8; }
 struct S2ScatterArgs {
   const uint32_t* cntA; const uint32_t* part_off; uint32_t* tmp_idx; uint16_t* tmp_lo;
-  size_t n, half, gap; int P, K, k, lo_log;
+  size_t n, half, gap; int P, K, k, lo_log, ib;
 };
-template <int C, int w, int SPT>
+template <int C, int w, int SPT, bool PACK>
 __device__ __forceinline__ void s2_scatter_window(const s2_u32x8 (&kk)[SPT], uint32_t (&carry)[SPT], const S2ScatterArgs& a) {
   constexpr int CH = 1024 * SPT;
   const int P = a.P, tid = threadIdx.x;
@@ -148,26 +151,37 @@
     const uint32_t b = (uint32_t)((d[i] < 0 ? -d[i] : d[i]) - 1), hi = b >> a.lo_log;
     const uint32_t pos = base[hi] + rank[i];
     size_t e = t0 + (size_t)i * 1024;
-    if (a.gap && e >= a.half) e += a.gap;
-    stage_idx[pos] = (uint32_t)e | (d[i] < 0 ? 0x80000000u : 0u);
-    stage_lo[pos] = (uint16_t)(b & ((1u << a.lo_log) - 1u)); stage_hi[pos] = (uint16_t)hi;
-  }
-  __syncthreads();
-  uint32_t* oi = a.tmp_idx + (size_t)w * a.n; uint16_t* ol = a.tmp_lo + (size_t)w * a.n;
-  for (uint32_t j = tid; j < total; j += 1024) {
-    const uint32_t pos = j + gdelta[stage_hi[j]];
-    oi[pos] = stage_idx[j]; ol[pos] = stage_lo[j];
-  }
-  __syncthreads();
-}
-template <int C, int SPT, int... Ws>
+    const uint32_t lo = b & ((1u << a.lo_log) - 1u);
+    if constexpr (PACK) {
+      stage_idx[pos] = (uint32_t)e | ((d[i] < 0 ? 1u : 0u) << a.ib) | (lo << (a.ib + 1));
+    } else {
+      if (a.gap && e >= a.half) e += a.gap;
+      stage_idx[pos] = (uint32_t)e | (d[i] < 0 ? 0x80000000u : 0u);
+      stage_lo[pos] = (uint16_t)lo;
+    }
+    stage_hi[pos] = (uint16_t)hi;
+  }
+  __syncthreads();
+  uint32_t* oi = a.tmp_idx + (size_t)w * a.n;
+  if constexpr (PACK) {
+    for (uint32_t j = tid; j < total; j += 1024) oi[j + gdelta[stage_hi[j]]] = stage_idx[j];
+  } else {
+    uint16_t* ol = a.tmp_lo + (size_t)w * a.n;
+    for (uint32_t j = tid; j < total; j += 1024) {
+      const uint32_t pos = j + gdelta[stage_hi[j]];
+      oi[pos] = stage_idx[j]; ol[pos] = stage_lo[j];
+    }
+  }
+  __syncthreads();
+}
+template <int C, int SPT, bool PACK, int... Ws>
 __device__ __forceinline__ void s2_scatter_windows(const s2_u32x8 (&kk)[SPT], uint32_t (&carry)[SPT], const S2ScatterArgs& a, std::integer_sequence<int, Ws...>) {
-  (s2_scatter_window<C, Ws, SPT>(kk, carry, a), ...);
-}
-template <int C, int SPT, int SW = 8>
+  (s2_scatter_window<C, Ws, SPT, PACK>(kk, carry, a), ...);
+}
+template <int C, int SPT, int SW = 8, bool PACK = false>
 __global__ void __launch_bounds__(1024) k_s2_scatter(const uint32_t* __restrict__ scalars, S2Geom g, const uint32_t* __restrict__ cntA ,
                                                      const uint32_t* __restrict__ part_off, uint32_t* __restrict__ tmp_idx, uint16_t* __restrict__ tmp_lo) {
-  S2ScatterArgs a; a.cntA = cntA; a.part_off = part_off; a.tmp_idx = tmp_idx; a.tmp_lo = tmp_lo; a.n = g.n; a.P = g.P; a.K = g.K; a.k = blockIdx.x; a.lo_log = g.lo_log;
+  S2ScatterArgs a; a.cntA = cntA; a.part_off = part_off; a.tmp_idx = tmp_idx; a.tmp_lo = tmp_lo; a.n = g.n; a.P = g.P; a.K = g.K; a.k = blockIdx.x; a.lo_log = g.lo_log; a.ib = g.ib;
   a.half = g.half; a.gap = SW == 8 ? 0 : g.gap;
   s2_u32x8 kk[SPT]; uint32_t carry[SPT];
 #pragma unroll
@@ -176,7 +190,7 @@
     carry[i] = 0;
     kk[i] = t < g.n ? s2_load_scalar<SW>(scalars, t) : (s2_u32x8)(0u);
   }
-  s2_scatter_windows<C, SPT>(kk, carry, a, std::make_integer_sequence<int, S2Shape<C, SW>::W>{});
+  s2_scatter_windows<C, SPT, PACK>(kk, carry, a, std::make_integer_sequence<int, S2Shape<C, SW>::W>{});
 }
 
 __device__ __forceinline__ bool s2_decode(const S2Geom& g, const uint32_t* __restrict__ sc_off, int& q, uint32_t& sidx, uint32_t& k2) {
@@ -196,17 +210,47 @@
   const size_t w = (size_t)(q / g.P);
   e0 = w * g.n + start + a; e1 = w * g.n + start + b;
 }
-__global__ void __launch_bounds__(1024) k_s2_hist(const uint16_t* __restrict__ tmp_lo, S2Geom g, const uint32_t* __restrict__ part_off, const uint32_t* __restrict__ part_cnt, const uint32_t* __restrict__ sc_off, uint32_t* __restrict__ blockhist) {
-  __shared__ uint32_t h[S2_LO_MAX];
+constexpr int S2_HIST_WORDS = 16384;
+template <bool PACK>
+__global__ void __launch_bounds__(1024) k_s2_hist(const void* __restrict__ ent, S2Geom g, const uint32_t* __restrict__ part_off, const uint32_t* __restrict__ part_cnt, const uint32_t* __restrict__ sc_off, uint32_t* __restrict__ blockhist) {
+  __shared__ uint32_t h[S2_HIST_WORDS];
   int q; uint32_t sidx, k2; if (!s2_decode(g, sc_off, q, sidx, k2)) return;
-  const int LO = 1 << g.lo_log;
-  for (int j = threadIdx.x; j < LO; j += 1024) h[j] = 0;
-  __syncthreads();
+  const int LO = 1 << g.lo_log, tid = threadIdx.x;
+  int copies = 16; while (copies * LO > S2_HIST_WORDS) copies >>= 1;
+  for (int j = tid; j < copies * LO; j += 1024) h[j] = 0;
+  __syncthreads();
+  uint32_t* mine = h + (size_t)((tid >> 6) & (copies - 1)) * LO;
   size_t e0, e1; s2_range(g, part_off, part_cnt, q, k2, e0, e1);
-  for (size_t e = e0 + threadIdx.x; e < e1; e += 1024) atomicAdd(&h[tmp_lo[e]], 1u);
+  constexpr size_t V = PACK ? 4 : 8;
+  size_t a0 = (e0 + V - 1) & ~(V - 1); if (a0 > e1) a0 = e1;
+  const size_t a1 = a0 + ((e1 - a0) & ~(V - 1));
+  const uint4* vec = reinterpret_cast<const uint4*>(ent);
+  const int sh = g.ib + 1;
+  auto count4 = [&](const uint4 x) {
+    if constexpr (PACK) {
+      atomicAdd(&mine[x.x >> sh], 1u); atomicAdd(&mine[x.y >> sh], 1u); atomicAdd(&mine[x.z >> sh], 1u); atomicAdd(&mine[x.w >> sh], 1u);
+    } else {
+      atomicAdd(&mine[x.x & 0xffffu], 1u); atomicAdd(&mine[x.x >> 16], 1u); atomicAdd(&mine[x.y & 0xffffu], 1u); atomicAdd(&mine[x.y >> 16], 1u);
+      atomicAdd(&mine[x.z & 0xffffu], 1u); atomicAdd(&mine[x.z >> 16], 1u); atomicAdd(&mine[x.w & 0xffffu], 1u); atomicAdd(&mine[x.w >> 16], 1u);
+    }
+  };
+  auto lo_of = [&](size_t e) -> uint32_t {
+    if constexpr (PACK) return reinterpret_cast<const uint32_t*>(ent)[e] >> sh;
+    else return reinterpret_cast<const uint16_t*>(ent)[e];
+  };
+  for (size_t e = e0 + tid; e < a0; e += 1024) atomicAdd(&mine[lo_of(e)], 1u);
+  const size_t v1 = a1 / V;
+  for (size_t vb = a0 / V; vb < v1; vb += 4 * 1024) {
+    uint4 x[4];
+#pragma unroll
+    for (int k = 0; k < 4; k++) { const size_t v = vb + (size_t)k * 1024 + tid; x[k] = vec[v < v1 ? v : v1 - 1]; }
+#pragma unroll
+    for (int k = 0; k < 4; k++) if (vb + (size_t)k * 1024 + tid < v1) count4(x[k]);
+  }
+  for (size_t e = a1 + tid; e < e1; e += 1024) atomicAdd(&mine[lo_of(e)], 1u);
   __syncthreads();
   uint32_t* o = blockhist + (size_t)sidx * LO;
-  for (int j = threadIdx.x; j < LO; j += 1024) o[j] = h[j];
+  for (int j = tid; j < LO; j += 1024) { uint32_t t = 0; for (int c = 0; c < copies; c++) t += h[c * LO + j]; o[j] = t; }
 }
 __global__ void __launch_bounds__(1024) k_s2_prefix2(uint32_t* __restrict__ blockhist, S2Geom g, const uint32_t* __restrict__ part_off, const uint32_t* __restrict__ sc_off, uint32_t* __restrict__ hist, uint32_t* __restrict__ offs) {
   __shared__ uint32_t tmp[17];
@@ -227,6 +271,7 @@
 }
 constexpr int S2_EPT = 8;
 __host__ __device__ inline size_t s2_place_lds_bytes(int lo_log) { return ((size_t)3 * ((size_t)1 << lo_log) + 32) * 4 + (size_t)1024 * S2_EPT * 6; }
+template <bool PACK>
 __global__ void __launch_bounds__(1024) k_s2_place(const uint16_t* __restrict__ tmp_lo, const uint32_t* __restrict__ tmp_idx, S2Geom g, const uint32_t* __restrict__ part_off, const uint32_t* __restrict__ part_cnt,
                                                    const uint32_t* __restrict__ sc_off, const uint32_t* __restrict__ blockhist ,
                                                    const uint32_t* __restrict__ offs, uint32_t* __restrict__ sorted, size_t estride) {
@@ -243,13 +288,32 @@
   __syncthreads();
   size_t e0, e1; s2_range(g, part_off, part_cnt, q, k2, e0, e1);
   uint32_t* out = sorted + (size_t)w * estride;
+  const int sh = g.ib + 1; const uint32_t imask = (1u << g.ib) - 1u;
+  const uint32_t half = (uint32_t)g.half, gap = (uint32_t)g.gap;
   for (size_t tile = e0; tile < e1; tile += T) {
     uint32_t lo[S2_EPT], idx[S2_EPT], rank[S2_EPT];
-#pragma unroll
-    for (int i = 0; i < S2_EPT; i++) {
-      const size_t e = tile + (size_t)i * 1024 + tid;
-      lo[i] = 0xffffffffu;
-      if (e < e1) { lo[i] = tmp_lo[e]; idx[i] = tmp_idx[e]; rank[i] = atomicAdd(&cnt[lo[i]], 1u); }
+    if constexpr (PACK) {
+      const uint32_t live = e1 - tile < T ? (uint32_t)(e1 - tile) : T;
+      const uint32_t* ti = tmp_idx + tile;
+#pragma unroll
+      for (int i = 0; i < S2_EPT; i++) {
+        const uint32_t o = (uint32_t)i * 1024u + (uint32_t)tid, x = ti[o < live ? o : live - 1];
+        uint32_t t = x & imask;
+        if (gap && t >= half) t += gap;
+        idx[i] = t | (((x >> g.ib) & 1u) << 31); lo[i] = x >> sh;
+      }
+#pragma unroll
+      for (int i = 0; i < S2_EPT; i++) {
+        if ((uint32_t)i * 1024u + (uint32_t)tid < live) rank[i] = atomicAdd(&cnt[lo[i]], 1u);
+        else lo[i] = 0xffffffffu;
+      }
+    } else {
+#pragma unroll
+      for (int i = 0; i < S2_EPT; i++) {
+        const size_t e = tile + (size_t)i * 1024 + tid;
+        lo[i] = 0xffffffffu;
+        if (e < e1) { lo[i] = tmp_lo[e]; idx[i] = tmp_idx[e]; rank[i] = atomicAdd(&cnt[lo[i]], 1u); }
+      }
     }
     __syncthreads();
     uint32_t total;
```

New measurement: 752.7 million points/s (median of 6 runs). Within noise of the previous version (+0.6%).
